# av-savchenko/HSE_FaceRec_tf

Measured on AMD Instinct MI355X. Metric: faces/sec embedding-extract (MobileNet-192, bs=256), higher is better.
Workload: dtype f32

## Files before the change

### hse_facerec_tf_amd/csrc/common.h

```cpp
#pragma once
#include <hip/hip_runtime.h>
#include <stdarg.h>
#include <stdio.h>

#include "../../include/hsefr.h"
#ifdef HSEFR_DEV
#include "hsefr_dev.h"
#endif

namespace hsefr {

void set_error(const char* fmt, ...);

#define HSEFR_HIP_CHECK(expr)                                                          \
    do {                                                                               \
        hipError_t _e = (expr);                                                        \
        if (_e != hipSuccess) {                                                        \
            ::hsefr::set_error("%s failed: %s (%s:%d)", #expr, hipGetErrorString(_e),  \
                               __FILE__, __LINE__);                                    \
            return HSEFR_ERR_HIP;                                                      \
        }                                                                              \
    } while (0)

#define HSEFR_REQUIRE(cond, code, ...)     \
// ... 88 lines not shown
__device__ __forceinline__ unsigned hsefr_udiv_do(unsigned x, hsefr_udiv k) {
    const unsigned q0 = __umulhi(x, k.m);
    return (((x - q0) >> 1) + q0) >> k.sh;
}

__device__ __forceinline__ unsigned xcd_remap_dir(unsigned bid, unsigned nwg, int reverse) {
    const unsigned lt = xcd_remap(bid, nwg);
    return reverse ? nwg - 1u - lt : lt;
}
int sweep_reverse();
void set_sweep_reverse(int v);

#ifdef HSEFR_DEV
#define HSEFR_KNOB(name, value) int name = value
#else
#define HSEFR_KNOB(name, value) constexpr int name = value
#endif

int launch_conv_c3(const float* x, const float* wgt, const float* shift, float* y, int n, int h, int w,
                   int kh, int kw, int stride, int pad_t, int pad_l, int oh, int ow, int cout, int act,
                   hipStream_t s);
int launch_dwconv3x3(const float* x, const float* wgt, const float* scale, const float* shift, float* y,
                     int n, int h, int w, int c, int stride, int pad_t, int pad_l, int oh, int ow, int act,
                     hipStream_t s);
int launch_dwconv3x3_split(const float* x, const float* wgt, const float* scale, const float* shift, void* y_split,
                           int n, int h, int w, int c, int stride, int pad_t, int pad_l, int oh, int ow, int act,
                           int a_log2, hipStream_t s);
int launch_pwconv_f32(const float* x, const float* wgt_t, const float* shift, float* y, long long m, int k,
                      int cout, int act, hipStream_t s);
int launch_pwconv_f16s(const float* x, const void* wsplit, const float* descale, const float* shift, float* y,
                       long long m, int k, int cout, int a_log2, int act, hipStream_t s);
bool pwconv_ps_supported(long long m, int k, int cout);
bool pwconv_ps_gap_supported(long long m, int k, int cout, int map_hw);
int launch_pwconv_ps_gap(const void* xs, const void* wsplit, const float* descale, const float* shift, float* y, long long m, int k, int cout,
                         int act, int map_hw, hipStream_t s);
bool pwconv_ps_dw_supported(long long m, int k, int cout, int map_w, int map_hw, int dw_stride);
int launch_pwconv_ps_dw(const void* xs, const void* wsplit, const float* descale, const float* shift, const float* dwc, void* ys, long long m,
                        int k, int cout, int act, int map_w, int map_hw, int dw_stride, int out_log2, hipStream_t s);
int launch_pwconv_ps(const void* xs, const void* wsplit, const float* descale, const float* shift, float* y, long long m, int k,
                     int cout, int act, hipStream_t s);
int launch_gap(const float* x, float* y, int n, int hw, int c, hipStream_t s);
int launch_dense(const float* x, const float* wgt, const float* bias, float* y, int n, int k, int cout,
                 int act, hipStream_t s);
int launch_softmax(const float* x, float* y, int n, int c, hipStream_t s);
int launch_heads_fused(const float* x, const float* w1, const float* b1, const float* wa, const float* ba, const float* wg, const float* bg,
                       float* hidden, float* logits, float* age_probs, float* gender, int n, int k, int a, hipStream_t s);
int launch_l2_normalize(const float* x, float* y, int n, int d, hipStream_t s);
int launch_nn1(const float* q, const float* g, int nq, int ng, int d, int* nn_index, float* nn_dist2,
               hipStream_t s);
int launch_knn(const float* q, const float* g, int nq, int ng, int d, int k, int* nn_index, float* nn_dist2, const int* g_label, int* pred,
               hipStream_t s);
long long nn1_fallbacks();

int launch_conv_bf16(const void* x, const void* wt, const float* scale, const float* shift, const void* res, void* y,
                     int n, int h, int w, int c, int oh, int ow, int cout, int kh, int kw, int stride, int pad_t,
                     int pad_l, int act, hipStream_t s);
int launch_conv1x1_bf16(const void* x, const void* wt, const float* scale, const float* shift, const void* res, void* y,
                        long long P, int K, int cout, int act, hipStream_t s);
int launch_conv1x1_sres_bf16(const void* x, const void* wt, const float* scale, const float* shift, const void* res, void* y, int n, int oh,
                             int ow, int K, int cout, int stride, int h2, int w2, int act, hipStream_t s);
bool conv1x1_bf16_enabled(bool has_res, int k, int cout);
int launch_conv1x1_proj_bf16(const void* x, const void* wt, const float* scale, const float* shift, const void* x2, const void* wt2,
                             const float* scale2, const float* shift2, void* y, int n, int oh, int ow, int K, int cout, int k2, int stride,
                             int h2, int w2, int act, hipStream_t s);
int launch_stem7x7_bf16(const float* x, const void* wt, const float* scale, const float* shift, void* y, int n, int h,
                        int w, int oh, int ow, int act, hipStream_t s);
int mtcnn_post_capacity();
int launch_mtcnn_stage1_level(const float* prob, const float* reg, int w, int h, double scale, float thr, double* found, int* counters,
                              hipStream_t s);
int launch_mtcnn_stage1_finish(const double* found, int* counters, double* boxes, int* tab, int img_w, int img_h, hipStream_t s);
int launch_mtcnn_stage23_finish(int stage, const double* boxes_in, int n, const float* prob, const float* reg, const float* pts, float thr,
                                double* boxes_out, int* tab_out, float* points_out, int* counters, int img_w, int img_h, hipStream_t s);
int launch_mtcnn_nms(const double* boxes, int n, double thr, int use_min, int* keep, int* n_keep, hipStream_t s);
bool conv3x3_win_forced();
bool conv3x3_win_bf16_supported(long long n, int h, int w, int c, int cout);
int launch_conv3x3_win_bf16(const void* x, const void* wt, const float* scale, const float* shift, const void* res, void* y, int n, int h,
                            int w, int c, int cout, int act, hipStream_t s);
bool conv3x3_w2_forced();
bool conv3x3_w2_bf16_supported(long long n, int h, int w, int c, int cout);
bool conv3x3_w2_bf16_preferred(int h, int w, int cout);
int launch_conv3x3_w2_bf16(const void* x, const void* wt, const float* scale, const float* shift, const void* res, void* y, int n, int h,
                           int w, int c, int cout, int act, hipStream_t s);
bool conv1x1_w4_forced();
bool conv1x1_w4_bf16_supported(long long n, int h, int w, int c, int oh, int ow, int cout, int stride);
bool conv1x1_w4_bf16_preferred(long long pixels, int c, int cout, bool has_res);
bool conv1x1_w4_proj_preferred(long long pixels, int c, int c2, int cout);
int launch_conv1x1_w4_proj_bf16(const void* x, const void* wt, const float* scale, const float* shift, const void* x2, const void* wt2,
                                const float* scale2, const float* shift2, void* y, int n, int oh, int ow, int c, int cout, int c2, int stride2,
                                int h2, int w2, int act, hipStream_t s);
int launch_conv1x1_w4_bf16(const void* x, const void* wt, const float* scale, const float* shift, const void* res, void* y, int n, int h,
                           int w, int c, int oh, int ow, int cout, int stride, int act, hipStream_t s);
bool conv1x1_pair_bf16_shape_supported(int c, int cout1, int cout2, int c2);
bool conv1x1_pair_bf16_supported(long long pixels, int c, int cout1, int cout2, int c2);
int launch_conv1x1_pair_bf16(const void* x, const void* w1, const float* scale1, const float* shift1, const void* res, const void* x2,
                             const void* wp, const float* scale_p, const float* shift_p, void* y1, const void* w2, const float* scale2,
                             const float* shift2, void* y2, long long pixels, int c, int cout1, int cout2, int c2, int act1, int act2,
                             hipStream_t s, int y1_stride = 1, int h = 0, int w = 0);
bool conv_dma_forced();
bool conv_dma_bf16_supported(long long n, int h, int w, int c, int oh, int ow, int cout, int kh, int kw);
int launch_conv_dma_bf16(const void* x, const void* wt, const float* scale, const float* shift, const void* res, void* y, int n, int h,
                         int w, int c, int oh, int ow, int cout, int kh, int kw, int stride, int pad_t, int pad_l, int act, hipStream_t s);
int launch_stem7x7_pool_bf16(const float* x, const void* wt, const float* scale, const float* shift, void* y, int n, int h, int w,
                             int ph, int pw, int pool_pad_t, int pool_pad_l, hipStream_t s, const void* wfrag = nullptr);
bool stem7s_stream_supported(long long n, int h, int w, int ph, int pw);
int launch_stem7s_stream(const float* x, const void* wt, const float* scale, const float* shift, void* y, int n, int h, int w, int ph, int pw,
                         int pool_pad_t, int pool_pad_l, hipStream_t s, const void* wfrag = nullptr);
constexpr size_t STEM7S_WFRAG_BYTES = 4 * 7 * 64 * 16;
int stem7s_reorder_weights(const void* wt, void* wfrag, hipStream_t s);
int launch_maxpool3x3s2_bf16(const void* x, void* y, int n, int h, int w, int c, int oh, int ow, int pad_t, int pad_l,
                             hipStream_t s);
int launch_gap_bf16(const void* x, float* y, int n, int hw, int c, hipStream_t s);

int launch_pil_resize(const unsigned char* in, unsigned char* tmp, float* out, int n, int H, int W, int oh, int ow, const int* xmin,
                      const int* xcnt, const int* xcoef, int xk, const int* ymin, const int* ycnt, const int* ycoef, int yk,
                      int mode, const double* mean, hipStream_t s);
int launch_cv_resize(const unsigned char* in, float* out, int n, int H, int W, int oh, int ow, const int* x0, const int* x1,
                     const int* wx1, const int* y0, const int* y1, const int* wy1, int mode, const double* mean, hipStream_t s);

int launch_area_level(const unsigned char* src, float* dst, int sh, int sw, int dh, int dw, hipStream_t s);
int launch_area_crops(const unsigned char* src, const int* boxes, float* dst, int sh, int sw, int n, int size, hipStream_t s);
int launch_pairwise_dist(const float* x, const float* y, int n, int m, int d, float* out, hipStream_t s);
struct DistSource {
    const float* x;
    int n, d;
    const float* born;
    const float* year;
    const double* dense;
};
int launch_single_linkage(const DistSource& src, int* edge_a, int* edge_b, double* edge_h, hipStream_t s);
int launch_dbscan(const DistSource& src, double eps, int min_samples, int* labels, unsigned char* core, hipStream_t s);
int launch_rank_order(const DistSource& src, const double* thresholds, int pairs, int* labels, int* iterations, hipStream_t s);
int launch_hier_linkage(const DistSource& src, int method, int* merge_a, int* merge_b, double* merge_h, int* merge_round, hipStream_t s);

bool dwpw_fused_supported(int c, int cout, int stride, int act_dw, int act_pw);
int launch_dwpw_fused(const float* x, const float* wd, const float* dscale, const float* dshift, const float* wp_t,
                      const float* pshift, float* y, int n, int h, int w, int c, int stride, int pad_t, int pad_l, int oh,
                      int ow, int cout, int act_dw, int act_pw, hipStream_t s);

int launch_conv2d_direct(const float* x, const float* w, const float* bias, const float* alpha, float* y, int n, int h, int wd, int c,
                         int oh, int ow, int cout, int kh, int kw, int stride, int pad_t, int pad_l, hipStream_t s);
int launch_conv_f32_mfma(const float* x, const float* w, const float* scale, const float* shift, const float* res, float* y, int n, int h,
                         int wd, int c, int oh, int ow, int cout, int kh, int kw, int stride, int pad_t, int pad_l, int act, hipStream_t s,
                         int res_stride = 0, int res_h = 0, int res_w = 0);
bool conv_f32_mfma_supported(int c, int cout);
int launch_conv2d_f32(const float* x, const float* w, const float* scale, const float* shift, const float* res, float* y, int n, int h,
                      int wd, int c, int oh, int ow, int cout, int kh, int kw, int stride, int pad_t, int pad_l, int act, hipStream_t s);
int launch_maxpool_f32(const float* x, float* y, int n, int h, int w, int c, int oh, int ow, int k, int stride, int pad_t, int pad_l,
                       hipStream_t s);

int launch_dwpw_f16s(const float* x, const float* wd, const float* dscale, const float* dshift, const void* wsplit,
                     const float* descale, const float* pshift, float* y, int n, int h, int w, int c, int stride, int pad_t,
                     int pad_l, int oh, int ow, int cout, int a_log2, int act, hipStream_t s);
bool dwpw_f16s_supported(int c, int cout, int stride);
int launch_stem_fused(const float* x, const float* cw, const float* cshift, const float* wd, const float* dscale,
                      const float* dshift, const void* wsplit, const float* descale, const float* pshift, float* y, int n,
                      int h, int w, int cpad_t, int cpad_l, int oh, int ow, int a_log2, int act, hipStream_t s);
int launch_stem2_fused(const float* x, const float* cw, const float* cshift, const float* wd1, const float* d1scale,
                       const float* d1shift, const void* wsplit, const float* descale, const float* pshift, const float* wd2,
                       const float* d2scale, const float* d2shift, float* y, int n, int h, int w, int cpad_t, int cpad_l,
                       int h1, int w1, int pad_t2, int pad_l2, int oh2, int ow2, int a_log2, int act, hipStream_t s);
int launch_stem3_fused(const float* x, const void* cw_split, const float* cdescale, const float* cshift, const float* wd1,
                       const float* d1scale, const float* d1shift, const void* wsplit, const float* descale, const float* pshift,
                       const float* wd2, const float* d2scale, const float* d2shift, float* y, int* overflow, int n, int h, int w,
                       int cpad_t, int cpad_l, int h1, int w1, int pad_t2, int pad_l2, int oh2, int ow2, int in_log2, int a_log2,
                       int act, hipStream_t s);
bool stem3_fused_supported(int cin, int c1, int c2, int conv_stride, int dw1_stride, int dw2_stride, int kh, int kw);
int launch_stem4_fused(const void* x, int x_is_u8, const void* cw4, const float* cdescale, const float* cshift, const float* wd1,
                       const float* d1scale, const float* d1shift, const void* wsplit, const float* descale, const float* pshift,
                       const float* wd2, const float* d2scale, const float* d2shift, float* y, int* overflow, int n, int h, int w,
                       int in_log2, int a_log2, int act, hipStream_t s);
bool stem4_fused_supported(int cin, int c1, int c2, int conv_stride, int dw1_stride, int dw2_stride, int kh, int kw, int h, int w);
int launch_stem5_stream(const void* x, int x_is_u8, const void* cw4, const float* cdescale, const float* cshift, const float* wd1,
                        const float* d1scale, const float* d1shift, const void* wsplit, const float* descale, const float* pshift,
                        const float* wd2, const float* d2scale, const float* d2shift, float* y, int* overflow, int n, int h, int w,
                        int in_log2, int a_log2, int act, hipStream_t s);
bool stem5_stream_supported(int cin, int c1, int c2, int conv_stride, int dw1_stride, int dw2_stride, int kh, int kw, int h, int w);
bool stem2_fused_supported(int cin, int c1, int c2, int conv_stride, int dw1_stride, int dw2_stride, int kh, int kw);
bool stem_fused_supported(int cin, int cmid, int cout, int conv_stride, int dw_stride, int kh, int kw);
int read_pws_stamps(void* host_out, size_t bytes);
int read_stem_stamps(void* host_out, size_t bytes);
#ifdef HSEFR_STEM_STAMPS
unsigned long long* stamp_buffer(hipStream_t s);
#define STEM_STAMP(i) do { const unsigned long long _t = __builtin_amdgcn_s_memtime(); st[i] += _t - tprev; tprev = _t; } while (0)
#define STEM_STAMP_DECL unsigned long long st[8] = {0, 0, 0, 0, 0, 0, 0, 0}; unsigned long long tprev = __builtin_amdgcn_s_memtime(); \
    const unsigned long long tstart = tprev; unsigned npatch = 0
#define STEM_STAMP_COUNT ++npatch
#define STEM_STAMP_FLUSH(buf, lane, wave) do { if ((lane) == 0 && (buf) && blockIdx.x < 512) { unsigned long long* o = (buf) + (blockIdx.x * 4 + (wave)) * 10; \
    for (int i_ = 0; i_ < 8; ++i_) o[i_] = st[i_]; o[8] = __builtin_amdgcn_s_memtime() - tstart; o[9] = npatch; } } while (0)
#else
#define STEM_STAMP(i) do { } while (0)
#define STEM_STAMP_DECL do { } while (0)
#define STEM_STAMP_COUNT do { } while (0)
#define STEM_STAMP_FLUSH(buf, lane, wave) do { } while (0)
#endif
#ifdef HSEFR_DEV
void set_stem4_grid(int v);
void set_stem5_grid(int v);
void set_stem5_segs(int v);
void set_c11(int v);
void set_c11_tile(int v);
void set_c11_bres(int v);
void set_c11_adv(int v);
int read_c11_stamps(void* host_out, size_t bytes);
void set_dwpws_tw(int v);
void set_dwpws_bn(int v);
void set_pw_tile(int v);
void set_pws_tile(int v);
void set_ps_mb(int v);
void set_ps_grid(int v);
void set_psdw_mode(int v);
void set_cd_rb(int v);
void set_w3_off(int v);
void set_w2_off(int v);
void set_w4_off(int v);
void set_w4_bres(int v);
void set_pair_off(int v);
void set_stem7s(int v);
void set_pair_ablate(int v);
void set_pair_nt(int v);
void set_nn1_y_mb(int v);
int read_w4_stamps(void* host_out, size_t bytes);
int read_s7_stamps(void* host_out, size_t bytes);
int read_w2_stamps(void* host_out, size_t bytes);
int read_w3_stamps(void* host_out, size_t bytes);
int read_cd_stamps(void* host_out, size_t bytes);
void set_cd_off(int v);
int read_ps_stamps(void* host_out, size_t bytes);
void set_pw_ablate(int v);
void set_pw_dma(int v);
void set_dw_th(int v);
void set_dw_variant(int v);
void set_dw_look(int v);
void set_dw_look2(int v);
void set_copy_variant(int v);
void set_clock_mode(int v);
void set_c3_impl(int v);
int launch_clock_probe(unsigned long long* out, int blocks, int iters, hipStream_t s);
int launch_copy(const void* src, void* dst, size_t bytes, hipStream_t s);
#endif

}
```

### hse_facerec_tf_amd/csrc/dwpw_f16s.hip

```cpp
#include "common.h"

namespace hsefr {

namespace {

typedef float f32x4 __attribute__((ext_vector_type(4)));
typedef float f32x16 __attribute__((ext_vector_type(16)));
typedef _Float16 f16x4 __attribute__((ext_vector_type(4)));
typedef _Float16 f16x8 __attribute__((ext_vector_type(8)));

struct DwPwSParams {
    const float4* x;
    const float4* wd;
    const float4* dscale;
    const float4* dshift;
    const float* wsplit;
    const float* descale;
    const float* pshift;
    float* y;
    int H, W, C4, KT, OH, OW, Cout, pad_t, pad_l, tiles_w, tiles_h, tiles_n;
    unsigned total;
    float a_scale;
    int reverse;
    int nimg;
    unsigned m_n, m_w, m_h;
    unsigned long long* stamps;
};

constexpr int ROWB = 128;
__device__ __forceinline__ int swzb(int row, int chunk) { return row * ROWB + 16 * (chunk ^ ((row >> 1) & 7) ^ ((row & 1) << 2)); }
__device__ __forceinline__ float4 fma4(float4 a, float4 b, float4 c) {
    return make_float4(fmaf(a.x, b.x, c.x), fmaf(a.y, b.y, c.y), fmaf(a.z, b.z, c.z), fmaf(a.w, b.w, c.w));
}
__device__ __forceinline__ float relu6(float v) { return fminf(fmaxf(v, 0.f), 6.f); }
__device__ __forceinline__ unsigned fastdiv(unsigned x, unsigned m) { return m ? __umulhi(x, m) : x; }

template <int STRIDE, int TW, int BN, int OCC, int ACT>
__global__ __launch_bounds__(256, OCC) void dwpw_f16s_kernel(DwPwSParams p) {
    constexpr int TH = 128 / TW;
    constexpr int U = TW * 8;
    constexpr int RG = 256 / U;
    constexpr int RPT = TH / RG;
    static_assert(RPT == 4, "patch shapes 8x16 and 16x8");
    constexpr int WN = BN / 2, NI = WN / 32, BP = BN / 32;
    __shared__ __attribute__((aligned(16))) unsigned char As[128 * ROWB];
    __shared__ __attribute__((aligned(16))) unsigned char Bs[BN * ROWB];

    const int tid = threadIdx.x;
    const int lane = tid & 63, wave = tid >> 6;
    const int wm = wave >> 1, wn = wave & 1;
    const int li = lane & 31, lh = lane >> 5;
    const int srow = tid >> 3, skq = tid & 7;
    const int u = tid % U, tw = u >> 3, c4l = u & 7;
    const int row0 = (tid / U) * RPT;
    const int arow = wm * 64 + li, brow = wn * WN + li;

    for (unsigned t = blockIdx.x; t < p.total; t += gridDim.x) {
        const unsigned lt = xcd_remap_dir(t, p.total, p.reverse);
        const int n0 = (lt % p.tiles_n) * BN;
        const unsigned pt = lt / p.tiles_n;
        const int ow0 = (pt % p.tiles_w) * TW;
        const int oh0 = ((pt / p.tiles_w) % p.tiles_h) * TH;
        const int n = pt / (p.tiles_w * p.tiles_h);

        const int ow = min(ow0 + tw, p.OW - 1);
        const int iw0 = ow * STRIDE - p.pad_l;
        const float ml = iw0 >= 0 ? 1.f : 0.f, mm = (iw0 + 1 >= 0 && iw0 + 1 < p.W) ? 1.f : 0.f, mr = iw0 + 2 < p.W ? 1.f : 0.f;
        const int cl = max(iw0, 0) * p.C4, cm = min(max(iw0 + 1, 0), p.W - 1) * p.C4, cr = min(iw0 + 2, p.W - 1) * p.C4;
        const float4* ximg = p.x + (size_t)n * p.H * p.W * p.C4;
        const int ih0 = (oh0 + row0) * STRIDE - p.pad_t;
        const float* bsrc = p.wsplit + (size_t)(n0 + srow) * p.KT * 32 + 4 * skq;

        f32x16 acc[2][NI];
#pragma unroll
        for (int mi = 0; mi < 2; ++mi)
#pragma unroll
            for (int ni = 0; ni < NI; ++ni)
#pragma unroll
                for (int r = 0; r < 16; ++r) acc[mi][ni][r] = 0.f;

        for (int kc = 0; kc < p.KT; ++kc) {
            f32x4 rb[BP];
#pragma unroll
            for (int q = 0; q < BP; ++q) rb[q] = *(const f32x4*)(bsrc + (size_t)32 * q * p.KT * 32 + kc * 32);
            const int c4 = kc * 8 + c4l;
            const float4* xin = ximg + c4;
            float4 wk[9];
#pragma unroll
            for (int i = 0; i < 9; ++i) {
                const float m = (i % 3 == 0) ? ml : (i % 3 == 1 ? mm : mr);
                const float4 wr = p.wd[i * p.C4 + c4];
                wk[i] = make_float4(wr.x * m, wr.y * m, wr.z * m, wr.w * m);
            }
            const float4 dsc = p.dscale[c4], dsh = p.dshift[c4];
            struct Row { float4 l, m, r; float k; };
            auto load_row = [&](int ih) {
                Row q;
                const int ihc = min(max(ih, 0), p.H - 1);
                const float4* row = xin + (size_t)ihc * p.W * p.C4;
                q.l = row[cl]; q.m = row[cm]; q.r = row[cr];
                q.k = (ih >= 0 && ih < p.H) ? 1.f : 0.f;
                return q;
            };
            auto row_sum = [&](const Row& q, int b) {
                float4 a = make_float4(q.l.x * wk[b].x, q.l.y * wk[b].y, q.l.z * wk[b].z, q.l.w * wk[b].w);
                a = fma4(q.m, wk[b + 1], a);
                return fma4(q.r, wk[b + 2], a);
            };
            f16x4 ohi[RPT], olo[RPT];
            auto emit = [&](int j, const Row& a, const Row& b, const Row& c) {
                const float4 sa = row_sum(a, 0), sb = row_sum(b, 3), sc = row_sum(c, 6);
                float4 s = make_float4(sa.x * a.k, sa.y * a.k, sa.z * a.k, sa.w * a.k);
                s = make_float4(fmaf(sb.x, b.k, s.x), fmaf(sb.y, b.k, s.y), fmaf(sb.z, b.k, s.z), fmaf(sb.w, b.k, s.w));
                s = make_float4(fmaf(sc.x, c.k, s.x), fmaf(sc.y, c.k, s.y), fmaf(sc.z, c.k, s.z), fmaf(sc.w, c.k, s.w));
                const float4 o = fma4(s, dsc, dsh);
                f32x4 v;
                v[0] = relu6(o.x); v[1] = relu6(o.y); v[2] = relu6(o.z); v[3] = relu6(o.w);
                v = v * p.a_scale;
                ohi[j] = __builtin_convertvector(v, f16x4);
                olo[j] = __builtin_convertvector(v - __builtin_convertvector(ohi[j], f32x4), f16x4);
            };
            if (STRIDE == 1) {
                Row r0 = load_row(ih0), r1 = load_row(ih0 + 1), r2 = load_row(ih0 + 2), r3 = load_row(ih0 + 3);
#pragma unroll
                for (int j = 0; j < RPT; ++j) {
                    const Row r4 = load_row(ih0 + j + 4);
                    emit(j, r0, r1, r2);
                    r0 = r1; r1 = r2; r2 = r3; r3 = r4;
                }
            } else {
                Row r0 = load_row(ih0), r1 = load_row(ih0 + 1), r2 = load_row(ih0 + 2);
#pragma unroll
                for (int j = 0; j < RPT; ++j) {
                    const Row n1 = load_row(ih0 + 2 * j + 3), n2 = load_row(ih0 + 2 * j + 4);
                    emit(j, r0, r1, r2);
                    r0 = r2; r1 = n1; r2 = n2;
                }
            }
            __syncthreads();
#pragma unroll
            for (int j = 0; j < RPT; ++j) {
                const int R = (row0 + j) * TW + tw;
                *(f16x4*)(&As[swzb(R, c4l >> 1) + 8 * (c4l & 1)]) = ohi[j];
                *(f16x4*)(&As[swzb(R, 4 + (c4l >> 1)) + 8 * (c4l & 1)]) = olo[j];
            }
#pragma unroll
            for (int q = 0; q < BP; ++q) *(f32x4*)(&Bs[swzb(srow + 32 * q, skq)]) = rb[q];
            __syncthreads();
#pragma unroll
            for (int s = 0; s < 2; ++s) {
                f16x8 ah[2], al[2], bh[NI], bl[NI];
#pragma unroll
// ... 191 lines not shown
        const int cw = wave - 4, wm = cw / CWN, wn = cw % CWN;
        const int li = lane & 31, lh = lane >> 5;
        const int arow = wm * 64 + li, brow = wn * WN + li;
        const int erow = lane >> 3, ech = lane & 7;
        unsigned bv[BPW];
        unsigned pb_i = 0;
        int pb_kc = 0, pb_step = 0;
        auto setup_b = [&](unsigned i) {
            const Item it = decode(i);
#pragma unroll
            for (int j = 0; j < BPW; ++j) {
                const int r = (cw * BPW + j) * 8 + (lane >> 3);
                bv[j] = ((unsigned)(it.n0 + r) * (unsigned)C + 4u * ((lane & 7) ^ ((r >> 1) & 7) ^ ((r & 1) << 2))) * 4u;
            }
        };
        auto b_dma = [&]() {
            const unsigned base = lds0 + B_OFF + (pb_step & 1) * B_ST;
            const unsigned so = (unsigned)pb_kc * 128u;
#pragma unroll
            for (int j = 0; j < BPW; ++j) piece(rw, base + (cw * BPW + j) * 1024, bv[j], so);
            ++pb_step;
            if (++pb_kc == KT) {
                pb_kc = 0;
                setup_b(++pb_i);
            }
        };
        f32x16 acc[2][NI];
        auto zero_acc = [&]() {
#pragma unroll
            for (int mi = 0; mi < 2; ++mi)
#pragma unroll
                for (int ni = 0; ni < NI; ++ni)
#pragma unroll
                    for (int r = 0; r < 16; ++r) acc[mi][ni][r] = 0.f;
        };
        auto epilogue = [&](const Item& cur, int stage) {
            unsigned char* scr = smem + B_OFF + stage * B_ST + cw * (BPW * 1024);
            const float* el = (const float*)(smem + E_OFF);
            unsigned sv[2][4];
#pragma unroll
            for (int mi = 0; mi < 2; ++mi)
#pragma unroll
                for (int i = 0; i < 4; ++i) {
                    const int R = wm * 64 + mi * 32 + erow + 8 * i;
                    const int oh = cur.oh0 + R / TW, ow = cur.ow0 + R % TW;
                    sv[mi][i] = (oh < p.OH && ow < p.OW)
                                    ? ((unsigned)((cur.n * p.OH + oh) * p.OW + ow) * (unsigned)p.Cout + (unsigned)(cur.n0 + wn * WN + 4 * ech)) * 4u
                                    : OOB;
                }
#pragma unroll
            for (int ni = 0; ni < NI; ++ni) {
                const int nl = cur.n0 + wn * WN + ni * 32 + 4 * ech;
                const f32x4 ds = *(const f32x4*)(el + nl), sh = *(const f32x4*)(el + CMAX2 + nl);
#pragma unroll
                for (int mi = 0; mi < 2; ++mi) {
#pragma unroll
                    for (int j = 0; j < 4; ++j) {
                        f32x4 v;
#pragma unroll
                        for (int e = 0; e < 4; ++e) v[e] = acc[mi][ni][4 * j + e];
                        *(f32x4*)(scr + li * 128 + 16 * ((2 * j + lh) ^ (li & 7))) = v;
                    }
                    f32x4 rv[4];
#pragma unroll
                    for (int i = 0; i < 4; ++i) {
                        const int r = erow + 8 * i;
                        rv[i] = *(const f32x4*)(scr + r * 128 + 16 * (ech ^ (r & 7)));
                    }
#pragma unroll
                    for (int i = 0; i < 4; ++i) {
                        const f32x4 v = rv[i];
                        const f32x4 z = __builtin_elementwise_fma(v, ds, sh);
                        f32x4 o;
#pragma unroll
                        for (int e = 0; e < 4; ++e) o[e] = apply_act<ACT>(z[e]);
                        bstore16_welded(o, ry, sv[mi][i], __builtin_amdgcn_readfirstlane((unsigned)(ni * 32) * 4u));
                    }
                }
            }
        };
        zero_acc();
        setup_b(0);
        Item cur = decode(0);
        unsigned ci = 0;
        int ckc = 0;
        bool pending = false;
        if (HALO_BY_CONSUMER) {
            setup_halo(0);
#pragma unroll
            for (int i = 0; i < HS - 1; ++i)
                if (i < nsteps) halo_dma();
            asm volatile("s_waitcnt vmcnt(0)" ::: "memory");
        }
        __syncthreads();
        for (int g = -1; g < nsteps; ++g) {
            if (pending) {
                epilogue(cur, (g + 1) & 1);
                zero_acc();
                cur = decode(++ci);
                pending = false;
                STEM_STAMP_COUNT;
            }
            STEM_STAMP(5);
            if (pb_step < nsteps) b_dma();
            const bool halo_issued = HALO_BY_CONSUMER && pf_step < nsteps;
            if (halo_issued) halo_dma();
            STEM_STAMP(1);
            if (g >= 0) {
                const unsigned char* As = smem + A_OFF + (g & 1) * (128 * ROWB);
                const unsigned char* Bs = smem + B_OFF + (g & 1) * B_ST;
#pragma unroll
                for (int s = 0; s < 2; ++s) {
                    f16x8 ah[2], al[2], bh[NI], bl[NI];
#pragma unroll
                    for (int mi = 0; mi < 2; ++mi) {
                        ah[mi] = *(const f16x8*)(As + swzb(arow + mi * 32, 2 * s + lh));
                        al[mi] = *(const f16x8*)(As + swzb(arow + mi * 32, 4 + 2 * s + lh));
                    }
#pragma unroll
                    for (int ni = 0; ni < NI; ++ni) {
                        bh[ni] = *(const f16x8*)(Bs + swzb(brow + ni * 32, 2 * s + lh));
                        bl[ni] = *(const f16x8*)(Bs + swzb(brow + ni * 32, 4 + 2 * s + lh));
                    }
#pragma unroll
                    for (int mi = 0; mi < 2; ++mi)
#pragma unroll
                        for (int ni = 0; ni < NI; ++ni) {
                            acc[mi][ni] = __builtin_amdgcn_mfma_f32_32x32x16_f16(bh[ni], al[mi], acc[mi][ni], 0, 0, 0);
                            acc[mi][ni] = __builtin_amdgcn_mfma_f32_32x32x16_f16(bl[ni], ah[mi], acc[mi][ni], 0, 0, 0);
                            acc[mi][ni] = __builtin_amdgcn_mfma_f32_32x32x16_f16(bh[ni], ah[mi], acc[mi][ni], 0, 0, 0);
                        }
                }
                if (++ckc == KT) { ckc = 0; pending = true; }
            }
            STEM_STAMP(4);
            if (HS >= 3 && halo_issued) asm volatile("s_waitcnt vmcnt(%0)" ::"n"(HPW) : "memory");
            else asm volatile("s_waitcnt vmcnt(0)" ::: "memory");
            STEM_STAMP(0);
            __syncthreads();
            STEM_STAMP(3);
        }
        if (pending) { epilogue(cur, (nsteps - 1) & 1); STEM_STAMP_COUNT; }
#ifdef HSEFR_STEM_STAMPS
        if (lane == 0 && p.stamps && blockIdx.x < 256 && cw < 4) {
            unsigned long long* o = p.stamps + ((blockIdx.x + 256) * 4 + cw) * 10;
            for (int i_ = 0; i_ < 8; ++i_) o[i_] = st[i_];
            o[8] = __builtin_amdgcn_s_memtime() - tstart;
            o[9] = npatch;
        }
#endif
    }
}

HSEFR_KNOB(g_tw, 0);
HSEFR_KNOB(g_bn, 0);

template <int STRIDE, int TW, int BN, int OCC>
int launch_t(DwPwSParams& p, int n, int act, hipStream_t s) {
    constexpr int TH = 128 / TW;
    p.tiles_w = (p.OW + TW - 1) / TW;
    p.tiles_h = (p.OH + TH - 1) / TH;
    p.tiles_n = p.Cout / BN;
    const long long total = (long long)n * p.tiles_w * p.tiles_h * p.tiles_n;
    HSEFR_REQUIRE(total < (1ll << 31), HSEFR_ERR_UNSUPPORTED, "dwpw_f16split: grid too large");
    p.total = (unsigned)total;
    const unsigned cap = 256u * OCC;
    const unsigned g = p.total < cap ? p.total : cap;
#define HSEFR_DWPWS(A) HSEFR_LAUNCH((dwpw_f16s_kernel<STRIDE, TW, BN, OCC, A>), dim3(g), dim3(256), 0, s, p)
    if (act == HSEFR_ACT_RELU6) HSEFR_DWPWS(HSEFR_ACT_RELU6);
    else if (act == HSEFR_ACT_RELU) HSEFR_DWPWS(HSEFR_ACT_RELU);
    else if (act == HSEFR_ACT_NONE) HSEFR_DWPWS(HSEFR_ACT_NONE);
    else { set_error("dwpw_f16split: act %d", act); return HSEFR_ERR_UNSUPPORTED; }
#undef HSEFR_DWPWS
    return launch_status("dwpw_f16split");
}

template <int STRIDE, int TW>
int launch_bn(DwPwSParams& p, int n, int bn, int act, hipStream_t s) {
    if (bn == 64) return launch_t<STRIDE, TW, 64, 2>(p, n, act, s);
#ifdef HSEFR_DEV
    if (bn == 256) return launch_t<STRIDE, TW, 256, 2>(p, n, act, s);
#endif
    return launch_t<STRIDE, TW, 128, 2>(p, n, act, s);
}

template <int TW, int BN, int HS>
int launch_v3(DwPwSParams& p, int n, int act, hipStream_t s) {
    constexpr int TH = 128 / TW;
    p.tiles_w = (p.OW + TW - 1) / TW;
    p.tiles_h = (p.OH + TH - 1) / TH;
    p.tiles_n = p.Cout / BN;
    const long long total = (long long)n * p.tiles_w * p.tiles_h * p.tiles_n;
    HSEFR_REQUIRE(total < (1ll << 31) / 16, HSEFR_ERR_UNSUPPORTED, "dwpw_f16split: grid too large");
    p.total = (unsigned)total;
    auto magic = [](unsigned d) { return d == 1 ? 0u : (unsigned)((0x100000000ull + d - 1) / d); };
    p.m_n = magic(p.tiles_n); p.m_w = magic(p.tiles_w); p.m_h = magic(p.tiles_h);
    HSEFR_REQUIRE(total * (long long)(p.tiles_n > p.tiles_w ? (p.tiles_n > p.tiles_h ? p.tiles_n : p.tiles_h) : (p.tiles_w > p.tiles_h ? p.tiles_w : p.tiles_h)) < (1ll << 32),
                  HSEFR_ERR_UNSUPPORTED, "dwpw_f16split: grid too large for the quotient multipliers");
    const unsigned g = p.total < 256u ? p.total : 256u;
#define HSEFR_DWPW3(A) HSEFR_LAUNCH((dwpw3_f16s_kernel<TW, BN, HS, A>), dim3(g), dim3(256 + 64 * (BN == 256 ? 8 : 4)), 0, s, p)
    if (act == HSEFR_ACT_RELU6) HSEFR_DWPW3(HSEFR_ACT_RELU6);
    else if (act == HSEFR_ACT_RELU) HSEFR_DWPW3(HSEFR_ACT_RELU);
    else if (act == HSEFR_ACT_NONE) HSEFR_DWPW3(HSEFR_ACT_NONE);
    else { set_error("dwpw_f16split: act %d", act); return HSEFR_ERR_UNSUPPORTED; }
#undef HSEFR_DWPW3
    return launch_status("dwpw_f16split");
}

}

#ifdef HSEFR_DEV
void set_dwpws_tw(int v) { g_tw = v; }
void set_dwpws_bn(int v) { g_bn = v; }
#endif

bool dwpw_f16s_supported(int c, int cout, int stride) {
    return c > 0 && c % 32 == 0 && cout > 0 && cout % 64 == 0 && (stride == 1 || stride == 2);
}

int launch_dwpw_f16s(const float* x, const float* wd, const float* dscale, const float* dshift, const void* wsplit,
                     const float* descale, const float* pshift, float* y, int n, int h, int w, int c, int stride, int pad_t,
                     int pad_l, int oh, int ow, int cout, int a_log2, int act, hipStream_t s) {
    HSEFR_REQUIRE(dwpw_f16s_supported(c, cout, stride), HSEFR_ERR_UNSUPPORTED,
                  "dwpw_f16split: c=%d cout=%d stride=%d not covered (c %% 32, cout %% 64, stride 1|2)", c, cout, stride);
    HSEFR_REQUIRE(n >= 0 && h > 0 && w > 0 && oh > 0 && ow > 0, HSEFR_ERR_INVALID, "dwpw_f16split: bad shape");
    HSEFR_REQUIRE(a_log2 > 0 && a_log2 <= 12, HSEFR_ERR_INVALID, "dwpw_f16split: a_log2=%d (the depthwise result is in [0,6]: 1..12)", a_log2);
    if (n == 0) return HSEFR_OK;
    DwPwSParams p;
    p.x = (const float4*)x; p.wd = (const float4*)wd; p.dscale = (const float4*)dscale; p.dshift = (const float4*)dshift;
    p.wsplit = (const float*)wsplit; p.descale = descale; p.pshift = pshift; p.y = y;
    p.H = h; p.W = w; p.C4 = c / 4; p.KT = c / 32; p.OH = oh; p.OW = ow; p.Cout = cout; p.pad_t = pad_t; p.pad_l = pad_l;
    p.a_scale = ldexpf(1.f, a_log2);
    p.reverse = sweep_reverse();
    p.nimg = n;
    p.stamps = nullptr;
#ifdef HSEFR_STEM_STAMPS
    p.stamps = stamp_buffer(s);
#endif
    const long long in_bytes = (long long)n * h * w * c * 4, out_bytes = (long long)n * oh * ow * cout * 4;
    if (stride == 1 && c <= 256 && cout <= CMAX2 && cout % 128 == 0 && in_bytes < (1ll << 32) - 16 && out_bytes < (1ll << 32) - 16) {
        auto padded = [&](int tw) { const int th = 128 / tw; return (long long)((ow + tw - 1) / tw * tw) * ((oh + th - 1) / th * th); };
        int tw = padded(16) <= padded(8) ? 16 : 8;
        if (g_tw == 8 || g_tw == 16) tw = g_tw;
        int bn = cout % 256 == 0 ? 256 : 128;
        if ((g_bn == 128 || g_bn == 256) && cout % g_bn == 0) bn = g_bn;
        if (bn == 256) return tw == 16 ? launch_v3<16, 256, 2>(p, n, act, s) : launch_v3<8, 256, 2>(p, n, act, s);
        return tw == 16 ? launch_v3<16, 128, 3>(p, n, act, s) : launch_v3<8, 128, 3>(p, n, act, s);
    }
    int bn = cout % 128 == 0 ? 128 : 64;
    if (g_bn && cout % g_bn == 0) bn = g_bn;
    int tw = (ow % 16 == 0 || ow % 8 != 0) ? 16 : 8;
    if (ow <= 8) tw = 8;
    if (g_tw == 8 || g_tw == 16) tw = g_tw;
    if (stride == 1) return tw == 16 ? launch_bn<1, 16>(p, n, bn, act, s) : launch_bn<1, 8>(p, n, bn, act, s);
    return tw == 16 ? launch_bn<2, 16>(p, n, bn, act, s) : launch_bn<2, 8>(p, n, bn, act, s);
}

}
```

### hse_facerec_tf_amd/csrc/engine.hip

```cpp
#include <math.h>
#include <string.h>

#include <cxxabi.h>
#include <dlfcn.h>
#include <elf.h>

#include <map>
#include <new>
#include <string>
#include <vector>

#include "common.h"

namespace hsefr {

static thread_local char g_err[512] = "";

void set_error(const char* fmt, ...) {
    va_list ap;
    va_start(ap, fmt);
    vsnprintf(g_err, sizeof(g_err), fmt, ap);
    va_end(ap);
}

// ... 114 lines not shown
                          "plan op %u: input exceeds buffer %d", i, o.in_buf);
        }
        HSEFR_REQUIRE(o.res_buf != o.out_buf, HSEFR_ERR_INVALID, "plan op %u: residual aliases the output", i);
        auto need = [&](uint64_t off, uint64_t bytes, const char* what) {
            if (off != HSEFR_NO_OFFSET && off + bytes <= h.blob_bytes) return true;
            set_error("plan op %u (kind %u): operand %s missing or %llu bytes beyond the %llu-byte blob", i, o.kind, what,
                      (unsigned long long)bytes, (unsigned long long)h.blob_bytes);
            return false;
        };
        const uint64_t co = o.cout, ci = o.cin, kk = (uint64_t)o.kh * o.kw;
        const Geometry g = geometry(o.aux);
        switch (o.kind) {
            case HSEFR_OP_GAP: case HSEFR_OP_SOFTMAX: case HSEFR_OP_MAXPOOL_BF16: case HSEFR_OP_GAP_BF16: case HSEFR_OP_MAXPOOL_F32:
                break;
            case HSEFR_OP_CONV_F32:
                if (!need(o.w_off, kk * ci * co * 4, "kernel")) return HSEFR_ERR_INVALID;
                if (o.scale_off != HSEFR_NO_OFFSET && !need(o.scale_off, co * 4, "scale")) return HSEFR_ERR_INVALID;
                if (o.shift_off != HSEFR_NO_OFFSET && !need(o.shift_off, co * 4, "shift")) return HSEFR_ERR_INVALID;
                HSEFR_REQUIRE(o.cout % 4 == 0, HSEFR_ERR_UNSUPPORTED, "plan op %u: fp32 convolution with cout=%d (must be a multiple of 4)", i, o.cout);
                if (o.aux != 0) {
                    HSEFR_REQUIRE(g.c2 == 0 && o.kh == 1 && o.kw == 1 && o.stride == 1 && o.pad_t == 0 && o.pad_l == 0 && o.res_buf >= 0 && g.stride2 >= 1 &&
                                      o.oh == o.h && o.ow == o.w && o.oh * o.ow > 1 && o.ow > 1 && (o.oh - 1) * g.stride2 < g.h2 &&
                                      (o.ow - 1) * g.stride2 < g.w2 && conv_f32_mfma_supported(o.cin, o.cout),
                                  HSEFR_ERR_INVALID, "plan op %u: bad strided residual (stride %d, %dx%d)", i, g.stride2, g.h2, g.w2);
                    HSEFR_REQUIRE((uint64_t)g.h2 * g.w2 * co * 4 <= bufs[o.res_buf].elems_per_image * bufs[o.res_buf].elem_bytes, HSEFR_ERR_INVALID,
                                  "plan op %u: strided residual exceeds buffer %d", i, o.res_buf);
                }
                break;
            case HSEFR_OP_CONV_C3:
                if (!need(o.w_off, kk * ci * co * 4, "kernel") || !need(o.shift_off, co * 4, "shift")) return HSEFR_ERR_INVALID;
                break;
            case HSEFR_OP_DWCONV3X3:
                if (!need(o.w_off, 9 * ci * 4, "kernel") || !need(o.scale_off, ci * 4, "scale") || !need(o.shift_off, ci * 4, "shift"))
                    return HSEFR_ERR_INVALID;
                HSEFR_REQUIRE(o.aux == 0 || (o.aux > 0 && o.aux <= 12 && o.act == HSEFR_ACT_RELU6 && o.cin % 32 == 0),
                              HSEFR_ERR_INVALID, "plan op %u: split-row depthwise output needs ReLU6, c %% 32 == 0 and a_log2 in [1, 12]", i);
                break;
            case HSEFR_OP_PWCONV_F32:
                if (!need(o.w_off, ci * co * 4, "kernel") || !need(o.shift_off, co * 4, "shift")) return HSEFR_ERR_INVALID;
                break;
            case HSEFR_OP_DENSE:
                if (!need(o.w_off, ci * co * 4, "kernel")) return HSEFR_ERR_INVALID;
                if (o.shift_off != HSEFR_NO_OFFSET && !need(o.shift_off, co * 4, "bias")) return HSEFR_ERR_INVALID;
                break;
            case HSEFR_OP_CONV_BF16:
                if (!need(o.w_off, kk * ci * co * 2, "kernel") || !need(o.scale_off, co * 4, "scale") || !need(o.shift_off, co * 4, "shift"))
                    return HSEFR_ERR_INVALID;
                if (o.w2_off != HSEFR_NO_OFFSET) {
                    HSEFR_REQUIRE(o.kh == 1 && o.kw == 1 && o.stride == 1 && o.res_buf >= 0 && g.c2 > 0 && g.c2 % 64 == 0 && g.stride2 >= 1 &&
                                      (o.oh - 1) * g.stride2 < g.h2 && (o.ow - 1) * g.stride2 < g.w2,
                                  HSEFR_ERR_INVALID, "plan op %u: bad projected shortcut (k2 %d, stride %d, %dx%d)", i, g.c2, g.stride2, g.h2, g.w2);
                    if (!need(o.w2_off, (uint64_t)g.c2 * co * 2, "projection kernel") || !need(o.shift2_off, 2 * co * 4, "projection scale / shift"))
                        return HSEFR_ERR_INVALID;
                    HSEFR_REQUIRE((uint64_t)g.h2 * g.w2 * g.c2 * 2 <= bufs[o.res_buf].elems_per_image * bufs[o.res_buf].elem_bytes, HSEFR_ERR_INVALID,
                                  "plan op %u: projected shortcut input exceeds buffer %d", i, o.res_buf);
                } else if (o.aux != 0) {
                    HSEFR_REQUIRE(g.c2 == 0 && o.kh == 1 && o.kw == 1 && o.stride == 1 && o.pad_t == 0 && o.pad_l == 0 && o.res_buf >= 0 && g.stride2 >= 1 &&
                                      o.oh == o.h && o.ow == o.w && o.oh * o.ow > 1 && o.ow > 1 && (o.oh - 1) * g.stride2 < g.h2 && (o.ow - 1) * g.stride2 < g.w2,
                                  HSEFR_ERR_INVALID, "plan op %u: bad strided residual (stride %d, %dx%d)", i, g.stride2, g.h2, g.w2);
                    HSEFR_REQUIRE((uint64_t)g.h2 * g.w2 * co * 2 <= bufs[o.res_buf].elems_per_image * bufs[o.res_buf].elem_bytes, HSEFR_ERR_INVALID,
                                  "plan op %u: strided residual exceeds buffer %d", i, o.res_buf);
                }
                break;
            case HSEFR_OP_STEM7X7_POOL_BF16:
                HSEFR_REQUIRE(o.act == HSEFR_ACT_RELU && (o.aux & ~(1 | 1 << HSEFR_AUX_POOL_PAD_L_SHIFT)) == 0 && o.cin == 3 && o.cout == 64, HSEFR_ERR_INVALID,
                              "plan op %u: fused stem + pool needs ReLU, 3 -> 64 channels and pool pads in {0, 1}", i);
                [[fallthrough]];
            case HSEFR_OP_STEM7X7_BF16:
                if (!need(o.w_off, 64 * 256 * 2, "kernel") || !need(o.scale_off, co * 4, "scale") || !need(o.shift_off, co * 4, "shift"))
                    return HSEFR_ERR_INVALID;
                break;
            case HSEFR_OP_PWCONV_PS_GAP:
                HSEFR_REQUIRE(pwconv_ps_gap_supported(0, o.cin, o.cout, o.h * o.w) && o.oh == 1 && o.ow == 1, HSEFR_ERR_UNSUPPORTED,
                              "plan op %u: fused pointwise + global pool on a %dx%d map not covered (33 .. 288 pixels)", i, o.h, o.w);
                if (!need(o.w_off, ci * co * 4, "split rows") || !need(o.scale_off, co * 4, "descale") || !need(o.shift_off, co * 4, "shift"))
                    return HSEFR_ERR_INVALID;
                HSEFR_REQUIRE(o.aux > 0 && o.aux <= 24, HSEFR_ERR_INVALID, "plan op %u: a_log2 out of range (reserved %d)", i, o.aux);
                break;
            case HSEFR_OP_PWCONV_PS_DW:
                HSEFR_REQUIRE(pwconv_ps_dw_supported(0, o.cin, o.cout, o.w, o.h * o.w, o.stride) && o.oh * o.stride == o.h && o.ow * o.stride == o.w &&
                                  (o.stride == 1 ? (o.pad_t == 1 && o.pad_l == 1) : (o.pad_t == 0 && o.pad_l == 0)),
                              HSEFR_ERR_UNSUPPORTED, "plan op %u: fused pointwise + depthwise (stride %d) on a %dx%d map not covered", i, o.stride, o.h, o.w);
                if (!need(o.w_off, ci * co * 4, "split rows") || !need(o.scale_off, co * 4, "descale") || !need(o.shift_off, co * 4, "shift") ||
                    !need(o.w2_off, 11 * co * 4, "depthwise constants"))
                    return HSEFR_ERR_INVALID;
                {
                    const PsDwAux a = ps_dw_aux(o.aux);
                    HSEFR_REQUIRE(a.a_log2 > 0 && a.a_log2 <= 24 && a.out_log2 >= 1 && a.out_log2 <= 12,
                                  HSEFR_ERR_INVALID, "plan op %u: a_log2 / out_log2 out of range (reserved %d)", i, o.aux);
                }
                break;
            case HSEFR_OP_PWCONV_PS:
                HSEFR_REQUIRE(pwconv_ps_supported(0, o.cin, o.cout), HSEFR_ERR_UNSUPPORTED,
                              "plan op %u: pre-split pointwise cin=%d cout=%d not covered", i, o.cin, o.cout);
                [[fallthrough]];
            case HSEFR_OP_PWCONV_F16S:
                if (!need(o.w_off, ci * co * 4, "split rows") || !need(o.scale_off, co * 4, "descale") || !need(o.shift_off, co * 4, "shift"))
                    return HSEFR_ERR_INVALID;
                HSEFR_REQUIRE(o.w_off != HSEFR_NO_OFFSET && o.scale_off != HSEFR_NO_OFFSET && o.shift_off != HSEFR_NO_OFFSET &&
                                  o.aux > 0 && o.aux <= 24,
                              HSEFR_ERR_INVALID, "plan op %u: split-f16 pointwise needs split rows, descale, shift and a_log2 in (0, 24]", i);
                break;
            case HSEFR_OP_STEM3_F16S: {
                const StemAux a = stem_aux(o.aux);
                HSEFR_REQUIRE(stem3_fused_supported(o.cin, 32, o.cout, o.stride, 1, 2, o.kh, stem_kw(o.kw).k) && a.a_log2 > 0 && a.a_log2 <= 12 &&
                                  a.in_log2 >= -8 && a.in_log2 <= 14 &&
                                  o.w_off != HSEFR_NO_OFFSET && o.w2_off != HSEFR_NO_OFFSET && o.shift2_off != HSEFR_NO_OFFSET &&
                                  o.w_off + HSEFR_STEM_PACK_STEM3_END * 4 <= h.blob_bytes && o.w2_off + 64 * 128 <= h.blob_bytes &&
                                  o.shift2_off + 128 * 4 <= h.blob_bytes && o.in_buf == HSEFR_BUF_INPUT,
                              HSEFR_ERR_UNSUPPORTED, "plan op %u: bounded fused stem cin=%d cout=%d stride=%d not covered", i, o.cin, o.cout, o.stride);
                break;
            }
            case HSEFR_OP_STEM2_F16S:
                HSEFR_REQUIRE(stem2_fused_supported(o.cin, 32, o.cout, o.stride, 1, 2, o.kh, stem_kw(o.kw).k) && o.aux > 0 && o.aux <= 12 &&
                                  o.w_off != HSEFR_NO_OFFSET && o.w2_off != HSEFR_NO_OFFSET && o.shift2_off != HSEFR_NO_OFFSET &&
                                  o.w_off + HSEFR_STEM_PACK_STEM2_END * 4 <= h.blob_bytes && o.in_buf == HSEFR_BUF_INPUT,
                              HSEFR_ERR_UNSUPPORTED, "plan op %u: fused stem+dw2 cin=%d cout=%d stride=%d not covered", i, o.cin, o.cout, o.stride);
                break;
            case HSEFR_OP_STEM_F16S:
#ifndef HSEFR_DEV
                set_error("plan op %u: HSEFR_OP_STEM_F16S (round 1's fused stem) runs on development builds of the library only", i);
                return HSEFR_ERR_UNSUPPORTED;
#else
                HSEFR_REQUIRE(stem_fused_supported(o.cin, 32, o.cout, o.stride, 1, o.kh, o.kw) && o.aux > 0 && o.aux <= 12 &&
                                  o.w_off != HSEFR_NO_OFFSET && o.w2_off != HSEFR_NO_OFFSET && o.shift2_off != HSEFR_NO_OFFSET &&
                                  o.w_off + HSEFR_STEM_PACK_DW2 * 4 <= h.blob_bytes && o.in_buf == HSEFR_BUF_INPUT,
                              HSEFR_ERR_UNSUPPORTED, "plan op %u: fused stem cin=%d cout=%d stride=%d not covered", i, o.cin, o.cout, o.stride);
                break;
#endif
            case HSEFR_OP_DWPW_F16S:
                if (!need(o.w_off, 9 * ci * 4, "depthwise kernel") || !need(o.scale_off, ci * 4, "scale") || !need(o.shift_off, ci * 4, "shift") ||
                    !need(o.w2_off, ci * co * 4, "split rows") || !need(o.shift2_off, 2 * co * 4, "descale | shift"))
                    return HSEFR_ERR_INVALID;
                HSEFR_REQUIRE(dwpw_f16s_supported(o.cin, o.cout, o.stride) && o.aux > 0 && o.aux <= 12 &&
                                  o.w_off != HSEFR_NO_OFFSET && o.scale_off != HSEFR_NO_OFFSET && o.shift_off != HSEFR_NO_OFFSET &&
                                  o.w2_off != HSEFR_NO_OFFSET && o.shift2_off != HSEFR_NO_OFFSET,
                              HSEFR_ERR_UNSUPPORTED, "plan op %u: split-f16 fused block cin=%d cout=%d stride=%d a_log2=%d not covered",
                              i, o.cin, o.cout, o.stride, o.aux);
                break;
            case HSEFR_OP_DWPW_F32:
                if (!need(o.w_off, 9 * ci * 4, "depthwise kernel") || !need(o.scale_off, ci * 4, "scale") || !need(o.shift_off, ci * 4, "shift") ||
                    !need(o.w2_off, ci * co * 4, "pointwise kernel") || !need(o.shift2_off, co * 4, "pointwise shift"))
                    return HSEFR_ERR_INVALID;
                HSEFR_REQUIRE(dwpw_fused_supported(o.cin, o.cout, o.stride, HSEFR_ACT_RELU6, (int)o.act), HSEFR_ERR_UNSUPPORTED,
                              "plan op %u: fused depthwise-pointwise block cin=%d cout=%d not covered", i, o.cin, o.cout);
                break;
            default:
                set_error("plan op %u: unknown kind %u", i, o.kind);
                return HSEFR_ERR_UNSUPPORTED;
        }
    }
    for (uint32_t i = 0; i < h.n_ops; ++i) {
        const hsefr_plan_op& o = ops[i];
        HSEFR_REQUIRE((o.flags & ~(HSEFR_OPF_PAIR_NEXT | HSEFR_OPF_HEADS | HSEFR_OPF_OUT_SUB2)) == 0, HSEFR_ERR_INVALID, "plan op %u: unknown flags 0x%x", i, o.flags);
        HSEFR_REQUIRE(!(o.flags & HSEFR_OPF_OUT_SUB2) || (o.flags & HSEFR_OPF_PAIR_NEXT), HSEFR_ERR_INVALID, "plan op %u: OUT_SUB2 without PAIR_NEXT", i);
        if (o.flags & HSEFR_OPF_PAIR_NEXT) {
            HSEFR_REQUIRE(i + 1 < h.n_ops, HSEFR_ERR_INVALID, "plan op %u: PAIR_NEXT on the last op", i);
            const hsefr_plan_op& b = ops[i + 1];
            const bool proj = o.w2_off != HSEFR_NO_OFFSET;
            const Geometry g = geometry(o.aux);
            const int c2 = proj ? g.c2 : 0;
            const bool sub2 = (o.flags & HSEFR_OPF_OUT_SUB2) != 0;
            HSEFR_REQUIRE(o.kind == HSEFR_OP_CONV_BF16 && b.kind == HSEFR_OP_CONV_BF16 && o.kh == 1 && o.kw == 1 && o.stride == 1 && o.pad_t == 0 &&
                              o.pad_l == 0 && (sub2 ? (o.oh == (o.h + 1) / 2 && o.ow == (o.w + 1) / 2 && o.h > 1 && o.w > 1) : (o.oh == o.h && o.ow == o.w)) &&
                              b.kh == 1 && b.kw == 1 && b.stride == 1 && b.pad_t == 0 && b.pad_l == 0 &&
                              b.h == o.h && b.w == o.w && b.oh == b.h && b.ow == b.w && b.cin == o.cout && b.in_buf == o.out_buf &&
                              b.res_buf == HSEFR_BUF_NONE && b.w2_off == HSEFR_NO_OFFSET && b.flags == 0 && o.res_buf >= 0 &&
                              (!proj || (g.stride2 == 1 && g.h2 == o.h && g.w2 == o.w)),
                          HSEFR_ERR_INVALID, "plan op %u: PAIR_NEXT needs two 1x1 stride-1 bf16 convolutions at the same pixels, the first with a residual "
                          "or a same-pixel projected shortcut, the second reading the first", i);
            HSEFR_REQUIRE(b.out_buf != o.in_buf && b.out_buf != o.res_buf && b.out_buf != o.out_buf, HSEFR_ERR_INVALID,
                          "plan op %u: PAIR_NEXT: the second output (buffer %d) aliases an operand of the first", i, b.out_buf);
            HSEFR_REQUIRE(conv1x1_pair_bf16_shape_supported(o.cin, o.cout, b.cout, c2), HSEFR_ERR_UNSUPPORTED,
                          "plan op %u: PAIR_NEXT %d -> %d -> %d (projection from %d) not covered", i, o.cin, o.cout, b.cout, c2);
        }
        if (o.flags & HSEFR_OPF_HEADS) {
            HSEFR_REQUIRE(i + 3 < h.n_ops, HSEFR_ERR_INVALID, "plan op %u: HEADS needs three ops behind it", i);
            const hsefr_plan_op &a = ops[i + 1], &sm = ops[i + 2], &g = ops[i + 3];
            HSEFR_REQUIRE(o.kind == HSEFR_OP_DENSE && o.act == HSEFR_ACT_RELU && o.cout == 256 && o.cin > 0 && o.cin % 256 == 0 && o.cin <= 2048 &&
                              o.shift_off != HSEFR_NO_OFFSET && a.kind == HSEFR_OP_DENSE && a.act == HSEFR_ACT_NONE && a.cin == 256 && a.cout >= 1 &&
                              a.cout <= 128 && a.in_buf == o.out_buf && a.shift_off != HSEFR_NO_OFFSET && sm.kind == HSEFR_OP_SOFTMAX &&
                              sm.in_buf == a.out_buf && sm.cout == a.cout && g.kind == HSEFR_OP_DENSE && g.act == HSEFR_ACT_SIGMOID && g.cin == 256 &&
                              g.cout == 1 && g.in_buf == o.out_buf && g.shift_off != HSEFR_NO_OFFSET && a.flags == 0 && sm.flags == 0 && g.flags == 0,
                          HSEFR_ERR_INVALID, "plan op %u: HEADS needs DENSE k -> 256 + ReLU, DENSE 256 -> a (<= 128) + bias, SOFTMAX, DENSE 256 -> 1 + sigmoid", i);
            const int outs[4] = {o.out_buf, a.out_buf, sm.out_buf, g.out_buf};
            for (int x = 0; x < 4; ++x) {
                HSEFR_REQUIRE(outs[x] != o.in_buf, HSEFR_ERR_INVALID, "plan op %u: HEADS: an output aliases the pooled features", i);
                for (int y = x + 1; y < 4; ++y)
                    HSEFR_REQUIRE(outs[x] != outs[y], HSEFR_ERR_INVALID, "plan op %u: HEADS: two of the four tensors share buffer %d", i, outs[x]);
            }
        }
    }
    for (int s = 0; s < HSEFR_N_OUTPUT_SLOTS; ++s) {
        HSEFR_REQUIRE(h.out_buffer[s] == HSEFR_BUF_NONE || (h.out_buffer[s] >= 0 && h.out_buffer[s] < (int)h.n_buffers),
                      HSEFR_ERR_INVALID, "plan: output slot %d names buffer %d", s, h.out_buffer[s]);
        if (h.out_buffer[s] == HSEFR_BUF_NONE) continue;
        const int b = h.out_buffer[s];
        uint32_t producers = 0;
        for (uint32_t i = 0; i < h.n_ops; ++i) producers += (ops[i].out_buf == b);
        HSEFR_REQUIRE(producers == 1, HSEFR_ERR_INVALID, "plan: output slot %d: buffer %d has %u producing ops (must be exactly 1)", s, b,
                      producers);
        HSEFR_REQUIRE((uint64_t)bufs[b].elems_per_image * bufs[b].elem_bytes == (uint64_t)h.out_elems[s] * 4, HSEFR_ERR_INVALID,
                      "plan: output slot %d: buffer %d holds %llu x %u bytes per image, the slot declares %u fp32 elements", s, b,
                      (unsigned long long)bufs[b].elems_per_image, (unsigned)bufs[b].elem_bytes, h.out_elems[s]);
    }
    return HSEFR_OK;
}

namespace hsefr {
#ifdef HSEFR_STEM_STAMPS
static unsigned long long* g_stamp_buf = nullptr;
unsigned long long* stamp_buffer(hipStream_t s) {
    if (!g_stamp_buf && hipMalloc((void**)&g_stamp_buf, 512 * 4 * 10 * 8) != hipSuccess) return nullptr;
    (void)hipMemsetAsync(g_stamp_buf, 0, 512 * 4 * 10 * 8, s);
    return g_stamp_buf;
}
int read_stem_stamps(void* host_out, size_t bytes) {
    HSEFR_REQUIRE(g_stamp_buf && bytes <= 512 * 4 * 10 * 8, HSEFR_ERR_INVALID, "read_stem_stamps: nothing recorded / too many bytes");
    HSEFR_HIP_CHECK(hipMemcpy(host_out, g_stamp_buf, bytes, hipMemcpyDeviceToHost));
    return HSEFR_OK;
}
#else
int read_stem_stamps(void* host_out, size_t bytes) {
    (void)host_out; (void)bytes;
    set_error("read_stem_stamps: library built without -DHSEFR_STEM_STAMPS");
    return HSEFR_ERR_UNSUPPORTED;
}
#endif
static thread_local std::string* g_route_sink = nullptr;
bool route_probe() { return g_route_sink != nullptr; }
static const std::map<uintptr_t, std::string>& stub_names() {
    static const std::map<uintptr_t, std::string> table = [] {
        std::map<uintptr_t, std::string> m;
        Dl_info info;
        if (!dladdr(reinterpret_cast<const void*>(&stub_names), &info) || !info.dli_fname) return m;
        FILE* f = fopen(info.dli_fname, "rb");
        if (!f) return m;
        std::vector<unsigned char> img;
        fseek(f, 0, SEEK_END);
        const long sz = ftell(f);
        fseek(f, 0, SEEK_SET);
        if (sz > 0) { img.resize((size_t)sz); if (fread(img.data(), 1, img.size(), f) != img.size()) img.clear(); }
        fclose(f);
        if (img.size() < sizeof(Elf64_Ehdr)) return m;
        const Elf64_Ehdr* eh = reinterpret_cast<const Elf64_Ehdr*>(img.data());
        if (memcmp(eh->e_ident, ELFMAG, SELFMAG) != 0 || eh->e_shentsize != sizeof(Elf64_Shdr) ||
            eh->e_shoff + (uint64_t)eh->e_shnum * sizeof(Elf64_Shdr) > img.size()) return m;
        const Elf64_Shdr* sh = reinterpret_cast<const Elf64_Shdr*>(img.data() + eh->e_shoff);
        for (int i = 0; i < eh->e_shnum; ++i) {
            if (sh[i].sh_type != SHT_SYMTAB || sh[i].sh_link >= eh->e_shnum) continue;
            const Elf64_Shdr& st = sh[sh[i].sh_link];
            if (sh[i].sh_offset + sh[i].sh_size > img.size() || st.sh_offset + st.sh_size > img.size()) continue;
            const Elf64_Sym* sym = reinterpret_cast<const Elf64_Sym*>(img.data() + sh[i].sh_offset);
            const char* str = reinterpret_cast<const char*>(img.data() + st.sh_offset);
            for (size_t k = 0; k < sh[i].sh_size / sizeof(Elf64_Sym); ++k) {
                if (ELF64_ST_TYPE(sym[k].st_info) != STT_OBJECT || sym[k].st_name >= st.sh_size) continue;
                const char* nm = str + sym[k].st_name;
                if (strncmp(nm, "_ZN5hsefr", 9) != 0 || !strstr(nm, "_kernel")) continue;
                int status = 0;
                char* dm = abi::__cxa_demangle(nm, nullptr, nullptr, &status);
                std::string t = (status == 0 && dm) ? dm : nm;
                free(dm);
                size_t cut = std::string::npos, depth = 0;
                for (size_t q = 0; q < t.size(); ++q) {
                    if (t[q] == '<') ++depth;
                    else if (t[q] == '>') --depth;
                    else if (t[q] == '(' && depth == 0 && q > 0 && t.compare(q, 21, "(anonymous namespace)") != 0) { cut = q; break; }
                }
                if (cut != std::string::npos) t.erase(cut);
                for (const char* ns : {"void ", "hsefr::", "(anonymous namespace)::", "__device_stub__"})
                    for (size_t q; (q = t.find(ns)) != std::string::npos;) t.erase(q, strlen(ns));
                m[(uintptr_t)info.dli_fbase + sym[k].st_value] = t;
            }
        }
        return m;
    }();
    return table;
}
void route_record(const void* host_stub, const char* expr) {
    if (!g_route_sink) return;
    const auto& tab = stub_names();
    const auto it = tab.find((uintptr_t)host_stub);
    std::string t = it != tab.end() ? it->second : std::string(expr ? expr : "?");
    if (!g_route_sink->empty() && g_route_sink->back() != '\t') *g_route_sink += " + ";
    *g_route_sink += t;
}
static thread_local int g_sweep_reverse = 0;
int sweep_reverse() { return g_sweep_reverse; }
void set_sweep_reverse(int v) { g_sweep_reverse = v; }
}
HSEFR_KNOB(g_sweep_alternate, 1);
HSEFR_KNOB(g_stem5, 1);
HSEFR_KNOB(g_heads_off, 0);
HSEFR_KNOB(g_stem4, 1);

#pragma GCC visibility push(default)
extern "C" {

int hsefr_version(void) { return HSEFR_VERSION; }

const char* hsefr_last_error_string(void) { return g_err; }

#ifdef HSEFR_DEV
int hsefr_debug_set(const char* key, int value) {
    HSEFR_REQUIRE(key, HSEFR_ERR_INVALID, "debug_set: null key");
    if (!strcmp(key, "pw_tile")) { set_pw_tile(value); return HSEFR_OK; }
    if (!strcmp(key, "pws_tile")) { set_pws_tile(value); return HSEFR_OK; }
    if (!strcmp(key, "ps_mb")) { set_ps_mb(value); return HSEFR_OK; }
    if (!strcmp(key, "ps_grid")) { set_ps_grid(value); return HSEFR_OK; }
    if (!strcmp(key, "psdw_mode")) { set_psdw_mode(value); return HSEFR_OK; }
    if (!strcmp(key, "cd_rb")) { set_cd_rb(value); return HSEFR_OK; }
    if (!strcmp(key, "cd_off")) { set_cd_off(value); return HSEFR_OK; }
    if (!strcmp(key, "w3_off")) { set_w3_off(value); return HSEFR_OK; }
    if (!strcmp(key, "w2_off")) { set_w2_off(value); return HSEFR_OK; }
    if (!strcmp(key, "w4_off")) { set_w4_off(value); return HSEFR_OK; }
    if (!strcmp(key, "w4_bres")) { set_w4_bres(value); return HSEFR_OK; }
    if (!strcmp(key, "nn1_y_mb")) { set_nn1_y_mb(value); return HSEFR_OK; }
    if (!strcmp(key, "c11")) { set_c11(value); return HSEFR_OK; }
    if (!strcmp(key, "c11_tile")) { set_c11_tile(value); return HSEFR_OK; }
    if (!strcmp(key, "c11_bres")) { set_c11_bres(value); return HSEFR_OK; }
    if (!strcmp(key, "c11_adv")) { set_c11_adv(value); return HSEFR_OK; }
    if (!strcmp(key, "stem4_grid")) { set_stem4_grid(value); return HSEFR_OK; }
    if (!strcmp(key, "stem4")) { g_stem4 = value; return HSEFR_OK; }
    if (!strcmp(key, "stem5")) { g_stem5 = value; return HSEFR_OK; }
    if (!strcmp(key, "stem5_grid")) { set_stem5_grid(value); return HSEFR_OK; }
    if (!strcmp(key, "stem5_segs")) { set_stem5_segs(value); return HSEFR_OK; }
    if (!strcmp(key, "pair_off")) { set_pair_off(value); return HSEFR_OK; }
    if (!strcmp(key, "stem7s")) { set_stem7s(value); return HSEFR_OK; }
    if (!strcmp(key, "pair_ablate")) { set_pair_ablate(value); return HSEFR_OK; }
    if (!strcmp(key, "pair_nt")) { set_pair_nt(value); return HSEFR_OK; }
    if (!strcmp(key, "heads_off")) { g_heads_off = value; return HSEFR_OK; }
    if (!strcmp(key, "dw_look")) { set_dw_look(value); return HSEFR_OK; }
    if (!strcmp(key, "dw_look2")) { set_dw_look2(value); return HSEFR_OK; }
    if (!strcmp(key, "sweep_alternate")) { g_sweep_alternate = value; return HSEFR_OK; }
    if (!strcmp(key, "clock_mode")) { set_clock_mode(value); return HSEFR_OK; }
    if (!strcmp(key, "dwpws_tw")) { set_dwpws_tw(value); return HSEFR_OK; }
    if (!strcmp(key, "dwpws_bn")) { set_dwpws_bn(value); return HSEFR_OK; }
    if (!strcmp(key, "pw_ablate")) { set_pw_ablate(value); return HSEFR_OK; }
    if (!strcmp(key, "pw_dma")) { set_pw_dma(value); return HSEFR_OK; }
    if (!strcmp(key, "dw_th")) { set_dw_th(value); return HSEFR_OK; }
    if (!strcmp(key, "dw_variant")) { set_dw_variant(value); return HSEFR_OK; }
    if (!strcmp(key, "copy_variant")) { set_copy_variant(value); return HSEFR_OK; }
    if (!strcmp(key, "c3_impl")) { set_c3_impl(value); return HSEFR_OK; }
    set_error("debug_set: unknown key %s", key);
    return HSEFR_ERR_INVALID;
}

int hsefr_debug_copy(const void* d_src, void* d_dst, size_t bytes, hsefr_stream_t stream) {
    HSEFR_REQUIRE(bytes == 0 || (d_src && d_dst), HSEFR_ERR_INVALID, "debug_copy: null pointer");
    return launch_copy(d_src, d_dst, bytes, (hipStream_t)stream);
}

int hsefr_debug_read_stamps(int kernel, void* host_out, size_t bytes) {
    switch (kernel) {
        case HSEFR_STAMPS_PWS: return read_pws_stamps(host_out, bytes);
        case HSEFR_STAMPS_STEM: return read_stem_stamps(host_out, bytes);
        case HSEFR_STAMPS_PS: return read_ps_stamps(host_out, bytes);
        case HSEFR_STAMPS_CD: return read_cd_stamps(host_out, bytes);
        case HSEFR_STAMPS_C11: return read_c11_stamps(host_out, bytes);
        case HSEFR_STAMPS_W4: return read_w4_stamps(host_out, bytes);
        case HSEFR_STAMPS_W2: return read_w2_stamps(host_out, bytes);
        case HSEFR_STAMPS_W3: return read_w3_stamps(host_out, bytes);
        case HSEFR_STAMPS_S7: return read_s7_stamps(host_out, bytes);
        default: set_error("debug_read_stamps: unknown kernel id %d", kernel); return HSEFR_ERR_INVALID;
    }
}

int hsefr_debug_clock_probe(unsigned long long* d_out, int blocks, int iters, hsefr_stream_t stream) {
    return launch_clock_probe(d_out, blocks, iters, (hipStream_t)stream);
}
#endif

static int check_plan_blob(const void* plan, size_t plan_bytes, hsefr_plan_header& h, std::vector<hsefr_plan_buffer>& bufs,
                           std::vector<hsefr_plan_op>& ops, const char*& blob) {
    HSEFR_REQUIRE(plan, HSEFR_ERR_INVALID, "plan: null pointer");
    HSEFR_REQUIRE(plan_bytes >= sizeof(hsefr_plan_header), HSEFR_ERR_INVALID, "engine_create: plan too short");
    memcpy(&h, plan, sizeof(h));
    HSEFR_REQUIRE(h.magic == HSEFR_PLAN_MAGIC && h.version == 2, HSEFR_ERR_INVALID, "engine_create: bad plan magic/version");
    const unsigned long long tables = sizeof(h) + (unsigned long long)h.n_buffers * sizeof(hsefr_plan_buffer) +
                                      (unsigned long long)h.n_ops * sizeof(hsefr_plan_op);
    HSEFR_REQUIRE(tables <= plan_bytes && h.blob_bytes == plan_bytes - tables, HSEFR_ERR_INVALID,
                  "engine_create: plan is %zu bytes, header implies %llu + %llu", plan_bytes, tables, (unsigned long long)h.blob_bytes);
    HSEFR_REQUIRE(h.n_buffers > 0 && h.n_ops > 0, HSEFR_ERR_INVALID, "engine_create: plan without %s", h.n_ops ? "buffers" : "ops");
    const char* p = (const char*)plan + sizeof(h);
    try {
        bufs.resize(h.n_buffers);
        ops.resize(h.n_ops);
    } catch (const std::bad_alloc&) {
        set_error("engine_create: out of host memory for %u buffers / %u ops", h.n_buffers, h.n_ops);
        return HSEFR_ERR_NOMEM;
    }
    memcpy(bufs.data(), p, h.n_buffers * sizeof(hsefr_plan_buffer));
    p += h.n_buffers * sizeof(hsefr_plan_buffer);
    memcpy(ops.data(), p, h.n_ops * sizeof(hsefr_plan_op));
    blob = p + h.n_ops * sizeof(hsefr_plan_op);
    return validate_plan(h, bufs.data(), ops.data());
}

int hsefr_plan_validate(const void* plan, size_t plan_bytes) {
    hsefr_plan_header h;
    std::vector<hsefr_plan_buffer> bufs;
    std::vector<hsefr_plan_op> ops;
    const char* blob = nullptr;
    return check_plan_blob(plan, plan_bytes, h, bufs, ops, blob);
}

int hsefr_engine_create(const void* plan, size_t plan_bytes, int max_batch, hsefr_engine** out) {
    HSEFR_REQUIRE(plan && out, HSEFR_ERR_INVALID, "engine_create: null argument");
    *out = nullptr;
    HSEFR_REQUIRE(max_batch > 0, HSEFR_ERR_INVALID, "engine_create: max_batch=%d", max_batch);
    hsefr_engine* e = new (std::nothrow) hsefr_engine();
    HSEFR_REQUIRE(e, HSEFR_ERR_NOMEM, "engine_create: out of host memory");
    const char* p = nullptr;
    int rc = check_plan_blob(plan, plan_bytes, e->hdr, e->bufs, e->ops, p);
    if (rc != HSEFR_OK) { delete e; return rc; }
    const hsefr_plan_header& h = e->hdr;
    e->max_batch = max_batch;

    auto fail = [&](int code) { hsefr_engine_destroy(e); return code; };
    if (hipGetDevice(&e->device) != hipSuccess) { set_error("engine_create: hipGetDevice failed"); return fail(HSEFR_ERR_HIP); }
    if (h.blob_bytes) {
        if (hipMalloc((void**)&e->d_blob, h.blob_bytes) != hipSuccess) {
            set_error("engine_create: hipMalloc(%llu) for weights failed", (unsigned long long)h.blob_bytes);
            return fail(HSEFR_ERR_NOMEM);
        }
        if (hipMemcpy(e->d_blob, p, h.blob_bytes, hipMemcpyHostToDevice) != hipSuccess) {
            set_error("engine_create: weight upload failed");
            return fail(HSEFR_ERR_HIP);
        }
        e->device_bytes += h.blob_bytes;
    }
    if (hipMalloc((void**)&e->d_overflow, 16) != hipSuccess || hipMemset(e->d_overflow, 0, 16) != hipSuccess) {
        set_error("engine_create: hipMalloc for the overflow flag failed");
        return fail(HSEFR_ERR_NOMEM);
    }
    e->d_derived.assign(e->ops.size(), nullptr);
    for (size_t i = 0; i < e->ops.size(); ++i) {
        const hsefr_plan_op& o = e->ops[i];
        if (o.kind != HSEFR_OP_STEM7X7_POOL_BF16) continue;
        if (hipMalloc(&e->d_derived[i], STEM7S_WFRAG_BYTES) != hipSuccess) {
            set_error("engine_create: hipMalloc for the stem's fragment-ordered weights failed");
            return fail(HSEFR_ERR_NOMEM);
        }
        e->device_bytes += STEM7S_WFRAG_BYTES;
        if (int rc = stem7s_reorder_weights(blob_ptr(e, o.w_off), e->d_derived[i], nullptr)) return fail(rc);
        if (hipStreamSynchronize(nullptr) != hipSuccess) { set_error("engine_create: re-ordering the stem's weights failed"); return fail(HSEFR_ERR_HIP); }
    }
    e->d_bufs.assign(h.n_buffers, nullptr);
    for (uint32_t i = 0; i < h.n_buffers; ++i) {
        const size_t bytes = (size_t)e->bufs[i].elems_per_image * e->bufs[i].elem_bytes * max_batch;
        if (hipMalloc(&e->d_bufs[i], bytes ? bytes : 16) != hipSuccess) {
            set_error("engine_create: hipMalloc(%zu) for activation buffer %u failed", bytes, i);
            return fail(HSEFR_ERR_NOMEM);
        }
        e->device_bytes += bytes;
    }
    *out = e;
    return HSEFR_OK;
}

size_t hsefr_engine_workspace_bytes(const hsefr_engine* e) { return e ? e->device_bytes : 0; }
int hsefr_engine_max_batch(const hsefr_engine* e) { return e ? e->max_batch : 0; }

void* hsefr_engine_buffer(hsefr_engine* e, int buffer) {
    if (!e || buffer < 0 || buffer >= (int)e->d_bufs.size()) return nullptr;
    return e->d_bufs[buffer];
}

int hsefr_engine_copy_buffer(hsefr_engine* e, int buffer, void* d_dst, size_t bytes, hsefr_stream_t stream) {
    HSEFR_REQUIRE(e && d_dst, HSEFR_ERR_INVALID, "copy_buffer: null argument");
    HSEFR_REQUIRE(buffer >= 0 && buffer < (int)e->d_bufs.size(), HSEFR_ERR_INVALID, "copy_buffer: buffer %d", buffer);
    const size_t cap = (size_t)e->bufs[buffer].elems_per_image * e->bufs[buffer].elem_bytes * e->max_batch;
    HSEFR_REQUIRE(bytes <= cap, HSEFR_ERR_SHAPE, "copy_buffer: %zu bytes exceed buffer %d (%zu)", bytes, buffer, cap);
    HSEFR_HIP_CHECK(hipMemcpyAsync(d_dst, e->d_bufs[buffer], bytes, hipMemcpyDeviceToDevice, (hipStream_t)stream));
    return HSEFR_OK;
}

int hsefr_engine_set_profiling(hsefr_engine* e, int depth) {
    HSEFR_REQUIRE(e && depth >= 0, HSEFR_ERR_INVALID, "set_profiling: bad argument");
    for (auto ev : e->events) (void)hipEventDestroy(ev);
    e->events.clear();
    e->prof_depth = 0;
    e->prof_calls = 0;
    if (depth > 0) {
        e->events.resize((size_t)depth * (e->ops.size() + 1));
        for (auto& ev : e->events) HSEFR_HIP_CHECK(hipEventCreate(&ev));
        e->prof_depth = depth;
    }
    return HSEFR_OK;
}

long long hsefr_engine_profiled_calls(const hsefr_engine* e) { return e ? e->prof_calls : 0; }

int hsefr_engine_op_times_ms(hsefr_engine* e, int slot, float* ms, int n_ops) {
    HSEFR_REQUIRE(e && ms, HSEFR_ERR_INVALID, "op_times: null argument");
    HSEFR_REQUIRE(e->prof_depth > 0 && slot >= 0 && slot < e->prof_depth && slot < e->prof_calls, HSEFR_ERR_INVALID,
                  "op_times: slot %d has no profiled forward (depth %d, calls %lld)", slot, e->prof_depth, e->prof_calls);
    HSEFR_REQUIRE(n_ops == (int)e->ops.size(), HSEFR_ERR_INVALID, "op_times: expected %zu ops", e->ops.size());
    hipEvent_t* ev = e->events.data() + (size_t)slot * (e->ops.size() + 1);
    HSEFR_HIP_CHECK(hipEventSynchronize(ev[n_ops]));
    for (int i = 0; i < n_ops; ++i) HSEFR_HIP_CHECK(hipEventElapsedTime(&ms[i], ev[i], ev[i + 1]));
    return HSEFR_OK;
}

static int run_ops(hsefr_engine* e, const std::vector<void*>& tab, const void* d_input, int n, const std::vector<char>& needed,
                   hipStream_t s, hipEvent_t* pev, bool input_u8 = false) {
    const bool prof = pev != nullptr;
    unsigned launches = 0;
    if (prof) HSEFR_HIP_CHECK(hipEventRecord(pev[0], s));
    for (size_t i = 0; i < e->ops.size(); ++i) {
        const hsefr_plan_op& o = e->ops[i];
        if (!needed[i]) {
            if (prof) HSEFR_HIP_CHECK(hipEventRecord(pev[i + 1], s));
            continue;
        }
        const void* in = buf_ptr(tab, o.in_buf, d_input);
        void* out = buf_ptr(tab, o.out_buf, d_input);
        int rc = HSEFR_OK;
        size_t covered = 0;
        set_sweep_reverse(g_sweep_alternate ? (int)(launches++ & 1) : 0);
        const bool sub2 = (o.flags & HSEFR_OPF_OUT_SUB2) != 0;
        const Geometry g = geometry(o.aux);
        const int c2 = o.w2_off != HSEFR_NO_OFFSET ? g.c2 : 0;
        const bool pair_ok = (o.flags & HSEFR_OPF_PAIR_NEXT) && needed[i + 1] &&
                             conv1x1_pair_bf16_supported((long long)n * o.h * o.w, o.cin, o.cout, e->ops[i + 1].cout, c2);
        HSEFR_REQUIRE(!sub2 || pair_ok, HSEFR_ERR_UNSUPPORTED, "forward: op %zu stores its output at every second pixel (OUT_SUB2) and cannot run without the pair launch", i);
        if (pair_ok) {
            const hsefr_plan_op& b = e->ops[i + 1];
            const bool proj = o.w2_off != HSEFR_NO_OFFSET;
            const float* ssp = (const float*)blob_ptr(e, o.shift2_off);
            rc = launch_conv1x1_pair_bf16(in, blob_ptr(e, o.w_off), (const float*)blob_ptr(e, o.scale_off), (const float*)blob_ptr(e, o.shift_off),
                                          proj ? nullptr : tab[o.res_buf], proj ? tab[o.res_buf] : nullptr, proj ? blob_ptr(e, o.w2_off) : nullptr,
                                          proj ? ssp : nullptr, proj ? ssp + o.cout : nullptr, out, blob_ptr(e, b.w_off),
                                          (const float*)blob_ptr(e, b.scale_off), (const float*)blob_ptr(e, b.shift_off), tab[b.out_buf],
                                          (long long)n * o.h * o.w, o.cin, o.cout, b.cout, c2, o.act, b.act, s, sub2 ? 2 : 1, o.h, o.w);
            covered = 1;
        } else if ((o.flags & HSEFR_OPF_HEADS) && !g_heads_off && needed[i + 1] && needed[i + 2] && needed[i + 3]) {
            const hsefr_plan_op &a = e->ops[i + 1], &sm = e->ops[i + 2], &g = e->ops[i + 3];
            rc = launch_heads_fused((const float*)in, (const float*)blob_ptr(e, o.w_off), (const float*)blob_ptr(e, o.shift_off),
                                    (const float*)blob_ptr(e, a.w_off), (const float*)blob_ptr(e, a.shift_off), (const float*)blob_ptr(e, g.w_off),
                                    (const float*)blob_ptr(e, g.shift_off), (float*)out, (float*)tab[a.out_buf], (float*)tab[sm.out_buf],
                                    (float*)tab[g.out_buf], n, o.cin, a.cout, s);
            covered = 3;
        } else
        switch (o.kind) {
            case HSEFR_OP_CONV_C3:
                rc = launch_conv_c3((const float*)in, (const float*)blob_ptr(e, o.w_off),
                                    (const float*)blob_ptr(e, o.shift_off), (float*)out, n, o.h, o.w, o.kh, o.kw,
                                    o.stride, o.pad_t, o.pad_l, o.oh, o.ow, o.cout, o.act, s);
                break;
            case HSEFR_OP_DWCONV3X3:
                if (o.aux > 0)
                    rc = launch_dwconv3x3_split((const float*)in, (const float*)blob_ptr(e, o.w_off),
                                                (const float*)blob_ptr(e, o.scale_off), (const float*)blob_ptr(e, o.shift_off),
                                                out, n, o.h, o.w, o.cin, o.stride, o.pad_t, o.pad_l, o.oh, o.ow, o.act, o.aux, s);
                else
                    rc = launch_dwconv3x3((const float*)in, (const float*)blob_ptr(e, o.w_off),
                                          (const float*)blob_ptr(e, o.scale_off), (const float*)blob_ptr(e, o.shift_off),
                                          (float*)out, n, o.h, o.w, o.cin, o.stride, o.pad_t, o.pad_l, o.oh, o.ow, o.act, s);
                break;
            case HSEFR_OP_PWCONV_PS_GAP:
                rc = launch_pwconv_ps_gap(in, blob_ptr(e, o.w_off), (const float*)blob_ptr(e, o.scale_off), (const float*)blob_ptr(e, o.shift_off),
                                          (float*)out, (long long)n * o.h * o.w, o.cin, o.cout, o.act, o.h * o.w, s);
                break;
            case HSEFR_OP_PWCONV_PS_DW:
                rc = launch_pwconv_ps_dw(in, blob_ptr(e, o.w_off), (const float*)blob_ptr(e, o.scale_off), (const float*)blob_ptr(e, o.shift_off),
                                         (const float*)blob_ptr(e, o.w2_off), out, (long long)n * o.h * o.w, o.cin, o.cout, o.act, o.w,
                                         o.h * o.w, o.stride, ps_dw_aux(o.aux).out_log2, s);
                break;
            case HSEFR_OP_PWCONV_PS:
                rc = launch_pwconv_ps(in, blob_ptr(e, o.w_off), (const float*)blob_ptr(e, o.scale_off),
                                      (const float*)blob_ptr(e, o.shift_off), (float*)out, (long long)n * o.h * o.w, o.cin, o.cout,
                                      o.act, s);
                break;
            case HSEFR_OP_PWCONV_F32:
                rc = launch_pwconv_f32((const float*)in, (const float*)blob_ptr(e, o.w_off),
                                       (const float*)blob_ptr(e, o.shift_off), (float*)out,
                                       (long long)n * o.h * o.w, o.cin, o.cout, o.act, s);
                break;
            case HSEFR_OP_PWCONV_F16S:
                rc = launch_pwconv_f16s((const float*)in, blob_ptr(e, o.w_off), (const float*)blob_ptr(e, o.scale_off),
                                        (const float*)blob_ptr(e, o.shift_off), (float*)out, (long long)n * o.h * o.w,
                                        o.cin, o.cout, o.aux, o.act, s);
                break;
            case HSEFR_OP_GAP:
                rc = launch_gap((const float*)in, (float*)out, n, o.h * o.w, o.cin, s);
                break;
            case HSEFR_OP_DENSE:
                rc = launch_dense((const float*)in, (const float*)blob_ptr(e, o.w_off),
                                  (const float*)blob_ptr(e, o.shift_off), (float*)out, n, o.cin, o.cout, o.act, s);
                break;
            case HSEFR_OP_SOFTMAX:
                rc = launch_softmax((const float*)in, (float*)out, n, o.cout, s);
                break;
            case HSEFR_OP_CONV_BF16:
                if (o.w2_off != HSEFR_NO_OFFSET) {
                    const float* ss2 = (const float*)blob_ptr(e, o.shift2_off);
                    rc = launch_conv1x1_proj_bf16(in, blob_ptr(e, o.w_off), (const float*)blob_ptr(e, o.scale_off),
                                                  (const float*)blob_ptr(e, o.shift_off), tab[o.res_buf], blob_ptr(e, o.w2_off), ss2, ss2 + o.cout,
                                                  out, n, o.oh, o.ow, o.cin, o.cout, g.c2, g.stride2, g.h2, g.w2, o.act, s);
                    break;
                }
                if (o.res_buf >= 0 && o.aux != 0) {
                    rc = launch_conv1x1_sres_bf16(in, blob_ptr(e, o.w_off), (const float*)blob_ptr(e, o.scale_off), (const float*)blob_ptr(e, o.shift_off),
                                                  tab[o.res_buf], out, n, o.oh, o.ow, o.cin, o.cout, g.stride2, g.h2, g.w2, o.act, s);
                    break;
                }
                rc = launch_conv_bf16(in, blob_ptr(e, o.w_off), (const float*)blob_ptr(e, o.scale_off),
                                      (const float*)blob_ptr(e, o.shift_off),
                                      o.res_buf >= 0 ? tab[o.res_buf] : nullptr, out, n, o.h, o.w, o.cin, o.oh,
                                      o.ow, o.cout, o.kh, o.kw, o.stride, o.pad_t, o.pad_l, o.act, s);
                break;
            case HSEFR_OP_CONV_F32:
                if (conv_f32_mfma_supported(o.cin, o.cout)) {
                    rc = launch_conv_f32_mfma((const float*)in, (const float*)blob_ptr(e, o.w_off), (const float*)blob_ptr(e, o.scale_off),
                                              (const float*)blob_ptr(e, o.shift_off), o.res_buf >= 0 ? (const float*)tab[o.res_buf] : nullptr,
                                              (float*)out, n, o.h, o.w, o.cin, o.oh, o.ow, o.cout, o.kh, o.kw, o.stride, o.pad_t, o.pad_l, o.act, s,
                                              o.res_buf >= 0 ? g.stride2 : 0, g.h2, g.w2);
                    break;
                }
                rc = launch_conv2d_f32((const float*)in, (const float*)blob_ptr(e, o.w_off), (const float*)blob_ptr(e, o.scale_off),
                                       (const float*)blob_ptr(e, o.shift_off), o.res_buf >= 0 ? (const float*)tab[o.res_buf] : nullptr,
                                       (float*)out, n, o.h, o.w, o.cin, o.oh, o.ow, o.cout, o.kh, o.kw, o.stride, o.pad_t, o.pad_l, o.act, s);
                break;
            case HSEFR_OP_MAXPOOL_F32:
                rc = launch_maxpool_f32((const float*)in, (float*)out, n, o.h, o.w, o.cin, o.oh, o.ow, o.kh, o.stride, o.pad_t, o.pad_l, s);
                break;
            case HSEFR_OP_STEM7X7_BF16:
                rc = launch_stem7x7_bf16((const float*)in, blob_ptr(e, o.w_off), (const float*)blob_ptr(e, o.scale_off),
                                         (const float*)blob_ptr(e, o.shift_off), out, n, o.h, o.w, o.oh, o.ow, o.act, s);
                break;
            case HSEFR_OP_STEM7X7_POOL_BF16:
                rc = launch_stem7x7_pool_bf16((const float*)in, blob_ptr(e, o.w_off), (const float*)blob_ptr(e, o.scale_off),
                                              (const float*)blob_ptr(e, o.shift_off), out, n, o.h, o.w, o.oh, o.ow, pool_pads(o.aux).t,
                                              pool_pads(o.aux).l, s, i < e->d_derived.size() ? e->d_derived[i] : nullptr);
                break;
            case HSEFR_OP_MAXPOOL_BF16:
                rc = launch_maxpool3x3s2_bf16(in, out, n, o.h, o.w, o.cin, o.oh, o.ow, o.pad_t, o.pad_l, s);
                break;
            case HSEFR_OP_GAP_BF16:
                rc = launch_gap_bf16(in, (float*)out, n, o.h * o.w, o.cin, s);
                break;
            case HSEFR_OP_DWPW_F32:
                rc = launch_dwpw_fused((const float*)in, (const float*)blob_ptr(e, o.w_off), (const float*)blob_ptr(e, o.scale_off),
                                       (const float*)blob_ptr(e, o.shift_off), (const float*)blob_ptr(e, o.w2_off),
                                       (const float*)blob_ptr(e, o.shift2_off), (float*)out, n, o.h, o.w, o.cin, o.stride,
                                       o.pad_t, o.pad_l, o.oh, o.ow, o.cout, HSEFR_ACT_RELU6, o.act, s);
                break;
            case HSEFR_OP_STEM3_F16S: {
                const StemPack p = stem_pack(e, o);
                const StemAux a = stem_aux(o.aux);
                const StemKw kw = stem_kw(o.kw);
                const int h1 = (o.h + 1) / 2, w1 = (o.w + 1) / 2;
                if (input_u8) {
                    rc = (g_stem5 ? launch_stem5_stream : launch_stem4_fused)(in, 1, p.conv4_u8, p.u8_descale, p.u8_shift, p.dw1, p.dw1_scale, p.dw1_shift,
                                                                            blob_ptr(e, o.w2_off), p.descale, p.pshift, p.dw2, p.dw2_scale, p.dw2_shift,
                                                                            (float*)out, nullptr, n, o.h, o.w, 0, a.a_log2, o.act, s);
                    break;
                }
                if (g_stem4 && stem4_route(o)) {
                    rc = (g_stem5 ? launch_stem5_stream : launch_stem4_fused)(in, 0, p.conv4, p.conv_descale, p.conv_shift, p.dw1, p.dw1_scale, p.dw1_shift,
                                                                            blob_ptr(e, o.w2_off), p.descale, p.pshift, p.dw2, p.dw2_scale, p.dw2_shift,
                                                                            (float*)out, e->d_overflow, n, o.h, o.w, a.in_log2, a.a_log2, o.act, s);
                    break;
                }
                rc = launch_stem3_fused((const float*)in, p.conv_split, p.conv_descale, p.conv_shift, p.dw1, p.dw1_scale, p.dw1_shift,
                                        blob_ptr(e, o.w2_off), p.descale, p.pshift, p.dw2, p.dw2_scale, p.dw2_shift, (float*)out, e->d_overflow, n,
                                        o.h, o.w, o.pad_t, o.pad_l, h1, w1, kw.pad_t2, kw.pad_l2, o.oh, o.ow, a.in_log2, a.a_log2, o.act, s);
                break;
            }
            case HSEFR_OP_STEM2_F16S: {
                const StemPack p = stem_pack(e, o);
                const StemKw kw = stem_kw(o.kw);
                const int h1 = (o.h + 1) / 2, w1 = (o.w + 1) / 2;
                rc = launch_stem2_fused((const float*)in, p.conv, p.conv_shift, p.dw1, p.dw1_scale, p.dw1_shift, blob_ptr(e, o.w2_off), p.descale,
                                        p.pshift, p.dw2, p.dw2_scale, p.dw2_shift, (float*)out, n, o.h, o.w, o.pad_t, o.pad_l, h1, w1,
                                        kw.pad_t2, kw.pad_l2, o.oh, o.ow, o.aux, o.act, s);
                break;
            }
#ifdef HSEFR_DEV
            case HSEFR_OP_STEM_F16S: {
                const StemPack p = stem_pack(e, o);
                rc = launch_stem_fused((const float*)in, p.conv, p.conv_shift, p.dw1, p.dw1_scale, p.dw1_shift, blob_ptr(e, o.w2_off), p.descale,
                                       p.pshift, (float*)out, n, o.h, o.w, o.pad_t, o.pad_l, o.oh, o.ow, o.aux, o.act, s);
                break;
            }
#endif
            case HSEFR_OP_DWPW_F16S: {
                const float* ds2 = (const float*)blob_ptr(e, o.shift2_off);
                rc = launch_dwpw_f16s((const float*)in, (const float*)blob_ptr(e, o.w_off), (const float*)blob_ptr(e, o.scale_off),
                                      (const float*)blob_ptr(e, o.shift_off), blob_ptr(e, o.w2_off), ds2, ds2 + o.cout,
                                      (float*)out, n, o.h, o.w, o.cin, o.stride, o.pad_t, o.pad_l, o.oh, o.ow, o.cout,
                                      o.aux, o.act, s);
                break;
            }
            default:
                set_error("forward: op %zu has unknown kind %u", i, o.kind);
                rc = HSEFR_ERR_UNSUPPORTED;
        }
        if (rc != HSEFR_OK) return rc;
        for (size_t k = 0; k <= covered; ++k)
            if (prof) HSEFR_HIP_CHECK(hipEventRecord(pev[i + 1 + k], s));
        i += covered;
    }
    set_sweep_reverse(0);
    return HSEFR_OK;
}

static int engine_forward(hsefr_engine* e, const void* d_input, bool input_u8, int n, void* d_features, void* d_age_probs,
                          void* d_gender, hsefr_stream_t stream);

int hsefr_engine_forward(hsefr_engine* e, const void* d_input, int n, void* d_features, void* d_age_probs,
                         void* d_gender, hsefr_stream_t stream) {
    return engine_forward(e, d_input, false, n, d_features, d_age_probs, d_gender, stream);
}

int hsefr_engine_accepts_u8(const hsefr_engine* e) {
    if (!e || e->ops.empty()) return 0;
    const hsefr_plan_op& o = e->ops[0];
    return o.kind == HSEFR_OP_STEM3_F16S && o.in_buf == HSEFR_BUF_INPUT && stem_aux(o.aux).u8 && stem4_route(o);
}

int hsefr_engine_forward_u8(hsefr_engine* e, const void* d_input_u8, int n, void* d_features, void* d_age_probs,
                            void* d_gender, hsefr_stream_t stream) {
    HSEFR_REQUIRE(e, HSEFR_ERR_INVALID, "forward_u8: null engine");
    HSEFR_REQUIRE(hsefr_engine_accepts_u8(e), HSEFR_ERR_UNSUPPORTED,
                  "forward_u8: this plan takes no uint8 input (it needs the fused stem lowered with a BGR mean and an input whose "
                  "edges are multiples of 4)");
    return engine_forward(e, d_input_u8, true, n, d_features, d_age_probs, d_gender, stream);
}

static int engine_forward(hsefr_engine* e, const void* d_input, bool input_u8, int n, void* d_features, void* d_age_probs,
                          void* d_gender, hsefr_stream_t stream) {
    HSEFR_REQUIRE(e, HSEFR_ERR_INVALID, "forward: null engine");
    HSEFR_REQUIRE(d_input || n == 0, HSEFR_ERR_INVALID, "forward: null input");
    HSEFR_REQUIRE(n >= 0 && n <= e->max_batch, HSEFR_ERR_SHAPE, "forward: batch %d outside [0, %d]", n, e->max_batch);
    void* outs[HSEFR_N_OUTPUT_SLOTS] = {d_features, d_age_probs, d_gender};
    for (int s = 0; s < HSEFR_N_OUTPUT_SLOTS; ++s)
        HSEFR_REQUIRE(!outs[s] || e->hdr.out_buffer[s] != HSEFR_BUF_NONE, HSEFR_ERR_INVALID,
                      "forward: the plan does not produce output slot %d", s);
    if (n == 0) return HSEFR_OK;
    hipStream_t s = (hipStream_t)stream;
    const bool prof = e->prof_depth > 0;
    hipEvent_t* pev = prof ? e->events.data() + (size_t)(e->prof_calls % e->prof_depth) * (e->ops.size() + 1) : nullptr;
    std::vector<char> needed(e->ops.size(), 1);
    if (d_features || d_age_probs || d_gender) {
        std::vector<char> live(e->d_bufs.size(), 0);
        for (int sl = 0; sl < HSEFR_N_OUTPUT_SLOTS; ++sl)
            if (outs[sl]) live[e->hdr.out_buffer[sl]] = 1;
        for (size_t i = e->ops.size(); i-- > 0;) {
            const hsefr_plan_op& o = e->ops[i];
            needed[i] = live[o.out_buf];
            if (!needed[i]) continue;
            live[o.out_buf] = 0;
            if (o.in_buf >= 0) live[o.in_buf] = 1;
            if (o.res_buf >= 0) live[o.res_buf] = 1;
        }
    }
    const int mask = (d_features ? 1 : 0) | (d_age_probs ? 2 : 0) | (d_gender ? 4 : 0);
    if (!prof && !input_u8 && mask != 0 && n <= e->graph_max_n && e->ops.size() > 0 && e->ops[0].in_buf == HSEFR_BUF_INPUT) {
        const size_t in_bytes = (size_t)e->hdr.in_h * e->hdr.in_w * e->hdr.in_c * sizeof(float);
        if (!e->d_in_stage) {
            HSEFR_HIP_CHECK(hipMalloc(&e->d_in_stage, in_bytes * e->graph_max_n));
            e->device_bytes += in_bytes * e->graph_max_n;
            HSEFR_HIP_CHECK(hipStreamCreateWithFlags(&e->cap_stream, hipStreamNonBlocking));
        }
        hipGraphExec_t exec = nullptr;
        for (const auto& g : e->graphs)
            if (g.n == n && g.mask == mask) exec = g.exec;
        if (!exec) {
            hipGraph_t graph = nullptr;
            HSEFR_HIP_CHECK(hipStreamBeginCapture(e->cap_stream, hipStreamCaptureModeThreadLocal));
            const int rc = run_ops(e, e->d_bufs, e->d_in_stage, n, needed, e->cap_stream, nullptr);
            const hipError_t ce = hipStreamEndCapture(e->cap_stream, &graph);
            if (rc != HSEFR_OK) { if (graph) (void)hipGraphDestroy(graph); return rc; }
            HSEFR_HIP_CHECK(ce);
            HSEFR_HIP_CHECK(hipGraphInstantiate(&exec, graph, nullptr, nullptr, 0));
            (void)hipGraphDestroy(graph);
            e->graphs.push_back({n, mask, exec});
        }
        HSEFR_HIP_CHECK(hipMemcpyAsync(e->d_in_stage, d_input, in_bytes * n, hipMemcpyDeviceToDevice, s));
        HSEFR_HIP_CHECK(hipGraphLaunch(exec, s));
        e->graph_launches++;
        for (int sl = 0; sl < HSEFR_N_OUTPUT_SLOTS; ++sl) {
            if (!outs[sl]) continue;
            const size_t bytes = (size_t)e->hdr.out_elems[sl] * sizeof(float) * n;
            HSEFR_HIP_CHECK(hipMemcpyAsync(outs[sl], e->d_bufs[e->hdr.out_buffer[sl]], bytes, hipMemcpyDeviceToDevice, s));
        }
    } else {
        std::vector<void*> tab(e->d_bufs);
        const void* src_of[HSEFR_N_OUTPUT_SLOTS] = {nullptr, nullptr, nullptr};
        for (int sl = 0; sl < HSEFR_N_OUTPUT_SLOTS; ++sl) {
            if (!outs[sl]) continue;
            const int b = e->hdr.out_buffer[sl];
            if (tab[b] != e->d_bufs[b]) { src_of[sl] = tab[b]; continue; }
            if (((uintptr_t)outs[sl] & 15) == 0) tab[b] = outs[sl];
            else src_of[sl] = e->d_bufs[b];
        }
        for (int sl = 0; sl < HSEFR_N_OUTPUT_SLOTS; ++sl)
            if (outs[sl] && src_of[sl] == e->d_bufs[e->hdr.out_buffer[sl]]) src_of[sl] = tab[e->hdr.out_buffer[sl]];
        const int rc = run_ops(e, tab, d_input, n, needed, s, prof ? pev : nullptr, input_u8);
        if (rc != HSEFR_OK) return rc;
        for (int sl = 0; sl < HSEFR_N_OUTPUT_SLOTS; ++sl)
            if (outs[sl] && src_of[sl])
                HSEFR_HIP_CHECK(hipMemcpyAsync(outs[sl], src_of[sl], (size_t)e->hdr.out_elems[sl] * sizeof(float) * n,
                                               hipMemcpyDeviceToDevice, s));
    }
    if (prof) e->prof_calls++;
    return HSEFR_OK;
}

int hsefr_plan_describe(const void* plan, size_t plan_bytes, int n, char* out, size_t out_bytes) {
    HSEFR_REQUIRE(out && out_bytes > 0 && n > 0, HSEFR_ERR_INVALID, "plan_describe: bad argument");
    out[0] = 0;
    hsefr_engine e;
    const char* blob = nullptr;
    int rc = check_plan_blob(plan, plan_bytes, e.hdr, e.bufs, e.ops, blob);
    if (rc != HSEFR_OK) return rc;
    e.max_batch = n;
    e.d_blob = reinterpret_cast<char*>(uintptr_t(1) << 40);
    e.d_overflow = reinterpret_cast<int*>(uintptr_t(1) << 39);
    e.d_bufs.resize(e.hdr.n_buffers);
    for (uint32_t i = 0; i < e.hdr.n_buffers; ++i) e.d_bufs[i] = reinterpret_cast<void*>((uintptr_t(2) << 40) + (uintptr_t(i) << 32));
    std::string text;
    std::vector<char> only(e.ops.size(), 0);
    for (size_t i = 0; i < e.ops.size(); ++i) {
        std::fill(only.begin(), only.end(), 0);
        only[i] = 1;
        const size_t span = (e.ops[i].flags & HSEFR_OPF_PAIR_NEXT) ? 1 : (e.ops[i].flags & HSEFR_OPF_HEADS) ? 3 : 0;
        for (size_t k = 1; k <= span && i + k < e.ops.size(); ++k) only[i + k] = 1;
        std::string line = std::to_string(i) + "\t" + std::to_string(e.ops[i].kind) + "\t";
        g_route_sink = &line;
        rc = run_ops(&e, e.d_bufs, reinterpret_cast<const void*>(uintptr_t(3) << 40), n, only, nullptr, nullptr,
                     false);
        g_route_sink = nullptr;
        if (rc != HSEFR_OK) { e.d_blob = nullptr; e.d_overflow = nullptr; e.d_bufs.clear(); return rc; }
        text += line + "\n";
        for (size_t k = 1; k <= span && i + k < e.ops.size(); ++k)
            text += std::to_string(i + k) + "\t" + std::to_string(e.ops[i + k].kind) + "\t(inside op " + std::to_string(i) + ")\n";
        i += span;
    }
    e.d_blob = nullptr; e.d_overflow = nullptr; e.d_bufs.clear();
    HSEFR_REQUIRE(text.size() + 1 <= out_bytes, HSEFR_ERR_INVALID, "plan_describe: the table needs %zu bytes, the buffer holds %zu", text.size() + 1, out_bytes);
    memcpy(out, text.c_str(), text.size() + 1);
    return HSEFR_OK;
}

int hsefr_engine_input_overflow(hsefr_engine* e, int* host_flag, hsefr_stream_t stream) {
    HSEFR_REQUIRE(e && host_flag, HSEFR_ERR_INVALID, "input_overflow: null argument");
    HSEFR_HIP_CHECK(hipMemcpyAsync(host_flag, e->d_overflow, sizeof(int), hipMemcpyDeviceToHost, (hipStream_t)stream));
    HSEFR_HIP_CHECK(hipMemsetAsync(e->d_overflow, 0, sizeof(int), (hipStream_t)stream));
    HSEFR_HIP_CHECK(hipStreamSynchronize((hipStream_t)stream));
    return HSEFR_OK;
}

int hsefr_engine_input_overflow_async(hsefr_engine* e, int* pinned_host_flag, hsefr_stream_t stream) {
    HSEFR_REQUIRE(e && pinned_host_flag, HSEFR_ERR_INVALID, "input_overflow_async: null argument");
    HSEFR_HIP_CHECK(hipMemcpyAsync(pinned_host_flag, e->d_overflow, sizeof(int), hipMemcpyDeviceToHost, (hipStream_t)stream));
    HSEFR_HIP_CHECK(hipMemsetAsync(e->d_overflow, 0, sizeof(int), (hipStream_t)stream));
    return HSEFR_OK;
}

int hsefr_engine_set_graph_batch(hsefr_engine* e, int max_n) {
    HSEFR_REQUIRE(e && max_n >= 0 && max_n <= e->max_batch, HSEFR_ERR_INVALID, "set_graph_batch: bad argument");
    for (auto& g : e->graphs) (void)hipGraphExecDestroy(g.exec);
    e->graphs.clear();
    if (e->d_in_stage) {
        (void)hipFree(e->d_in_stage);
        e->d_in_stage = nullptr;
        e->device_bytes -= (size_t)e->hdr.in_h * e->hdr.in_w * e->hdr.in_c * sizeof(float) * e->graph_max_n;
        (void)hipStreamDestroy(e->cap_stream);
        e->cap_stream = nullptr;
    }
    e->graph_max_n = max_n;
    return HSEFR_OK;
}

long long hsefr_engine_graph_launches(const hsefr_engine* e) { return e ? e->graph_launches : 0; }

int hsefr_engine_destroy(hsefr_engine* e) {
    if (!e) return HSEFR_OK;
    for (void* b : e->d_bufs)
        if (b) (void)hipFree(b);
    if (e->d_blob) (void)hipFree(e->d_blob);
    if (e->d_overflow) (void)hipFree(e->d_overflow);
    for (void* b : e->d_derived)
        if (b) (void)hipFree(b);
    for (auto ev : e->events) (void)hipEventDestroy(ev);
    for (auto& g : e->graphs) (void)hipGraphExecDestroy(g.exec);
    if (e->cap_stream) (void)hipStreamDestroy(e->cap_stream);
    if (e->d_in_stage) (void)hipFree(e->d_in_stage);
    delete e;
    return HSEFR_OK;
}

int hsefr_conv_c3_bias_act(const float* x, const float* wgt, const float* shift, float* y, int n, int h, int w,
                           int kh, int kw, int stride, int pad_t, int pad_l, int oh, int ow, int cout, int act,
                           hsefr_stream_t stream) {
    HSEFR_REQUIRE(n == 0 || (x && wgt && shift && y), HSEFR_ERR_INVALID, "conv_c3: null pointer");
    return launch_conv_c3(x, wgt, shift, y, n, h, w, kh, kw, stride, pad_t, pad_l, oh, ow, cout, act, (hipStream_t)stream);
}

int hsefr_dwconv3x3_bn_relu6(const float* x, const float* wgt, const float* scale, const float* shift, float* y,
                             int n, int h, int w, int c, int stride, int pad_t, int pad_l, int oh, int ow, int act,
                             hsefr_stream_t stream) {
    HSEFR_REQUIRE(n == 0 || (x && wgt && scale && shift && y), HSEFR_ERR_INVALID, "dwconv3x3: null pointer");
    return launch_dwconv3x3(x, wgt, scale, shift, y, n, h, w, c, stride, pad_t, pad_l, oh, ow, act, (hipStream_t)stream);
}

int hsefr_dwconv3x3_bn_relu6_split(const float* x, const float* wgt, const float* scale, const float* shift, void* y_split,
                                   int n, int h, int w, int c, int stride, int pad_t, int pad_l, int oh, int ow, int act,
                                   int a_log2, hsefr_stream_t stream) {
    HSEFR_REQUIRE(n == 0 || (x && wgt && scale && shift && y_split), HSEFR_ERR_INVALID, "dwconv3x3_split: null pointer");
    return launch_dwconv3x3_split(x, wgt, scale, shift, y_split, n, h, w, c, stride, pad_t, pad_l, oh, ow, act, a_log2, (hipStream_t)stream);
}

int hsefr_pwconv1x1_presplit_gap(const void* x_split, const void* w_split, const float* descale, const float* shift, float* y,
                                 long long m, int k, int cout, int act, int map_hw, hsefr_stream_t stream) {
    HSEFR_REQUIRE(m == 0 || (x_split && w_split && descale && shift && y), HSEFR_ERR_INVALID, "pwconv1x1_presplit_gap: null pointer");
    return launch_pwconv_ps_gap(x_split, w_split, descale, shift, y, m, k, cout, act, map_hw, (hipStream_t)stream);
}

int hsefr_pwconv1x1_presplit_dw(const void* x_split, const void* w_split, const float* descale, const float* shift, const float* dw_consts,
                                void* y_split, long long m, int k, int cout, int act, int map_w, int map_hw, int dw_stride, int out_log2,
                                hsefr_stream_t stream) {
    HSEFR_REQUIRE(m == 0 || (x_split && w_split && descale && shift && dw_consts && y_split), HSEFR_ERR_INVALID, "pwconv1x1_presplit_dw: null pointer");
    return launch_pwconv_ps_dw(x_split, w_split, descale, shift, dw_consts, y_split, m, k, cout, act, map_w, map_hw, dw_stride, out_log2,
                               (hipStream_t)stream);
}

int hsefr_pwconv1x1_presplit(const void* x_split, const void* w_split, const float* descale, const float* shift, float* y,
                             long long m, int k, int cout, int act, hsefr_stream_t stream) {
    HSEFR_REQUIRE(m == 0 || (x_split && w_split && descale && shift && y), HSEFR_ERR_INVALID, "pwconv_presplit: null pointer");
    return launch_pwconv_ps(x_split, w_split, descale, shift, y, m, k, cout, act, (hipStream_t)stream);
}

int hsefr_pwconv1x1_bias_relu6(const float* x, const float* wgt_t, const float* shift, float* y, long long m, int k,
                               int cout, int act, hsefr_stream_t stream) {
    HSEFR_REQUIRE(m == 0 || (x && wgt_t && shift && y), HSEFR_ERR_INVALID, "pwconv: null pointer");
    return launch_pwconv_f32(x, wgt_t, shift, y, m, k, cout, act, (hipStream_t)stream);
}

int hsefr_pwconv1x1_f16split(const float* x, const void* w_split, const float* descale, const float* shift, float* y,
                             long long m, int k, int cout, int a_log2, int act, hsefr_stream_t stream) {
    HSEFR_REQUIRE(m == 0 || (x && w_split && descale && shift && y), HSEFR_ERR_INVALID, "pwconv_f16split: null pointer");
    return launch_pwconv_f16s(x, w_split, descale, shift, y, m, k, cout, a_log2, act, (hipStream_t)stream);
}

int hsefr_stem2_fused(const float* x, const float* conv_w, const float* conv_shift, const float* wd1, const float* d1scale,
                      const float* d1shift, const void* w_split, const float* descale, const float* pshift, const float* wd2,
                      const float* d2scale, const float* d2shift, float* y, int n, int h, int w, int cpad_t, int cpad_l,
                      int h1, int w1, int pad_t2, int pad_l2, int oh2, int ow2, int a_log2, int act, hsefr_stream_t stream) {
    HSEFR_REQUIRE(n == 0 || (x && conv_w && conv_shift && wd1 && d1scale && d1shift && w_split && descale && pshift && wd2 &&
                             d2scale && d2shift && y), HSEFR_ERR_INVALID, "stem2_fused: null pointer");
    return launch_stem2_fused(x, conv_w, conv_shift, wd1, d1scale, d1shift, w_split, descale, pshift, wd2, d2scale, d2shift, y, n,
                              h, w, cpad_t, cpad_l, h1, w1, pad_t2, pad_l2, oh2, ow2, a_log2, act, (hipStream_t)stream);
}

int hsefr_stem3_fused(const float* x, const void* cw_split, const float* cdescale, const float* conv_shift, const float* wd1,
                      const float* d1scale, const float* d1shift, const void* w_split, const float* descale, const float* pshift,
                      const float* wd2, const float* d2scale, const float* d2shift, float* y, int* d_overflow, int n, int h, int w,
                      int cpad_t, int cpad_l, int h1, int w1, int pad_t2, int pad_l2, int oh2, int ow2, int in_log2, int a_log2,
                      int act, hsefr_stream_t stream) {
    HSEFR_REQUIRE(n == 0 || (x && cw_split && cdescale && conv_shift && wd1 && d1scale && d1shift && w_split && descale && pshift && wd2 &&
                             d2scale && d2shift && y), HSEFR_ERR_INVALID, "stem3_fused: null pointer");
    return launch_stem3_fused(x, cw_split, cdescale, conv_shift, wd1, d1scale, d1shift, w_split, descale, pshift, wd2, d2scale, d2shift, y,
                              d_overflow, n, h, w, cpad_t, cpad_l, h1, w1, pad_t2, pad_l2, oh2, ow2, in_log2, a_log2, act, (hipStream_t)stream);
}

int hsefr_stem4_fused(const void* x, int x_is_u8, const void* cw4, const float* cdescale, const float* conv_shift, const float* wd1,
                      const float* d1scale, const float* d1shift, const void* w_split, const float* descale, const float* pshift,
                      const float* wd2, const float* d2scale, const float* d2shift, float* y, int* d_overflow, int n, int h, int w,
                      int in_log2, int a_log2, int act, hsefr_stream_t stream) {
    HSEFR_REQUIRE(n == 0 || (x && cw4 && cdescale && conv_shift && wd1 && d1scale && d1shift && w_split && descale && pshift && wd2 &&
                             d2scale && d2shift && y), HSEFR_ERR_INVALID, "stem4_fused: null pointer");
    return launch_stem4_fused(x, x_is_u8, cw4, cdescale, conv_shift, wd1, d1scale, d1shift, w_split, descale, pshift, wd2, d2scale, d2shift, y,
                              d_overflow, n, h, w, in_log2, a_log2, act, (hipStream_t)stream);
}

int hsefr_stem5_stream(const void* x, int x_is_u8, const void* cw4, const float* cdescale, const float* conv_shift, const float* wd1,
                       const float* d1scale, const float* d1shift, const void* w_split, const float* descale, const float* pshift,
                       const float* wd2, const float* d2scale, const float* d2shift, float* y, int* d_overflow, int n, int h, int w,
// ... 296 lines not shown
```

### hse_facerec_tf_amd/csrc/fuzz_plan.cc

```cpp
#include <stdint.h>
#include <stdio.h>
#include <stdlib.h>
#include <string.h>

#include <string>
#include <vector>

#include "../../include/hsefr.h"

static uint64_t rng_state = 0x9E3779B97F4A7C15ull;
static uint64_t rnd() {
    rng_state ^= rng_state << 13;
    rng_state ^= rng_state >> 7;
    rng_state ^= rng_state << 17;
    return rng_state;
}

static long long n_ok = 0, n_err = 0, n_silent = 0;

static void run_one(const void* blob, size_t bytes, const char* what) {
    int rc = hsefr_plan_validate(blob, bytes);
    if (rc == HSEFR_OK) {
        ++n_ok;
        static char table[1 << 18];
        const int rd = hsefr_plan_describe(blob, bytes, 4, table, sizeof(table));
        if (rd != HSEFR_OK && !hsefr_last_error_string()[0]) { ++n_silent; fprintf(stderr, "no message for status %d (%s, plan_describe)\n", rd, what); }
        hsefr_engine* e = nullptr;
        rc = hsefr_engine_create(blob, bytes, 4, &e);
        if (rc == HSEFR_OK) hsefr_engine_destroy(e);
        else if (!hsefr_last_error_string()[0]) { ++n_silent; fprintf(stderr, "no message for status %d (%s, engine_create)\n", rc, what); }
        return;
    }
    ++n_err;
    if (rc > 0 || rc < HSEFR_ERR_SHAPE || !hsefr_last_error_string()[0]) {
        ++n_silent;
        fprintf(stderr, "status %d without a message / outside hsefr_status (%s)\n", rc, what);
    }
    hsefr_engine* e = nullptr;
    const int rc2 = hsefr_engine_create(blob, bytes, 4, &e);
    if (rc2 == HSEFR_OK) { fprintf(stderr, "engine_create accepted what plan_validate refused (%s)\n", what); abort(); }
}

int main(int argc, char** argv) {
    if (argc < 3) { fprintf(stderr, "usage: fuzz_plan <mutants per seed> <plan file>...\n"); return 2; }
    const long long per_seed = atoll(argv[1]);
    static const int32_t edge32[] = {0, 1, -1, -2, -3, 2, 3, 7, 63, 64, 65, 127, 128, 255, 256, 511, 512, 4095, 4096, 65535, 65536, 0x7fffffff,
                                     (int32_t)0x80000000, (int32_t)0xffff0000, 1 << 20, 1 << 24, 1 << 30};
    static const uint64_t edge64[] = {0ull, 1ull, 15ull, 16ull, 17ull, 0xffffffffull, 0x100000000ull, 0x7fffffffffffffffull, 0x8000000000000000ull,
                                      0xffffffffffffffffull, 0xfffffffffffffff0ull};
    for (int f = 2; f < argc; ++f) {
        FILE* fp = fopen(argv[f], "rb");
        if (!fp) { perror(argv[f]); return 2; }
        fseek(fp, 0, SEEK_END);
        const size_t bytes = (size_t)ftell(fp);
        fseek(fp, 0, SEEK_SET);
        std::vector<unsigned char> seed(bytes);
        if (fread(seed.data(), 1, bytes, fp) != bytes) { fprintf(stderr, "short read\n"); return 2; }
        fclose(fp);
        if (bytes < sizeof(hsefr_plan_header)) { fprintf(stderr, "%s: not a plan\n", argv[f]); return 2; }
        hsefr_plan_header h;
        memcpy(&h, seed.data(), sizeof(h));
        const size_t tables = sizeof(h) + (size_t)h.n_buffers * sizeof(hsefr_plan_buffer) + (size_t)h.n_ops * sizeof(hsefr_plan_op);
        if (hsefr_plan_validate(seed.data(), bytes) != HSEFR_OK) {
            fprintf(stderr, "%s: the seed itself is refused: %s\n", argv[f], hsefr_last_error_string());
            return 1;
        }
        unsigned char* w = (unsigned char*)malloc(bytes);
        memcpy(w, seed.data(), bytes);
        char what[160];
        for (long long it = 0; it < per_seed; ++it) {
            const unsigned mode = (unsigned)(rnd() % 10);
            if (mode == 0) {
                size_t cut = (rnd() & 1) ? (size_t)(rnd() % (tables + 64 < bytes ? tables + 64 : bytes)) : (size_t)(rnd() % bytes);
                unsigned char* t = (unsigned char*)malloc(cut ? cut : 1);
                memcpy(t, seed.data(), cut);
                snprintf(what, sizeof(what), "%s truncated to %zu", argv[f], cut);
                run_one(t, cut, what);
                free(t);
                continue;
            }
            const int nmut = 1 + (int)(rnd() % 3);
            size_t where[3];
            unsigned char saved[3][8];
            size_t len[3];
            for (int m = 0; m < nmut; ++m) {
                size_t off;
                if (mode == 1) {
                    off = (size_t)(rnd() % tables);
                    len[m] = 1;
                    memcpy(saved[m], w + off, 1);
                    w[off] ^= (unsigned char)(1u << (rnd() % 8));
                } else if (mode == 2 && bytes > tables) {
                    off = tables + (size_t)(rnd() % (bytes - tables));
                    len[m] = 1;
                    memcpy(saved[m], w + off, 1);
                    w[off] = (unsigned char)rnd();
                } else if (mode <= 6) {
                    off = (size_t)(rnd() % (tables / 4)) * 4;
                    len[m] = 4;
                    memcpy(saved[m], w + off, 4);
                    const int32_t v = edge32[rnd() % (sizeof(edge32) / sizeof(edge32[0]))];
                    memcpy(w + off, &v, 4);
                } else if (mode <= 8) {
                    off = (size_t)(rnd() % (tables / 8)) * 8;
                    len[m] = 8;
                    memcpy(saved[m], w + off, 8);
                    uint64_t v = edge64[rnd() % (sizeof(edge64) / sizeof(edge64[0]))];
                    if (rnd() & 1) v = h.blob_bytes - 64 + (rnd() % 128);
                    if (rnd() % 4 == 0) v &= ~15ull;
                    memcpy(w + off, &v, 8);
                } else {
                    off = (size_t)(rnd() % (tables / 4)) * 4;
                    len[m] = 4;
                    memcpy(saved[m], w + off, 4);
                    const uint32_t v = (uint32_t)rnd();
                    memcpy(w + off, &v, 4);
                }
                where[m] = off;
            }
            snprintf(what, sizeof(what), "%s mode %u at %zu", argv[f], mode, where[0]);
            run_one(w, bytes, what);
            for (int m = nmut - 1; m >= 0; --m) memcpy(w + where[m], saved[m], len[m]);
        }
        if (memcmp(w, seed.data(), bytes) != 0) { fprintf(stderr, "internal: working copy not restored\n"); return 1; }
        free(w);
    }
    printf("fuzz_plan: %lld mutants still valid, %lld refused, %lld without a message\n", n_ok, n_err, n_silent);
    return n_silent ? 1 : 0;
}
```

### hse_facerec_tf_amd/lowering.py

```python
from __future__ import annotations

import struct
from dataclasses import dataclass, field
from typing import Dict, List, Optional, Sequence, Tuple

import numpy as np

from .graphdef import Graph, GraphNode

ACT_NONE, ACT_RELU, ACT_RELU6, ACT_SIGMOID = 0, 1, 2, 3
OP_CONV_C3, OP_DWCONV3X3, OP_PWCONV_F32, OP_GAP, OP_DENSE, OP_SOFTMAX = 1, 2, 3, 4, 5, 6
OP_CONV_BF16, OP_MAXPOOL_BF16, OP_GAP_BF16, OP_STEM7X7_BF16, OP_DWPW_F32 = 7, 8, 9, 10, 11
OP_PWCONV_F16S = 12
OP_DWPW_F16S = 13
OP_STEM_F16S = 14
OP_STEM2_F16S = 15
OP_STEM3_F16S = 17
OP_CONV_F32, OP_MAXPOOL_F32 = 18, 19
OP_STEM7X7_POOL_BF16 = 20
OP_PWDW_PS = 21
OP_PWGAP_PS = 22
OP_PWCONV_PS = 16
_BF16_OUT = (OP_CONV_BF16, OP_MAXPOOL_BF16, OP_STEM7X7_BF16, OP_STEM7X7_POOL_BF16)
OUT_FEATURES, OUT_AGE, OUT_GENDER = 0, 1, 2
BUF_INPUT, BUF_NONE = -1, -2
PLAN_MAGIC = 0x314C505246455348
NO_OFFSET = 0xFFFFFFFFFFFFFFFF

_HEADER = struct.Struct("<QIIIIII3i3IQ")
_BUFFER = struct.Struct("<QII")
_OP = struct.Struct("<II3i3i3i3i2iii5Q")
OPF_PAIR_NEXT, OPF_HEADS, OPF_OUT_SUB2 = 1, 2, 4
AUX_C2_SHIFT, AUX_C2_BITS, AUX_STRIDE2_SHIFT, AUX_STRIDE2_BITS = 0, 12, 12, 2
AUX_H2_SHIFT, AUX_H2_BITS, AUX_W2_SHIFT, AUX_W2_BITS = 14, 9, 23, 9
AUX_LOG2_BITS, AUX_OUT_LOG2_SHIFT, AUX_IN_LOG2_SHIFT, AUX_IN_LOG2_BIAS, AUX_U8_BIT = 8, 8, 8, 64, 16
AUX_POOL_PAD_L_SHIFT = 4
STEM_KW_PAD_T2_BIT, STEM_KW_PAD_L2_BIT = 4, 5
STEM_PACK_CONV, STEM_PACK_CONV_SHIFT, STEM_PACK_DW1, STEM_PACK_DW1_SCALE, STEM_PACK_DW1_SHIFT = 0, 864, 896, 1184, 1216
STEM_PACK_DW2, STEM_PACK_DW2_SCALE, STEM_PACK_DW2_SHIFT, STEM_PACK_STEM2_END = 1248, 1824, 1888, 1952
STEM_PACK_CONV_SPLIT, STEM_PACK_CONV_DESCALE, STEM_PACK_CONV4, STEM_PACK_CONV4_U8 = 1952, 2976, 3008, 5056
STEM_PACK_U8_SHIFT, STEM_PACK_U8_DESCALE, STEM_PACK_STEM3_END = 7104, 7232, 7264
STEM_SHIFT2_DESCALE, STEM_SHIFT2_SHIFT = 0, 64


PRODUCT_KERNEL_FAMILIES = frozenset({
    "stem5_stream_kernel", "stem4_fused_kernel", "stem3_fused_kernel", "stem2_fused_kernel", "conv3x3_c3_kernel", "conv3x3_c3_mfma_kernel",
    "dwconv3x3_kernel", "pwconv_f32_dma_kernel", "pwconv_f32_kernel", "pwconv_f16s_kernel", "pwconv_ps_kernel", "dwpw_fused_kernel",
    "dwpw_f16s_kernel", "dwpw2_f16s_kernel", "dwpw3_f16s_kernel", "gap_kernel", "dense_kernel", "softmax_kernel", "heads_kernel",
    "stem7s_stream_kernel", "stem7x7_pool_bf16_kernel", "stem7x7_bf16_kernel", "maxpool3x3s2_bf16_kernel", "conv_bf16_kernel", "conv1x1_bf16_kernel",
    "conv1x1_w4_bf16_kernel", "conv1x1_pair_bf16_kernel", "conv3x3_w2_bf16_kernel", "conv_dma_bf16_kernel", "gap_bf16_kernel",
    "conv_f32_mfma_kernel", "conv2d_f32_kernel", "maxpool_f32_kernel"})


class LoweringError(NotImplementedError):
    """The graph uses a construct the engine has no kernel for (analogue of TF's
    'No OpKernel was registered' error)."""


def dequantize_min_first_u8(q: np.ndarray, range_min, range_max) -> np.ndarray:
    lo = np.float32(range_min)
    hi = np.float32(range_max)
    if lo == hi:
        return np.full(q.shape, lo, dtype=np.float32)
    step = np.float32(np.float64(hi - lo) / 255.0)
    lo_snapped = np.float32(np.round(lo / step) * step)
    return q.astype(np.float32) * step + lo_snapped


def tf_same_padding(size: int, k: int, stride: int) -> Tuple[int, int]:
    out = (size + stride - 1) // stride
    total = max((out - 1) * stride + k - size, 0)
    return out, total // 2


F16S_ACT_LOG2_RELU6 = 12


def split_pointwise_weights(w_t: np.ndarray, a_log2: int = F16S_ACT_LOG2_RELU6) -> Tuple[np.ndarray, np.ndarray]:
    w = np.ascontiguousarray(w_t, dtype=np.float32)
    cout, k = w.shape
    if k % 32:
        raise LoweringError("split_pointwise_weights: k=%d must be a multiple of 32" % k)
    amax = np.abs(w).max(axis=1).astype(np.float64)
    e = np.zeros(cout, np.int64)
    nz = amax > 0
    e[nz] = 14 - np.frexp(amax[nz])[1]
    e = np.clip(e, -100, 100)
    ws = np.ldexp(w.astype(np.float64), e[:, None]).astype(np.float32)
    hi = ws.astype(np.float16)
    lo = (ws - hi.astype(np.float32)).astype(np.float16)
    assert np.isfinite(hi.astype(np.float32)).all()
    img = np.empty((cout, k // 32, 64), np.uint16)
    img[:, :, :32] = hi.view(np.uint16).reshape(cout, k // 32, 32)
    img[:, :, 32:] = lo.view(np.uint16).reshape(cout, k // 32, 32)
    descale = np.ldexp(np.ones(cout, np.float64), -(e + a_log2)).astype(np.float32)
    return img, descale


def stem4_conv_image(w_hwio: np.ndarray, in_log2: int, reverse_channels: bool = False) -> Tuple[np.ndarray, np.ndarray]:
    w = np.asarray(w_hwio, dtype=np.float32).reshape(3, 3, 3, 32)
    if reverse_channels:
        w = w[:, :, ::-1, :]
    w = w.reshape(3, 9, 32)
    full = np.zeros((32, 64), np.float32)
    for dy in range(3):
        full[:, 8 * dy:8 * dy + 8] = w[dy, :8, :].T
        full[:, 32 + 8 * dy] = w[dy, 8, :]
    img, ds = split_pointwise_weights(full, in_log2)
    return np.ascontiguousarray(img.transpose(1, 0, 2)), ds


def stem4_u8_shifts(w_hwio: np.ndarray, shift: np.ndarray, mean_bgr) -> np.ndarray:
    w = np.asarray(w_hwio, dtype=np.float64).reshape(3, 3, 3, 32)
    m = np.asarray(mean_bgr, dtype=np.float64).reshape(1, 1, 3, 1)
    out = np.zeros((4, 32), np.float64)
    for case in range(4):
        rows = 2 if case & 2 else 3
        cols = 2 if case & 1 else 3
        out[case] = np.asarray(shift, np.float64) - (w[:rows, :cols] * m).sum(axis=(0, 1, 2))
    return out.astype(np.float32)


def unsplit_pointwise_weights(img: np.ndarray, descale: np.ndarray, a_log2: int) -> np.ndarray:
    cout, kt, _ = img.shape
    hi = img[:, :, :32].copy().view(np.float16).astype(np.float64).reshape(cout, kt * 32)
    lo = img[:, :, 32:].copy().view(np.float16).astype(np.float64).reshape(cout, kt * 32)
    return (hi + lo) * (descale.astype(np.float64) * 2.0 ** a_log2)[:, None]


@dataclass
class Layer:
    kind: int
    name: str
    src: int
    in_shape: Tuple[int, int, int]
    out_shape: Tuple[int, int, int]
    w: Optional[np.ndarray] = None
    scale: Optional[np.ndarray] = None
    shift: Optional[np.ndarray] = None
    act: int = ACT_NONE
    kh: int = 1
    kw: int = 1
    stride: int = 1
    pad_t: int = 0
    pad_l: int = 0
    tensors: List[str] = field(default_factory=list)
    sealed: bool = False
    version: int = 0
    res: int = -1
    w2: Optional[np.ndarray] = None
    shift2: Optional[np.ndarray] = None
    a_log2: int = 0
    w0: Optional[np.ndarray] = None
    shift0: Optional[np.ndarray] = None
    w3: Optional[np.ndarray] = None
    scale3: Optional[np.ndarray] = None
    shift3: Optional[np.ndarray] = None
    pad3: Tuple[int, int] = (0, 0)
    in_log2: int = 0
    u8_mean_bgr: Optional[Tuple[float, float, float]] = None
    proj: Optional[Tuple[int, int, int, int]] = None
    res_geom: Optional[Tuple[int, int, int]] = None
    graph_hw: Optional[Tuple[int, int]] = None
    out_split: int = 0
    in_split: bool = False
    flags: int = 0
    out_buf: int = BUF_NONE

    @property
    def out_bytes(self) -> int:
        return int(np.prod(self.out_shape)) * (2 if self.kind in _BF16_OUT else 4)


def geometry_word(c2: int, stride2: int, h2: int, w2: int) -> int:
    assert 0 <= c2 < 1 << AUX_C2_BITS and 1 <= stride2 < 1 << AUX_STRIDE2_BITS and 0 < h2 < 1 << AUX_H2_BITS and 0 < w2 < 1 << AUX_W2_BITS
    aux = c2 << AUX_C2_SHIFT | stride2 << AUX_STRIDE2_SHIFT | h2 << AUX_H2_SHIFT | w2 << AUX_W2_SHIFT
    return aux - (1 << 32) if aux >= 1 << 31 else aux


def stem_pack(L: Layer) -> np.ndarray:
    segs = [(STEM_PACK_CONV, L.w0), (STEM_PACK_CONV_SHIFT, L.shift0), (STEM_PACK_DW1, L.w), (STEM_PACK_DW1_SCALE, L.scale),
            (STEM_PACK_DW1_SHIFT, L.shift)]
    end = STEM_PACK_DW2
    if L.kind != OP_STEM_F16S:
        segs += [(STEM_PACK_DW2, L.w3), (STEM_PACK_DW2_SCALE, L.scale3), (STEM_PACK_DW2_SHIFT, L.shift3)]
        end = STEM_PACK_STEM2_END
    if L.kind == OP_STEM3_F16S:
        cw_t = np.zeros((32, 32), np.float32)
        cw_t[:, :27] = L.w0.reshape(27, 32).T
        cimg, cds = split_pointwise_weights(cw_t, L.in_log2)
        img4, ds4 = stem4_conv_image(L.w0, L.in_log2)
        assert np.array_equal(ds4, cds)
        if L.u8_mean_bgr is not None:
            img8, ds8 = stem4_conv_image(L.w0, 0, reverse_channels=True)
            sh8 = stem4_u8_shifts(L.w0, L.shift0, L.u8_mean_bgr)
        else:
            img8, ds8, sh8 = np.zeros_like(img4), np.zeros(32, np.float32), np.zeros((4, 32), np.float32)

        def rows(img):
            return np.ascontiguousarray(img).reshape(-1).view(np.float32)

# ... 423 lines not shown
            h, wd, c = self.shape_of(src)
            s = node.attr_ints("strides")
            if s[1] != s[2] or s[0] != 1 or s[3] != 1:
                raise LoweringError("%s: strides %r" % (node.name, s))
            if any(d != 1 for d in node.attr_ints("dilations") or [1]):
                raise LoweringError("%s: dilated convolution" % node.name)
            kh, kw = int(w.shape[0]), int(w.shape[1])
            pad = node.attr_s("padding")
            if pad == "SAME":
                oh, pt = tf_same_padding(h, kh, s[1])
                ow, pl = tf_same_padding(wd, kw, s[1])
            elif pad == "VALID":
                oh, ow, pt, pl = (h - kh) // s[1] + 1, (wd - kw) // s[1] + 1, 0, 0
            else:
                raise LoweringError("%s: padding %r" % (node.name, pad))
            if op == "DepthwiseConv2dNative":
                if w.shape[3] != 1 or (kh, kw) != (3, 3) or w.shape[2] != c or c % 4:
                    raise LoweringError("%s: depthwise kernel %r over %d channels" % (node.name, w.shape, c))
                L = Layer(OP_DWCONV3X3, node.name, src, (h, wd, c), (oh, ow, c), w=w, kh=3, kw=3, stride=s[1],
                          pad_t=pt, pad_l=pl)
            else:
                cout = int(w.shape[3])
                if w.shape[2] != c:
                    raise LoweringError("%s: kernel %r does not match %d input channels" % (node.name, w.shape, c))
                if (kh, kw) == (1, 1) and s[1] == 1 and c % 32 == 0 and cout % 64 == 0:
                    kind = OP_PWCONV_F32
                elif c == 3 and (kh, kw) == (3, 3) and cout % 4 == 0:
                    kind = OP_CONV_C3
                else:
                    raise LoweringError("%s: no fp32 kernel for Conv2D k=%r stride %d" % (node.name, w.shape, s[1]))
                L = Layer(kind, node.name, src, (h, wd, c), (oh, ow, cout), w=w, kh=kh, kw=kw, stride=s[1],
                          pad_t=pt, pad_l=pl)
            return self.new_layer(L, node)
        if op == "MatMul":
            if node.attr_b("transpose_a") or node.attr_b("transpose_b"):
                raise LoweringError("%s: transposed MatMul" % node.name)
            src = self.finished(self.lower_node(acts[0][0]))
            w = consts[0].astype(np.float32)
            h, wd, c = self.shape_of(src)
            if h * wd * c != w.shape[0]:
                raise LoweringError("%s: MatMul %r on a tensor of %d features" % (node.name, w.shape, h * wd * c))
            L = Layer(OP_DENSE, node.name, src, (1, 1, int(w.shape[0])), (1, 1, int(w.shape[1])), w=w)
            return self.new_layer(L, node)
        if op == "Mean":
            axes = sorted(int(a) for a in consts[0].reshape(-1))
            if axes != [1, 2]:
                raise LoweringError("%s: Mean over axes %r" % (node.name, axes))
            src = self.finished(self.lower_node(acts[0][0]))
            h, wd, c = self.shape_of(src)
            L = Layer(OP_GAP_BF16 if self.bf16 else OP_GAP, node.name, src, (h, wd, c), (1, 1, c), sealed=True)
            return self.new_layer(L, node)
        if op == "Softmax":
            src = self.finished(self.lower_node(acts[0][0]))
            shp = self.shape_of(src)
            L = Layer(OP_SOFTMAX, node.name, src, shp, shp, sealed=True)
            return self.new_layer(L, node)
        if op in ("Reshape", "Squeeze"):
            r = self.lower_node(acts[0][0])
            if self.shape_of(r)[0] * self.shape_of(r)[1] != 1:
                raise LoweringError("%s: reshape of a spatial tensor" % node.name)
            self.where[node.name] = r
            return r

        if len(acts) != 1:
            raise LoweringError("%s: op %s with %d non-constant inputs" % (node.name, op, len(acts)))
        idx = self.lower_node(acts[0][0])
        if idx < 0:
            raise LoweringError("%s: elementwise op directly on the graph input" % node.name)
        L = self.layers[idx]
        nconsumers = self.live_consumers(acts[0][0].name)
        if nconsumers != 1:
            raise LoweringError("%s: cannot fuse, input %s has %d consumers" % (node.name, acts[0][0].name, nconsumers))
        cout = L.out_shape[2]

        def vec(v):
            v = np.asarray(v, dtype=np.float32).reshape(-1)
            if v.size == 1:
                v = np.full(cout, v[0], np.float32)
            if v.size != cout:
                raise LoweringError("%s: operand of %d elements against %d channels" % (node.name, v.size, cout))
            return v

        if L.res >= 0 and op not in ("Relu", "Relu6", "Minimum", "Maximum"):
            raise LoweringError("%s: affine op after a fused residual sum" % node.name)
        if op in ("Mul",) and not L.sealed and L.act == ACT_NONE and L.kind in (OP_CONV_C3, OP_DWCONV3X3, OP_PWCONV_F32, OP_DENSE, OP_CONV_BF16, OP_STEM7X7_BF16, OP_CONV_F32):
            v = vec(consts[0])
            L.scale = v if L.scale is None else L.scale * v
            if L.shift is not None:
                L.shift = L.shift * v
        elif op in ("Add", "AddV2", "BiasAdd") and not L.sealed and L.act == ACT_NONE and L.kind in (OP_CONV_C3, OP_DWCONV3X3, OP_PWCONV_F32, OP_DENSE, OP_CONV_BF16, OP_STEM7X7_BF16, OP_CONV_F32):
            v = vec(consts[0])
            L.shift = v if L.shift is None else L.shift + v
        elif op == "Sub" and not L.sealed and L.act == ACT_NONE and ins[0][0] is acts[0][0]:
            v = vec(consts[0])
            L.shift = -v if L.shift is None else L.shift - v
        elif op in ("FusedBatchNorm", "FusedBatchNormV3") and not L.sealed and L.act == ACT_NONE:
            if node.attr_b("is_training", True):
                raise LoweringError("%s: training-mode FusedBatchNorm in a frozen graph" % node.name)
            gamma, beta, mean, var = [vec(c) for c in consts[:4]]
            k = gamma / np.sqrt(var + np.float32(node.attr_f("epsilon", 1e-3)))
            L.scale = k if L.scale is None else L.scale * k
            L.shift = (beta - mean * k) if L.shift is None else (L.shift * k + beta - mean * k)
        elif op == "Relu" and not L.sealed and L.act == ACT_NONE:
            L.act = ACT_RELU
        elif op == "Relu6" and not L.sealed and L.act == ACT_NONE:
            L.act = ACT_RELU6
        elif op == "Minimum" and not L.sealed and L.act == ACT_RELU and float(np.asarray(consts[0]).reshape(-1)[0]) == 6.0:
            L.act = ACT_RELU6
        elif op == "Maximum" and L.act in (ACT_RELU, ACT_RELU6) and float(np.asarray(consts[0]).reshape(-1)[0]) == 0.0:
            pass
        elif op == "Sigmoid" and not L.sealed and L.act == ACT_NONE and L.kind == OP_DENSE:
            L.act = ACT_SIGMOID
        else:
            raise LoweringError("%s: cannot fuse op %s into layer %s (act=%d sealed=%s)" %
                                (node.name, op, L.name, L.act, L.sealed))
        L.version += 1
        self.where[node.name] = idx
        return idx

    def is_final(self, name: str) -> bool:
        li = self.where[name]
        return li >= 0 and self.ver.get(name, 0) == self.layers[li].version


def assign_buffers(layers: List[Layer], pinned) -> List[int]:
    last_use = list(range(len(layers)))
    for i, L in enumerate(layers):
        for s in (L.src, L.res):
            if s >= 0:
                last_use[s] = i
    for i, L in enumerate(layers):
        span = 1 if L.flags & OPF_PAIR_NEXT else 3 if L.flags & OPF_HEADS else 0
        for j in range(i, min(i + span, len(layers) - 1) + 1 if span else i):
            for s in (layers[j].src, layers[j].res, j):
                if s >= 0:
                    last_use[s] = max(last_use[s], i + span)
    buffers: List[int] = []
    free: List[int] = []
    for i, L in enumerate(layers):
        need = L.out_bytes
        pick = None
        if i not in pinned and free:
            fits = [b for b in free if buffers[b] >= need]
            pick = min(fits, key=lambda b: buffers[b]) if fits else max(free, key=lambda b: buffers[b])
            free.remove(pick)
            buffers[pick] = max(buffers[pick], need)
        if pick is None:
            buffers.append(need)
            pick = len(buffers) - 1
        L.out_buf = pick
        for j in range(i + 1):
            if last_use[j] == i and j not in pinned and layers[j].out_buf not in free:
                free.append(layers[j].out_buf)
    return buffers


def consumers_of(layers: List[Layer]) -> Dict[int, List[Tuple[int, str]]]:
    consumers: Dict[int, List[Tuple[int, str]]] = {}
    for i, L in enumerate(layers):
        for how in ("src", "res"):
            s = getattr(L, how)
            if s >= 0:
                consumers.setdefault(s, []).append((i, how))
    return consumers


def sole_reader(consumers: Dict[int, List[Tuple[int, str]]], i: int, keep: Sequence[int]) -> int:
    cons = consumers.get(i, [])
    return cons[0][0] if i not in keep and len(cons) == 1 and cons[0][1] == "src" else -1


def rebuild(layers: List[Layer], drop, put: Dict[int, Layer]) -> Tuple[List[Layer], Dict[int, int]]:
    new_layers: List[Layer] = []
    remap: Dict[int, int] = {}
    for i, L in enumerate(layers):
        if i in drop:
            remap[i] = -1
        else:
            remap[i] = len(new_layers)
            new_layers.append(put.get(i, L))
    for L in new_layers:
        for how in ("src", "res"):
            s = getattr(L, how)
            if s >= 0:
                if remap[s] < 0:
                    raise LoweringError("%s still reads %s (as %s), which a fusion pass removed" % (L.name, layers[s].name, how))
                setattr(L, how, remap[s])
    return new_layers, remap


def dwpw_fusable(dw: Layer, pw: Layer) -> bool:
    return (dw.kind == OP_DWCONV3X3 and pw.kind == OP_PWCONV_F32 and dw.act == ACT_RELU6 and pw.act == ACT_RELU6 and
            dw.in_shape[2] in (32, 64) and pw.out_shape[2] in (64, 128) and dw.stride in (1, 2))


def fuse_dwpw(layers: List[Layer], keep: Sequence[int]) -> Tuple[List[Layer], Dict[int, int]]:
    consumers = consumers_of(layers)
    put: Dict[int, Layer] = {}
    drop = set()
    for i, dw in enumerate(layers):
        j = sole_reader(consumers, i, keep)
        if dw.kind == OP_DWCONV3X3 and j >= 0 and dwpw_fusable(dw, layers[j]):
            pw = layers[j]
            put[j] = Layer(OP_DWPW_F32, pw.name, dw.src, dw.in_shape, pw.out_shape, w=dw.w, scale=dw.scale, shift=dw.shift,
                           act=pw.act, kh=3, kw=3, stride=dw.stride, pad_t=dw.pad_t, pad_l=dw.pad_l, sealed=True,
                           w2=pw.w, shift2=pw.shift)
            drop.add(i)
    return rebuild(layers, drop, put)


def fuse_stem_pool(layers: List[Layer], keep: Sequence[int]) -> Tuple[List[Layer], Dict[int, int]]:
    consumers = consumers_of(layers)
    for i, L in enumerate(layers):
        p = sole_reader(consumers, i, keep)
        if not (L.kind == OP_STEM7X7_BF16 and L.act == ACT_RELU and p >= 0):
            continue
        P = layers[p]
        oh, ow = L.out_shape[0], L.out_shape[1]
        if not (P.kind == OP_MAXPOOL_BF16 and P.pad_t in (0, 1) and P.pad_l in (0, 1) and
                2 * (P.out_shape[0] - 1) - P.pad_t < oh and 2 * (P.out_shape[1] - 1) - P.pad_l < ow):
            continue
        S = Layer(OP_STEM7X7_POOL_BF16, P.name, -1, L.in_shape, P.out_shape, w=L.w, scale=L.scale, shift=L.shift, act=ACT_RELU,
                  kh=7, kw=7, stride=2, pad_t=3, pad_l=3, sealed=True, pad3=(P.pad_t, P.pad_l), tensors=list(P.tensors))
        return rebuild(layers, {i}, {p: S})
    return rebuild(layers, set(), {})


def fuse_proj(layers: List[Layer], keep: Sequence[int]) -> Tuple[List[Layer], Dict[int, int]]:
    consumers = consumers_of(layers)
    drop = set()
    for i, P in enumerate(layers):
        cons = consumers.get(i, [])
        if not (P.kind == OP_CONV_BF16 and P.kh == 1 and P.kw == 1 and P.pad_t == 0 and P.pad_l == 0 and P.act == ACT_NONE and P.res < 0 and
                P.proj is None and P.src >= 0 and i not in keep and len(cons) == 1 and cons[0][1] == "res" and 1 <= P.stride <= 3):
            continue
        I = layers[cons[0][0]]
        h2, w2, c2 = P.in_shape
        oh, ow, cout = I.out_shape
        if not (I.kind == OP_CONV_BF16 and I.kh == 1 and I.kw == 1 and I.stride == 1 and I.pad_t == 0 and I.pad_l == 0 and I.proj is None and
                I.src != i and tuple(P.out_shape) == tuple(I.out_shape) and c2 % 64 == 0 and I.in_shape[2] % 64 == 0 and cout % 64 == 0 and
                c2 < 4096 and h2 < 512 and w2 < 512 and (oh - 1) * P.stride < h2 and (ow - 1) * P.stride < w2):
            continue
        I.res, I.proj, I.w2 = P.src, (c2, P.stride, h2, w2), P.w
        I.shift2 = np.concatenate([P.scale.astype(np.float32).reshape(-1), P.shift.astype(np.float32).reshape(-1)])
        I.tensors = list(I.tensors)
        drop.add(i)
    return rebuild(layers, drop, {})


def subsample_stage_tails(layers: List[Layer], keep: Sequence[int]) -> int:
    consumers = consumers_of(layers)
    done = 0
    for t, I in enumerate(layers):
        cons = consumers.get(t, [])
        conv = I.kind
        if conv == OP_CONV_F32 and I.out_shape[2] % 64 != 0:
            continue
        if not cons or t in keep or not (I.kind in (OP_CONV_BF16, OP_CONV_F32) and I.kh == 1 and I.kw == 1 and I.stride == 1 and I.pad_t == 0 and I.pad_l == 0 and
                                         I.res >= 0 and I.proj is None and I.res_geom is None and I.src >= 0 and I.flags == 0):
            continue
        h, w, c = I.out_shape
        strides = set()
        for j, how in cons:
            C = layers[j]
            if how == "src" and C.kind == conv and C.kh == 1 and C.kw == 1 and C.pad_t == 0 and C.pad_l == 0 and C.stride > 1 and C.proj is None:
                strides.add(C.stride)
            elif how == "res" and C.kind == conv and C.proj is not None and C.proj[1] > 1 and C.proj[2:] == (h, w):
                strides.add(C.proj[1])
            else:
                strides.add(0)
        if len(strides) != 1 or 0 in strides:
            continue
        s = strides.pop()
        X = layers[I.src]
        if not (X.kind == conv and X.kh == 3 and X.kw == 3 and X.stride == 1 and X.pad_t == 1 and X.pad_l == 1 and X.res < 0 and X.proj is None and
                I.src not in keep and [q for q, _ in consumers.get(I.src, [])] == [t] and X.flags == 0 and tuple(X.out_shape[:2]) == (h, w) and
                tuple(layers[I.res].out_shape) == (h, w, c) and h < 512 and w < 512):
            continue
        oh, ow = (h - 1) // s + 1, (w - 1) // s + 1
        if oh * ow <= 1 or ow <= 1:
            continue
        X.stride, X.out_shape, X.graph_hw = s, (oh, ow, X.out_shape[2]), (h, w)
        I.in_shape, I.out_shape, I.res_geom, I.graph_hw = X.out_shape, (oh, ow, c), (s, h, w), (h, w)
        for j, how in cons:
            C = layers[j]
            if how == "src":
                C.stride, C.in_shape = 1, I.out_shape
                assert tuple(C.out_shape[:2]) == (oh, ow), (C.name, C.out_shape, oh, ow)
            else:
                C.proj = (C.proj[0], 1, oh, ow)
        done += 1
    return done


def pair_fusable(A: Layer, B: Layer, a_index: int) -> bool:
    def plain_1x1(L):
        return (L.kind == OP_CONV_BF16 and L.kh == 1 and L.kw == 1 and L.stride == 1 and L.pad_t == 0 and L.pad_l == 0 and
                tuple(L.in_shape[:2]) == tuple(L.out_shape[:2]) and L.flags == 0)
    if not (plain_1x1(A) and plain_1x1(B) and B.src == a_index and B.res < 0 and B.proj is None and A.res >= 0 and A.res_geom is None):
        return False
    if A.proj is not None and not (A.proj[0] == 64 and A.proj[1] == 1 and tuple(A.proj[2:]) == tuple(A.out_shape[:2])):
        return False
    return A.in_shape[2] == 64 and A.out_shape[2] == 256 and B.out_shape[2] == 64 and A.act in (ACT_NONE, ACT_RELU, ACT_RELU6) and \
        B.act in (ACT_NONE, ACT_RELU, ACT_RELU6)


def mark_pairs(layers: List[Layer]) -> int:
    n = 0
    for i in range(len(layers) - 1):
        if layers[i].flags == 0 and pair_fusable(layers[i], layers[i + 1], i):
            layers[i].flags |= OPF_PAIR_NEXT
            n += 1
    return n


def compact_pair_outputs(layers: List[Layer], keep: Sequence[int]) -> int:
    consumers = consumers_of(layers)
    done = 0
    for a, A in enumerate(layers):
        if not (A.flags & OPF_PAIR_NEXT) or A.flags & OPF_OUT_SUB2 or a in keep or a + 1 >= len(layers) or layers[a + 1].src != a:
            continue
        h, w, c = A.out_shape
        others = [layers[j] for j, _ in consumers.get(a, []) if j != a + 1]
        if not others or h < 2 or w < 2 or tuple(A.in_shape[:2]) != (h, w):
            continue
        if not all(L.res == a and L.src != a and L.proj is None and L.res_geom == (2, h, w) for L in others):
            continue
        A.flags |= OPF_OUT_SUB2
        A.graph_hw, A.out_shape = (h, w), ((h + 1) // 2, (w + 1) // 2, c)
        for L in others:
            assert tuple(L.out_shape) == tuple(A.out_shape), (L.name, L.out_shape, A.out_shape)
            L.res_geom = None
        done += 1
    return done


def mark_heads(layers: List[Layer]) -> int:
    n = 0
    for i in range(len(layers) - 3):
        F, A, S, G = layers[i:i + 4]
        if (F.kind == OP_DENSE and F.act == ACT_RELU and F.out_shape[2] == 256 and F.in_shape[2] % 256 == 0 and F.in_shape[2] <= 2048 and F.flags == 0 and
                A.kind == OP_DENSE and A.act == ACT_NONE and A.src == i and 1 <= A.out_shape[2] <= 128 and
                S.kind == OP_SOFTMAX and S.src == i + 1 and
                G.kind == OP_DENSE and G.act == ACT_SIGMOID and G.src == i and G.out_shape[2] == 1 and
                all(L.shift is not None and L.scale is None for L in (F, A, G))):
            F.flags |= OPF_HEADS
            n += 1
    return n


def fuse_stem(layers: List[Layer], keep: Sequence[int]) -> Tuple[List[Layer], Dict[int, int]]:
    consumers = consumers_of(layers)
    for i, L in enumerate(layers):
        b = sole_reader(consumers, i, keep)
        if not (L.kind == OP_CONV_C3 and b >= 0 and L.src == -1 and L.in_shape[2] == 3 and
                L.out_shape[2] == 32 and L.stride == 2 and L.kh == 3 and L.kw == 3 and L.act == ACT_RELU6):
            continue
        B = layers[b]
        if not (B.kind == OP_DWPW_F32 and B.stride == 1 and B.in_shape[2] == 32 and B.out_shape[2] == 64):
            continue
        S = Layer(OP_STEM_F16S, B.name, -1, L.in_shape, B.out_shape, w=B.w, scale=B.scale, shift=B.shift, act=B.act, kh=3, kw=3,
                  stride=2, pad_t=L.pad_t, pad_l=L.pad_l, sealed=True, w2=B.w2, shift2=B.shift2, a_log2=F16S_ACT_LOG2_RELU6,
                  w0=L.w, shift0=L.shift)
        return rebuild(layers, {i}, {b: S})
    return rebuild(layers, set(), {})


def fuse_stem2(layers: List[Layer], keep: Sequence[int]) -> Tuple[List[Layer], Dict[int, int]]:
    consumers = consumers_of(layers)
    for i0, L0 in enumerate(layers):
        if not (L0.kind == OP_CONV_C3 and L0.src == -1 and L0.in_shape[2] == 3 and L0.out_shape[2] == 32 and L0.stride == 2 and
                L0.kh == 3 and L0.kw == 3 and L0.act == ACT_RELU6):
            continue
        i1 = sole_reader(consumers, i0, keep)
        if i1 < 0 or not (layers[i1].kind == OP_DWCONV3X3 and layers[i1].stride == 1 and layers[i1].act == ACT_RELU6):
            continue
        i2 = sole_reader(consumers, i1, keep)
        if i2 < 0 or not (layers[i2].kind == OP_PWCONV_F32 and layers[i2].out_shape[2] == 64 and layers[i2].act == ACT_RELU6):
            continue
        i3 = sole_reader(consumers, i2, keep)
        if i3 < 0 or not (layers[i3].kind == OP_DWCONV3X3 and layers[i3].stride == 2 and layers[i3].in_shape[2] == 64 and
                          layers[i3].act in (ACT_NONE, ACT_RELU, ACT_RELU6)):
            continue
        L1, L2, L3 = layers[i1], layers[i2], layers[i3]
        S = Layer(OP_STEM2_F16S, L3.name, -1, L0.in_shape, L3.out_shape, w=L1.w, scale=L1.scale, shift=L1.shift, act=L3.act, kh=3, kw=3,
                  stride=2, pad_t=L0.pad_t, pad_l=L0.pad_l, sealed=True, w2=L2.w, shift2=L2.shift, a_log2=F16S_ACT_LOG2_RELU6,
                  w0=L0.w, shift0=L0.shift, w3=L3.w, scale3=L3.scale, shift3=L3.shift, pad3=(L3.pad_t, L3.pad_l))
        return rebuild(layers, {i0, i1, i2}, {i3: S})
    return rebuild(layers, set(), {})


BLOCK_F16S_AUTO = ((128, 128), (256, 256))


def block_f16s_fusable(dw: Layer, pw: Layer, which: str) -> bool:
    c, cout = dw.in_shape[2], pw.out_shape[2]
    if not (dw.kind == OP_DWCONV3X3 and pw.kind == OP_PWCONV_F32 and pw.a_log2 > 0 and dw.act == ACT_RELU6 and
            pw.act in (ACT_NONE, ACT_RELU, ACT_RELU6) and dw.stride in (1, 2) and c % 32 == 0 and cout % 64 == 0):
        return False
    return which == "all" or (dw.stride == 1 and (c, cout) in BLOCK_F16S_AUTO)


def fuse_block_f16s(layers: List[Layer], keep: Sequence[int], which: str) -> Tuple[List[Layer], Dict[int, int]]:
    consumers = consumers_of(layers)
    put: Dict[int, Layer] = {}
    drop = set()
    for i, dw in enumerate(layers):
        j = sole_reader(consumers, i, keep)
        if dw.kind == OP_DWCONV3X3 and j >= 0 and block_f16s_fusable(dw, layers[j], which):
            pw = layers[j]
            put[j] = Layer(OP_DWPW_F16S, pw.name, dw.src, dw.in_shape, pw.out_shape, w=dw.w, scale=dw.scale, shift=dw.shift,
                           act=pw.act, kh=3, kw=3, stride=dw.stride, pad_t=dw.pad_t, pad_l=dw.pad_l, sealed=True,
                           w2=pw.w, shift2=pw.shift, a_log2=pw.a_log2)
            drop.add(i)
    return rebuild(layers, drop, put)


def choose_pointwise_math(layers: List[Layer], pw_math: str) -> None:
    if pw_math not in ("auto", "f32", "f16split"):
        raise ValueError("pw_math must be 'auto', 'f32' or 'f16split', not %r" % (pw_math,))
    if pw_math == "f32":
        return
    for L in layers:
        if L.kind != OP_PWCONV_F32:
            continue
        bounded = L.src >= 0 and layers[L.src].act == ACT_RELU6 and layers[L.src].kind not in _BF16_OUT
        if bounded and L.in_shape[2] % 32 == 0 and L.out_shape[2] % 64 == 0:
            L.a_log2 = F16S_ACT_LOG2_RELU6
        elif pw_math == "f16split":
            raise LoweringError("%s: split-f16 pointwise needs a ReLU6-bounded input, k %% 32 == 0 and cout %% 64 == 0" % L.name)


PRESPLIT_MIN_K = 256


def presplit_activations(layers: List[Layer], keep: Sequence[int]) -> int:
    consumers = consumers_of(layers)
    n = 0
    for i, L in enumerate(layers):
        if not (L.kind == OP_PWCONV_F32 and L.a_log2 > 0 and L.src >= 0):
            continue
        P = layers[L.src]
        k, cout = L.in_shape[2], L.out_shape[2]
        if (P.kind == OP_DWCONV3X3 and P.act == ACT_RELU6 and L.src not in keep and consumers.get(L.src) == [(i, "src")] and
                k % 32 == 0 and k >= PRESPLIT_MIN_K and cout % 128 == 0 and 0 < L.a_log2 <= 12):
            P.out_split = L.a_log2
            L.in_split = True
            n += 1
    return n


def pwdw_fusable(pw: Layer, dw: Layer) -> bool:
    h, w, _ = dw.in_shape
    if not (pw.kind == OP_PWCONV_F32 and pw.a_log2 > 0 and pw.in_split and pw.out_shape[2] % 128 == 0 and
            dw.kind == OP_DWCONV3X3 and dw.act == ACT_RELU6 and 0 < dw.out_split <= 12 and h * w <= 288):
        return False
    if dw.stride == 1:
        return dw.pad_t == 1 and dw.pad_l == 1 and dw.out_shape == dw.in_shape
    return (dw.stride == 2 and (h, w) in ((12, 12), (14, 14)) and (dw.pad_t, dw.pad_l) == (0, 0) and dw.out_shape[:2] == (h // 2, w // 2) and
            pw.act == ACT_RELU6)


def fuse_pwgap(layers: List[Layer], keep: Sequence[int]) -> Tuple[List[Layer], Dict[int, int]]:
    consumers = consumers_of(layers)
    for i, L in enumerate(layers):
        j = sole_reader(consumers, i, keep)
        h, w, c = L.out_shape
        if not (L.kind == OP_PWCONV_F32 and L.a_log2 > 0 and L.in_split and c % 128 == 0 and j >= 0 and
                layers[j].kind == OP_GAP and 33 <= h * w <= 288):
            continue
        G = layers[j]
        F = Layer(OP_PWGAP_PS, G.name, L.src, L.in_shape, G.out_shape, w=L.w, shift=L.shift, act=L.act, sealed=True, a_log2=L.a_log2,
                  in_split=True, tensors=list(G.tensors))
        return rebuild(layers, {i}, {j: F})
    return rebuild(layers, set(), {})


def fuse_pwdw(layers: List[Layer], keep: Sequence[int]) -> Tuple[List[Layer], Dict[int, int]]:
    consumers = consumers_of(layers)
    put: Dict[int, Layer] = {}
    drop = set()
    for i, pw in enumerate(layers):
        j = sole_reader(consumers, i, keep)
        if j >= 0 and pwdw_fusable(pw, layers[j]):
            dw = layers[j]
            put[j] = Layer(OP_PWDW_PS, dw.name, pw.src, pw.in_shape, dw.out_shape, w=pw.w, shift=pw.shift, act=pw.act, sealed=True,
                           a_log2=pw.a_log2, in_split=True, w3=dw.w, scale3=dw.scale, shift3=dw.shift, out_split=dw.out_split, kh=3, kw=3,
                           stride=dw.stride, pad_t=dw.pad_t, pad_l=dw.pad_l, tensors=list(dw.tensors))
            drop.add(i)
    return rebuild(layers, drop, put)


def lower_graph(g: Graph, input_tensor: str, outputs: Dict[int, str], input_hw: Optional[Tuple[int, int]] = None,
                feeds: Optional[Dict[str, object]] = None, fuse: bool = True, dtype: str = "f32",
                pw_math: Optional[str] = None, fuse_stem_block: Optional[bool] = None, stem_fusion: Optional[str] = None,
                block_fusion: Optional[str] = None, presplit: Optional[str] = None, input_bound: Optional[float] = None,
                pwdw_fusion: Optional[str] = None, u8_mean_bgr: Optional[Sequence[float]] = None, launch_fusion: bool = True) -> Plan:
    if dtype not in ("f32", "bf16", "f32g"):
        raise ValueError("dtype must be 'f32', 'bf16' or 'f32g', not %r" % (dtype,))
    in_node, _ = g.get_tensor_by_name(input_tensor)
    shape = g.placeholder_shape(in_node.name)
    if input_hw is None:
        if shape is None or len(shape) != 4 or shape[1] <= 0 or shape[2] <= 0:
            raise ValueError("input tensor %s has no static HxW; pass input_hw" % input_tensor)
        input_hw = (int(shape[1]), int(shape[2]))
    feeds_n = {}
    for k, v in (feeds or {}).items():
        feeds_n[g.get_tensor_by_name(k)[0].name] = v
    low = _Lowerer(g, in_node.name, input_hw, feeds_n, dtype)
    if shape is not None and len(shape) == 4 and shape[3] > 0:
        low.in_c = int(shape[3])
    out_layers: Dict[int, Tuple[int, int]] = {}
    low.mark_live([g.get_tensor_by_name(t)[0] for t in outputs.values()])
    for slot, tname in outputs.items():
        node, _ = g.get_tensor_by_name(tname)
        li = low.lower_node(node)
        if li < 0:
            raise LoweringError("output %s is the graph input" % tname)
        out_layers[slot] = (li, int(np.prod(low.layers[li].out_shape)))
    layers = low.layers

    for L in layers:
        if L.kind in (OP_CONV_C3, OP_PWCONV_F32, OP_DENSE) and L.scale is not None:
            L.w = (L.w * L.scale.reshape((1,) * (L.w.ndim - 1) + (-1,))).astype(np.float32)
            L.scale = None
        if L.kind in (OP_CONV_C3, OP_PWCONV_F32, OP_DWCONV3X3, OP_DENSE) and L.shift is None:
            L.shift = np.zeros(L.out_shape[2], np.float32)
        if L.kind == OP_DWCONV3X3 and L.scale is None:
            L.scale = np.ones(L.out_shape[2], np.float32)
        if L.kind == OP_CONV_F32 and L.act not in (ACT_NONE, ACT_RELU, ACT_RELU6):
            raise LoweringError("%s: activation %d on a general convolution" % (L.name, L.act))
        if L.kind in (OP_CONV_BF16, OP_STEM7X7_BF16):
            cout = L.out_shape[2]
            L.scale = np.ones(cout, np.float32) if L.scale is None else L.scale.astype(np.float32)
            L.shift = np.zeros(cout, np.float32) if L.shift is None else L.shift.astype(np.float32)
            if L.act not in (ACT_NONE, ACT_RELU, ACT_RELU6):
                raise LoweringError("%s: activation %d on a bf16 convolution" % (L.name, L.act))
            from .resnet50 import pack_conv_weight, pack_stem_weight
            L.w = pack_stem_weight(L.w) if L.kind == OP_STEM7X7_BF16 else pack_conv_weight(L.w)

    for slot, tname in outputs.items():
        nm = g.get_tensor_by_name(tname)[0].name
        if not low.is_final(nm):
            raise LoweringError("output %s is an intermediate of fused layer %s; fetch the layer's final tensor"
                                % (tname, layers[low.where[nm]].name))
    tensor_layer = {name: li for name, li in low.where.items() if li >= 0 and low.is_final(name)}

    def keep() -> List[int]:
        return [li for li, _ in out_layers.values()]

    def apply(fuse_pass, *args) -> None:
        nonlocal layers, out_layers, tensor_layer
        layers, remap = fuse_pass(layers, keep(), *args)
        out_layers = {slot: (remap[li], e) for slot, (li, e) in out_layers.items()}
        tensor_layer = {name: remap[li] for name, li in tensor_layer.items() if remap[li] >= 0}

    pw_math = pw_math or "auto"
    if stem_fusion is None:
        stem_fusion = "none" if fuse_stem_block is False else "stem2"
    if stem_fusion not in ("none", "stem", "stem2"):
        raise ValueError("stem_fusion must be 'none', 'stem' or 'stem2', not %r" % (stem_fusion,))
    want_stem = fuse and dtype == "f32" and pw_math != "f32" and stem_fusion != "none"
    if want_stem and stem_fusion == "stem2":
        apply(fuse_stem2)
        if input_bound is not None:
            if not (input_bound > 0 and np.isfinite(input_bound)):
                raise ValueError("input_bound must be a positive finite number, not %r" % (input_bound,))
            in_log2 = int(np.floor(np.log2(32768.0 / float(input_bound))))
            in_log2 = max(-8, min(14, in_log2))
            if float(input_bound) * 2.0 ** in_log2 <= 32768.0:
                for L in layers:
                    if L.kind == OP_STEM2_F16S:
                        L.kind, L.in_log2 = OP_STEM3_F16S, in_log2
                        if u8_mean_bgr is not None:
                            if len(u8_mean_bgr) != 3 or not all(0.0 <= float(m) <= 255.0 for m in u8_mean_bgr):
                                raise ValueError("u8_mean_bgr must be three means in [0, 255], not %r" % (u8_mean_bgr,))
                            if float(input_bound) < 256.0:
                                raise ValueError("uint8 input needs input_bound >= 256 (pixels minus a mean), not %r" % (input_bound,))
                            L.u8_mean_bgr = tuple(float(m) for m in u8_mean_bgr)
    if fuse and dtype == "bf16":
        for fuse_pass in (fuse_stem_pool, fuse_proj):
            apply(fuse_pass)
        subsample_stage_tails(layers, keep())
    if fuse:
        apply(fuse_dwpw)

    if dtype == "f32":
        choose_pointwise_math(layers, pw_math)
        if want_stem:
            apply(fuse_stem)
        block_fusion = block_fusion or "auto"
        if block_fusion not in ("auto", "none", "all"):
            raise ValueError("block_fusion must be 'auto', 'none' or 'all', not %r" % (block_fusion,))
        if fuse and block_fusion != "none":
            apply(fuse_block_f16s, block_fusion)
        presplit = presplit or "auto"
        if presplit not in ("auto", "none"):
            raise ValueError("presplit must be 'auto' or 'none', not %r" % (presplit,))
        if presplit == "auto":
            presplit_activations(layers, keep())
            pwdw_fusion = pwdw_fusion or "auto"
            if pwdw_fusion not in ("auto", "none"):
                raise ValueError("pwdw_fusion must be 'auto' or 'none', not %r" % (pwdw_fusion,))
            if fuse and pwdw_fusion == "auto":
                apply(fuse_pwdw)
                apply(fuse_pwgap)
    if fuse and launch_fusion:
        if dtype == "bf16":
            mark_pairs(layers)
            compact_pair_outputs(layers, keep())
        if dtype == "f32":
            mark_heads(layers)
    buffers = assign_buffers(layers, set(keep()))
    return Plan(layers, (input_hw[0], input_hw[1], low.in_c), buffers, out_layers, tensor_layer)
```

### include/hsefr.h

```cpp
#ifndef HSEFR_H
#define HSEFR_H

#include <stddef.h>
#include <stdint.h>

#ifdef __cplusplus
extern "C" {
#endif

#define HSEFR_VERSION 141

typedef enum hsefr_status {
    HSEFR_OK = 0,
    HSEFR_ERR_INVALID = -1,
    HSEFR_ERR_UNSUPPORTED = -2,
    HSEFR_ERR_HIP = -3,
    HSEFR_ERR_NOMEM = -4,
    HSEFR_ERR_SHAPE = -5
} hsefr_status;

typedef enum hsefr_act {
    HSEFR_ACT_NONE = 0,
    HSEFR_ACT_RELU = 1,
    HSEFR_ACT_RELU6 = 2,
    HSEFR_ACT_SIGMOID = 3
} hsefr_act;

typedef void* hsefr_stream_t;

int hsefr_version(void);
const char* hsefr_last_error_string(void);

#define HSEFR_PLAN_MAGIC 0x314c505246455348ull
#define HSEFR_NO_OFFSET 0xffffffffffffffffull
#define HSEFR_BUF_INPUT (-1)
#define HSEFR_BUF_NONE (-2)

typedef enum hsefr_op_kind {
    HSEFR_OP_CONV_C3 = 1,
    HSEFR_OP_DWCONV3X3 = 2,
    HSEFR_OP_PWCONV_F32 = 3,
    HSEFR_OP_GAP = 4,
    HSEFR_OP_DENSE = 5,
    HSEFR_OP_SOFTMAX = 6,
    HSEFR_OP_CONV_BF16 = 7,
    HSEFR_OP_MAXPOOL_BF16 = 8,
    HSEFR_OP_GAP_BF16 = 9,
    HSEFR_OP_STEM7X7_BF16 = 10,
    HSEFR_OP_DWPW_F32 = 11,
    HSEFR_OP_PWCONV_F16S = 12,
    HSEFR_OP_DWPW_F16S = 13,
    HSEFR_OP_STEM_F16S = 14,
    HSEFR_OP_CONV_F32 = 18,
    HSEFR_OP_MAXPOOL_F32 = 19,
    HSEFR_OP_STEM7X7_POOL_BF16 = 20,
    HSEFR_OP_PWCONV_PS_DW = 21,
    HSEFR_OP_PWCONV_PS_GAP = 22,
    HSEFR_OP_STEM3_F16S = 17,
    HSEFR_OP_PWCONV_PS = 16,
    HSEFR_OP_STEM2_F16S = 15
} hsefr_op_kind;

typedef enum hsefr_output_slot {
    HSEFR_OUT_FEATURES = 0,
    HSEFR_OUT_AGE = 1,
    HSEFR_OUT_GENDER = 2,
    HSEFR_N_OUTPUT_SLOTS = 3
} hsefr_output_slot;

typedef struct hsefr_plan_header {
    uint64_t magic;
    uint32_t version;
    uint32_t n_buffers;
    uint32_t n_ops;
    uint32_t in_h, in_w, in_c;
    int32_t out_buffer[HSEFR_N_OUTPUT_SLOTS];
    uint32_t out_elems[HSEFR_N_OUTPUT_SLOTS];
    uint64_t blob_bytes;
} hsefr_plan_header;

typedef struct hsefr_plan_buffer {
    uint64_t elems_per_image;
    uint32_t elem_bytes;
    uint32_t reserved;
} hsefr_plan_buffer;

typedef enum hsefr_op_flags {
    HSEFR_OPF_PAIR_NEXT = 1,
    HSEFR_OPF_HEADS = 2,
    HSEFR_OPF_OUT_SUB2 = 4
} hsefr_op_flags;

enum {
    HSEFR_AUX_C2_SHIFT = 0, HSEFR_AUX_C2_BITS = 12,
    HSEFR_AUX_STRIDE2_SHIFT = 12, HSEFR_AUX_STRIDE2_BITS = 2,
    HSEFR_AUX_H2_SHIFT = 14, HSEFR_AUX_H2_BITS = 9,
    HSEFR_AUX_W2_SHIFT = 23, HSEFR_AUX_W2_BITS = 9,
    HSEFR_AUX_LOG2_BITS = 8,
    HSEFR_AUX_OUT_LOG2_SHIFT = 8,
    HSEFR_AUX_IN_LOG2_SHIFT = 8,
    HSEFR_AUX_IN_LOG2_BIAS = 64,
    HSEFR_AUX_U8_BIT = 16,
    HSEFR_AUX_POOL_PAD_L_SHIFT = 4
};

enum { HSEFR_STEM_KW_PAD_T2_BIT = 4, HSEFR_STEM_KW_PAD_L2_BIT = 5 };

enum {
    HSEFR_STEM_PACK_CONV = 0,
    HSEFR_STEM_PACK_CONV_SHIFT = 864,
    HSEFR_STEM_PACK_DW1 = 896,
    HSEFR_STEM_PACK_DW1_SCALE = 1184,
    HSEFR_STEM_PACK_DW1_SHIFT = 1216,
    HSEFR_STEM_PACK_DW2 = 1248,
    HSEFR_STEM_PACK_DW2_SCALE = 1824,
    HSEFR_STEM_PACK_DW2_SHIFT = 1888,
    HSEFR_STEM_PACK_STEM2_END = 1952,
    HSEFR_STEM_PACK_CONV_SPLIT = 1952,
    HSEFR_STEM_PACK_CONV_DESCALE = 2976,
    HSEFR_STEM_PACK_CONV4 = 3008,
    HSEFR_STEM_PACK_CONV4_U8 = 5056,
    HSEFR_STEM_PACK_U8_SHIFT = 7104,
    HSEFR_STEM_PACK_U8_DESCALE = 7232,
    HSEFR_STEM_PACK_STEM3_END = 7264
};

enum { HSEFR_STEM_SHIFT2_DESCALE = 0, HSEFR_STEM_SHIFT2_SHIFT = 64 };

typedef struct hsefr_plan_op {
    uint32_t kind;
    uint32_t act;
    int32_t in_buf, out_buf, res_buf;
    int32_t h, w, cin;
    int32_t oh, ow, cout;
    int32_t kh, kw, stride;
    int32_t pad_t, pad_l;
    int32_t aux;
    int32_t flags;
    uint64_t w_off;
    uint64_t scale_off;
    uint64_t shift_off;
    uint64_t w2_off;
    uint64_t shift2_off;
} hsefr_plan_op;

typedef struct hsefr_engine hsefr_engine;

int hsefr_engine_create(const void* plan, size_t plan_bytes, int max_batch, hsefr_engine** out);

int hsefr_plan_validate(const void* plan, size_t plan_bytes);

int hsefr_plan_describe(const void* plan, size_t plan_bytes, int n, char* out, size_t out_bytes);

int hsefr_engine_set_graph_batch(hsefr_engine* e, int max_n);
long long hsefr_engine_graph_launches(const hsefr_engine* e);

size_t hsefr_engine_workspace_bytes(const hsefr_engine* e);
int hsefr_engine_max_batch(const hsefr_engine* e);

int hsefr_engine_forward(hsefr_engine* e, const void* d_input, int n, void* d_features,
                         void* d_age_probs, void* d_gender, hsefr_stream_t stream);

int hsefr_engine_accepts_u8(const hsefr_engine* e);
int hsefr_engine_forward_u8(hsefr_engine* e, const void* d_input_u8, int n, void* d_features, void* d_age_probs, void* d_gender,
                            hsefr_stream_t stream);

void* hsefr_engine_buffer(hsefr_engine* e, int buffer);
int hsefr_engine_copy_buffer(hsefr_engine* e, int buffer, void* d_dst, size_t bytes, hsefr_stream_t stream);

int hsefr_engine_set_profiling(hsefr_engine* e, int depth);
long long hsefr_engine_profiled_calls(const hsefr_engine* e);
int hsefr_engine_op_times_ms(hsefr_engine* e, int slot, float* ms, int n_ops);

int hsefr_engine_input_overflow(hsefr_engine* e, int* host_flag, hsefr_stream_t stream);
int hsefr_engine_input_overflow_async(hsefr_engine* e, int* pinned_host_flag, hsefr_stream_t stream);
int hsefr_engine_destroy(hsefr_engine* e);


int hsefr_conv_c3_bias_act(const float* x, const float* wgt, const float* shift, float* y, int n, int h,
                           int w, int kh, int kw, int stride, int pad_t, int pad_l, int oh, int ow,
                           int cout, int act, hsefr_stream_t stream);

int hsefr_dwconv3x3_bn_relu6(const float* x, const float* wgt, const float* scale, const float* shift,
                             float* y, int n, int h, int w, int c, int stride, int pad_t, int pad_l,
                             int oh, int ow, int act, hsefr_stream_t stream);

int hsefr_dwconv3x3_bn_relu6_split(const float* x, const float* wgt, const float* scale, const float* shift, void* y_split,
                                   int n, int h, int w, int c, int stride, int pad_t, int pad_l, int oh, int ow, int act,
                                   int a_log2, hsefr_stream_t stream);

int hsefr_pwconv1x1_bias_relu6(const float* x, const float* wgt_t, const float* shift, float* y,
                               long long m, int k, int cout, int act, hsefr_stream_t stream);

int hsefr_pwconv1x1_f16split(const float* x, const void* w_split, const float* descale, const float* shift, float* y,
                             long long m, int k, int cout, int a_log2, int act, hsefr_stream_t stream);

int hsefr_pwconv1x1_presplit(const void* x_split, const void* w_split, const float* descale, const float* shift, float* y,
                             long long m, int k, int cout, int act, hsefr_stream_t stream);

int hsefr_pwconv1x1_presplit_gap(const void* x_split, const void* w_split, const float* descale, const float* shift, float* y,
                                 long long m, int k, int cout, int act, int map_hw, hsefr_stream_t stream);

int hsefr_pwconv1x1_presplit_dw(const void* x_split, const void* w_split, const float* descale, const float* shift, const float* dw_consts,
                                void* y_split, long long m, int k, int cout, int act, int map_w, int map_hw, int dw_stride, int out_log2,
                                hsefr_stream_t stream);

int hsefr_dwpw_f16split(const float* x, const float* wd, const float* dscale, const float* dshift, const void* w_split,
                        const float* descale, const float* pshift, float* y, int n, int h, int w, int c, int stride,
                        int pad_t, int pad_l, int oh, int ow, int cout, int a_log2, int act, hsefr_stream_t stream);

int hsefr_stem2_fused(const float* x, const float* conv_w, const float* conv_shift, const float* wd1, const float* d1scale,
                      const float* d1shift, const void* w_split, const float* descale, const float* pshift, const float* wd2,
                      const float* d2scale, const float* d2shift, float* y, int n, int h, int w, int cpad_t, int cpad_l,
                      int h1, int w1, int pad_t2, int pad_l2, int oh2, int ow2, int a_log2, int act, hsefr_stream_t stream);

int hsefr_stem3_fused(const float* x, const void* cw_split, const float* cdescale, const float* conv_shift, const float* wd1,
                      const float* d1scale, const float* d1shift, const void* w_split, const float* descale, const float* pshift,
                      const float* wd2, const float* d2scale, const float* d2shift, float* y, int* d_overflow, int n, int h, int w,
                      int cpad_t, int cpad_l, int h1, int w1, int pad_t2, int pad_l2, int oh2, int ow2, int in_log2, int a_log2,
                      int act, hsefr_stream_t stream);

int hsefr_stem4_fused(const void* x, int x_is_u8, const void* cw4, const float* cdescale, const float* conv_shift, const float* wd1,
                      const float* d1scale, const float* d1shift, const void* w_split, const float* descale, const float* pshift,
                      const float* wd2, const float* d2scale, const float* d2shift, float* y, int* d_overflow, int n, int h, int w,
                      int in_log2, int a_log2, int act, hsefr_stream_t stream);
int hsefr_stem5_stream(const void* x, int x_is_u8, const void* cw4, const float* cdescale, const float* conv_shift, const float* wd1,
                      const float* d1scale, const float* d1shift, const void* w_split, const float* descale, const float* pshift,
                      const float* wd2, const float* d2scale, const float* d2shift, float* y, int* d_overflow, int n, int h, int w,
                      int in_log2, int a_log2, int act, hsefr_stream_t stream);

int hsefr_dwpw_fused(const float* x, const float* wd, const float* dscale, const float* dshift, const float* wp_t,
                     const float* pshift, float* y, int n, int h, int w, int c, int stride, int pad_t, int pad_l, int oh,
                     int ow, int cout, hsefr_stream_t stream);

int hsefr_gap(const float* x, float* y, int n, int hw, int c, hsefr_stream_t stream);

int hsefr_dense(const float* x, const float* wgt, const float* bias, float* y, int n, int k, int cout,
                int act, hsefr_stream_t stream);

int hsefr_softmax(const float* x, float* y, int n, int c, hsefr_stream_t stream);

int hsefr_heads_fused(const float* x, const float* w1, const float* b1, const float* wa, const float* ba, const float* wg, const float* bg,
                      float* hidden, float* logits, float* age_probs, float* gender, int n, int k, int a, hsefr_stream_t stream);
// ... 108 lines not shown
```

Baseline: 241,200.

## Fuse stride-2 depthwise 128->pointwise 256 pair into a warp-specialized f16-split kernel

New measurement: 247,800, median of 6. +2.7%, better.

```diff
diff --git a/hse_facerec_tf_amd/csrc/common.h b/hse_facerec_tf_amd/csrc/common.h
--- a/hse_facerec_tf_amd/csrc/common.h
+++ b/hse_facerec_tf_amd/csrc/common.h
@@ -264,6 +264,8 @@
                      const float* descale, const float* pshift, float* y, int n, int h, int w, int c, int stride, int pad_t,
                      int pad_l, int oh, int ow, int cout, int a_log2, int act, hipStream_t s);
 bool dwpw_f16s_supported(int c, int cout, int stride);
+bool dwpw_s2_covered(int c, int cout, int stride);
+bool dwpw_s2_off();
 int launch_stem_fused(const float* x, const float* cw, const float* cshift, const float* wd, const float* dscale,
                       const float* dshift, const void* wsplit, const float* descale, const float* pshift, float* y, int n,
                       int h, int w, int cpad_t, int cpad_l, int oh, int ow, int a_log2, int act, hipStream_t s);
@@ -314,6 +316,7 @@
 void set_c11_bres(int v);
 void set_c11_adv(int v);
 int read_c11_stamps(void* host_out, size_t bytes);
+void set_dwpw_s2_off(int v);
 void set_dwpws_tw(int v);
 void set_dwpws_bn(int v);
 void set_pw_tile(int v);
diff --git a/hse_facerec_tf_amd/csrc/dwpw_f16s.hip b/hse_facerec_tf_amd/csrc/dwpw_f16s.hip
--- a/hse_facerec_tf_amd/csrc/dwpw_f16s.hip
+++ b/hse_facerec_tf_amd/csrc/dwpw_f16s.hip
@@ -1,3 +1,5 @@
+#include <type_traits>
+
 #include "common.h"
 
 namespace hsefr {
@@ -495,6 +497,254 @@
     }
 }
 
+constexpr unsigned S2_GRID = 256;
+constexpr int S2_C = 128, S2_COUT = 256, S2_KT = S2_C / 32, S2_T = 8, S2_M = S2_T * S2_T;
+constexpr int S2_B_ST = S2_COUT * ROWB;
+constexpr int S2_A_ST = S2_M * ROWB;
+constexpr int S2_SCR = 16 * ROWB;
+constexpr int S2_A_OFF = S2_KT * S2_B_ST, S2_S_OFF = S2_A_OFF + 2 * S2_A_ST, S2_W_OFF = S2_S_OFF + 4 * S2_SCR;
+constexpr int S2_E_OFF = S2_W_OFF + 11 * S2_C * 4, S2_LDS = S2_E_OFF + 2 * S2_COUT * 4;
+static_assert(S2_LDS <= 160 * 1024, "LDS budget");
+
+template <int ACT>
+__global__ __launch_bounds__(512, 1) void dwpws2_f16s_kernel(DwPwSParams p) {
+    __shared__ __attribute__((aligned(1024))) unsigned char smem[S2_LDS];
+    const int tid = threadIdx.x;
+    const int lane = tid & 63;
+    const int wave = __builtin_amdgcn_readfirstlane(tid >> 6);
+    const __amdgpu_buffer_rsrc_t rx = make_rsrc(p.x, (long long)p.nimg * p.H * p.W * S2_C * 4);
+    const __amdgpu_buffer_rsrc_t rw = make_rsrc(p.wsplit, (long long)S2_COUT * S2_C * 4);
+    const __amdgpu_buffer_rsrc_t ry = make_rsrc(p.y, (long long)p.nimg * p.OH * p.OW * S2_COUT * 4);
+    const unsigned OOB = 0xFFFFFFF0u;
+    {
+        const unsigned lds0 = (unsigned)(unsigned long long)(__attribute__((address_space(3))) unsigned char*)smem;
+#pragma unroll
+        for (int j = 0; j < 16; ++j) {
+            const int pc = wave * 16 + j;
+            const int r = (pc & 31) * 8 + (lane >> 3);
+            const unsigned v = ((unsigned)r * (unsigned)S2_C + 4u * ((lane & 7) ^ ((r >> 1) & 7) ^ ((r & 1) << 2))) * 4u;
+            asm volatile("s_mov_b32 m0, %0\n\ts_nop 0\n\tbuffer_load_dwordx4 %1, %2, %3 offen lds" ::"s"(__builtin_amdgcn_readfirstlane(lds0 + pc * 1024)),
+                         "v"(v), "s"(rw), "s"(__builtin_amdgcn_readfirstlane((unsigned)(pc >> 5) * 128u))
+                         : "memory", "m0");
+        }
+        float4* wl = (float4*)(smem + S2_W_OFF);
+        for (int i = tid; i < 11 * (S2_C / 4); i += 512)
+            wl[i] = i < 9 * (S2_C / 4) ? p.wd[i] : (i < 10 * (S2_C / 4) ? p.dscale[i - 9 * (S2_C / 4)] : p.dshift[i - 10 * (S2_C / 4)]);
+        float* el = (float*)(smem + S2_E_OFF);
+        for (int i = tid; i < S2_COUT; i += 512) { el[i] = p.descale[i]; el[S2_COUT + i] = p.pshift[i]; }
+        asm volatile("s_waitcnt vmcnt(0)" ::: "memory");
+    }
+    const unsigned nitem = (p.total - blockIdx.x + gridDim.x - 1) / gridDim.x;
+    const int nsteps = (int)(nitem * S2_KT);
+    struct Item { int n, oh0, ow0; };
+    auto decode = [&](unsigned i) {
+        const unsigned lt = xcd_remap_dir(blockIdx.x + (i < nitem ? i : nitem - 1) * gridDim.x, p.total, p.reverse);
+        Item it;
+        const unsigned pr = fastdiv(lt, p.m_w);
+        it.ow0 = (lt - pr * p.tiles_w) * S2_T;
+        it.n = fastdiv(pr, p.m_h);
+        it.oh0 = (pr - it.n * p.tiles_h) * S2_T;
+        return it;
+    };
+    typedef std::integral_constant<int, 0> S0;
+    typedef std::integral_constant<int, 1> S1;
+    __syncthreads();
+
+    if (wave < 4) {
+        const int quad = tid & 7, col = (tid >> 3) & 7, row0 = 2 * wave;
+        const f32x4* wl = (const f32x4*)(smem + S2_W_OFF) + quad;
+        f32x4 xr[2][5][3];
+        unsigned vo[5][3];
+        float mk[3], rk[5];
+        unsigned pf_i = 0, ci = 0;
+        int pf_kc = 0, ckc = 0;
+        auto setup_loads = [&](unsigned i) {
+            const Item it = decode(i);
+            const int iw0 = min(it.ow0 + col, p.OW - 1) * 2 - p.pad_l;
+            const int cc[3] = {max(iw0, 0), min(max(iw0 + 1, 0), p.W - 1), min(iw0 + 2, p.W - 1)};
+            const int ih0 = (it.oh0 + row0) * 2 - p.pad_t;
+#pragma unroll
+            for (int a = 0; a < 5; ++a) {
+                const unsigned rb = (unsigned)((it.n * p.H + min(max(ih0 + a, 0), p.H - 1)) * p.W);
+#pragma unroll
+                for (int b = 0; b < 3; ++b) vo[a][b] = ((rb + (unsigned)cc[b]) * (unsigned)S2_C + 4u * quad) * 4u;
+            }
+        };
+        auto setup_factors = [&](unsigned i) {
+            const Item it = decode(i);
+            const int iw0 = min(it.ow0 + col, p.OW - 1) * 2 - p.pad_l;
+            mk[0] = iw0 >= 0 ? 1.f : 0.f;
+            mk[1] = (iw0 + 1 >= 0 && iw0 + 1 < p.W) ? 1.f : 0.f;
+            mk[2] = iw0 + 2 < p.W ? 1.f : 0.f;
+            const int ih0 = (it.oh0 + row0) * 2 - p.pad_t;
+#pragma unroll
+            for (int a = 0; a < 5; ++a) rk[a] = (ih0 + a >= 0 && ih0 + a < p.H) ? 1.f : 0.f;
+        };
+        auto gload = [&](auto SET) {
+            constexpr int S = decltype(SET)::value;
+            const unsigned so = (unsigned)pf_kc * 128u;
+#pragma unroll
+            for (int a = 0; a < 5; ++a)
+#pragma unroll
+                for (int b = 0; b < 3; ++b) xr[S][a][b] = bload16(rx, vo[a][b], so);
+            if (++pf_kc == S2_KT) {
+                pf_kc = 0;
+                setup_loads(++pf_i);
+            }
+        };
+        auto produce = [&](auto SET, unsigned char* At) {
+            constexpr int S = decltype(SET)::value;
+            f32x4 wk[9];
+#pragma unroll
+            for (int i = 0; i < 9; ++i) wk[i] = wl[i * (S2_C / 4) + ckc * 8] * mk[i % 3];
+            const f32x4 dsc = wl[9 * (S2_C / 4) + ckc * 8], dsh = wl[10 * (S2_C / 4) + ckc * 8];
+            auto row_sum = [&](int a, int b) {
+                f32x4 t = xr[S][a][0] * wk[b];
+                t = __builtin_elementwise_fma(xr[S][a][1], wk[b + 1], t);
+                return __builtin_elementwise_fma(xr[S][a][2], wk[b + 2], t);
+            };
+#pragma unroll
+            for (int j = 0; j < 2; ++j) {
+                const f32x4 sa = row_sum(2 * j, 0), sb = row_sum(2 * j + 1, 3), sc = row_sum(2 * j + 2, 6);
+                const float fb = rk[2 * j + 1], fc = rk[2 * j + 2];
+                f32x4 sum = sa * rk[2 * j];
+                sum = __builtin_elementwise_fma(sb, f32x4{fb, fb, fb, fb}, sum);
+                sum = __builtin_elementwise_fma(sc, f32x4{fc, fc, fc, fc}, sum);
+                const f32x4 o = __builtin_elementwise_fma(sum, dsc, dsh);
+                f32x4 v;
+#pragma unroll
+                for (int e = 0; e < 4; ++e) v[e] = relu6(o[e]);
+                v = v * p.a_scale;
+                const f16x4 hi = __builtin_convertvector(v, f16x4);
+                const f16x4 lo = __builtin_convertvector(v - __builtin_convertvector(hi, f32x4), f16x4);
+                const int R = (row0 + j) * S2_T + col;
+                *(f16x4*)(At + swzb(R, quad >> 1) + 8 * (quad & 1)) = hi;
+                *(f16x4*)(At + swzb(R, 4 + (quad >> 1)) + 8 * (quad & 1)) = lo;
+            }
+            if (++ckc == S2_KT) {
+                ckc = 0;
+                setup_factors(++ci);
+            }
+        };
+        setup_loads(0);
+        setup_factors(0);
+        gload(S0());
+        for (int t = 0; t < nsteps; t += 2) {
+            gload(S1());
+            produce(S0(), smem + S2_A_OFF);
+            __syncthreads();
+            gload(S0());
+            produce(S1(), smem + S2_A_OFF + S2_A_ST);
+            __syncthreads();
+        }
+    } else {
+        const int cw = wave - 4;
+        const int li = lane & 31, lh = lane >> 5;
+        const int brow = cw * 64 + li;
+        const int erow = lane >> 3, ech = lane & 7;
+        f32x16 acc[2][2];
+        auto zero_acc = [&]() {
+#pragma unroll
+            for (int mi = 0; mi < 2; ++mi)
+#pragma unroll
+                for (int ni = 0; ni < 2; ++ni)
+#pragma unroll
+                    for (int r = 0; r < 16; ++r) acc[mi][ni][r] = 0.f;
+        };
+        auto epilogue = [&](const Item& cur) {
+            unsigned char* scr = smem + S2_S_OFF + cw * S2_SCR;
+            const float* el = (const float*)(smem + S2_E_OFF);
+            unsigned sv[2][2][2];
+#pragma unroll
+            for (int mi = 0; mi < 2; ++mi)
+#pragma unroll
+                for (int hb = 0; hb < 2; ++hb)
+#pragma unroll
+                    for (int i = 0; i < 2; ++i) {
+                        const int R = mi * 32 + hb * 16 + erow + 8 * i;
+                        const int oh = cur.oh0 + R / S2_T, ow = cur.ow0 + R % S2_T;
+                        sv[mi][hb][i] = (oh < p.OH && ow < p.OW)
+                                            ? ((unsigned)((cur.n * p.OH + oh) * p.OW + ow) * (unsigned)S2_COUT + (unsigned)(cw * 64 + 4 * ech)) * 4u
+                                            : OOB;
+                    }
+#pragma unroll
+            for (int ni = 0; ni < 2; ++ni) {
+                const int nl = cw * 64 + ni * 32 + 4 * ech;
+                const f32x4 ds = *(const f32x4*)(el + nl), sh = *(const f32x4*)(el + S2_COUT + nl);
+#pragma unroll
+                for (int mi = 0; mi < 2; ++mi)
+#pragma unroll
+                    for (int hb = 0; hb < 2; ++hb) {
+                        if ((li >> 4) == hb) {
+#pragma unroll
+                            for (int j = 0; j < 4; ++j) {
+                                f32x4 v;
+#pragma unroll
+                                for (int e = 0; e < 4; ++e) v[e] = acc[mi][ni][4 * j + e];
+                                *(f32x4*)(scr + (li & 15) * 128 + 16 * ((2 * j + lh) ^ (li & 7))) = v;
+                            }
+                        }
+                        f32x4 rv[2];
+#pragma unroll
+                        for (int i = 0; i < 2; ++i) {
+                            const int r = erow + 8 * i;
+                            rv[i] = *(const f32x4*)(scr + r * 128 + 16 * (ech ^ (r & 7)));
+                        }
+#pragma unroll
+                        for (int i = 0; i < 2; ++i) {
+                            const f32x4 z = __builtin_elementwise_fma(rv[i], ds, sh);
+                            f32x4 o;
+#pragma unroll
+                            for (int e = 0; e < 4; ++e) o[e] = apply_act<ACT>(z[e]);
+                            bstore16_welded(o, ry, sv[mi][hb][i], __builtin_amdgcn_readfirstlane((unsigned)(ni * 32) * 4u));
+                        }
+                    }
+            }
+        };
+        zero_acc();
+        Item cur = decode(0);
+        unsigned ci = 0;
+        int ckc = 0;
+        bool pending = false;
+        for (int g = 0; g < nsteps; ++g) {
+            if (pending) {
+                epilogue(cur);
+                zero_acc();
+                cur = decode(++ci);
+                pending = false;
+            }
+            __syncthreads();
+            const unsigned char* As = smem + S2_A_OFF + (g & 1) * S2_A_ST;
+            const unsigned char* Bs = smem + ckc * S2_B_ST;
+#pragma unroll
+            for (int s = 0; s < 2; ++s) {
+                f16x8 ah[2], al[2], bh[2], bl[2];
+#pragma unroll
+                for (int mi = 0; mi < 2; ++mi) {
+                    ah[mi] = *(const f16x8*)(As + swzb(li + mi * 32, 2 * s + lh));
+                    al[mi] = *(const f16x8*)(As + swzb(li + mi * 32, 4 + 2 * s + lh));
+                }
+#pragma unroll
+                for (int ni = 0; ni < 2; ++ni) {
+                    bh[ni] = *(const f16x8*)(Bs + swzb(brow + ni * 32, 2 * s + lh));
+                    bl[ni] = *(const f16x8*)(Bs + swzb(brow + ni * 32, 4 + 2 * s + lh));
+                }
+#pragma unroll
+                for (int mi = 0; mi < 2; ++mi)
+#pragma unroll
+                    for (int ni = 0; ni < 2; ++ni) {
+                        acc[mi][ni] = __builtin_amdgcn_mfma_f32_32x32x16_f16(bh[ni], al[mi], acc[mi][ni], 0, 0, 0);
+                        acc[mi][ni] = __builtin_amdgcn_mfma_f32_32x32x16_f16(bl[ni], ah[mi], acc[mi][ni], 0, 0, 0);
+                        acc[mi][ni] = __builtin_amdgcn_mfma_f32_32x32x16_f16(bh[ni], ah[mi], acc[mi][ni], 0, 0, 0);
+                    }
+            }
+            if (++ckc == S2_KT) { ckc = 0; pending = true; }
+        }
+        epilogue(cur);
+    }
+}
+
+HSEFR_KNOB(g_s2_off, 0);
 HSEFR_KNOB(g_tw, 0);
 HSEFR_KNOB(g_bn, 0);
 
@@ -550,12 +800,38 @@
     return launch_status("dwpw_f16split");
 }
 
+int launch_s2(DwPwSParams& p, int n, int act, hipStream_t s) {
+    p.tiles_w = (p.OW + S2_T - 1) / S2_T;
+    p.tiles_h = (p.OH + S2_T - 1) / S2_T;
+    p.tiles_n = 1;
+    const long long total = (long long)n * p.tiles_w * p.tiles_h;
+    HSEFR_REQUIRE(total < (1ll << 31) / 16, HSEFR_ERR_UNSUPPORTED, "dwpw_f16split: grid too large");
+    p.total = (unsigned)total;
+    auto magic = [](unsigned d) { return d == 1 ? 0u : (unsigned)((0x100000000ull + d - 1) / d); };
+    p.m_n = 0; p.m_w = magic(p.tiles_w); p.m_h = magic(p.tiles_h);
+    HSEFR_REQUIRE(total * (long long)(p.tiles_w > p.tiles_h ? p.tiles_w : p.tiles_h) < (1ll << 32), HSEFR_ERR_UNSUPPORTED,
+                  "dwpw_f16split: grid too large for the quotient multipliers");
+    const unsigned g = p.total < S2_GRID ? p.total : S2_GRID;
+#define HSEFR_DWPWS2(A) HSEFR_LAUNCH((dwpws2_f16s_kernel<A>), dim3(g), dim3(512), 0, s, p)
+    if (act == HSEFR_ACT_RELU6) HSEFR_DWPWS2(HSEFR_ACT_RELU6);
+    else if (act == HSEFR_ACT_RELU) HSEFR_DWPWS2(HSEFR_ACT_RELU);
+    else if (act == HSEFR_ACT_NONE) HSEFR_DWPWS2(HSEFR_ACT_NONE);
+    else { set_error("dwpw_f16split: act %d", act); return HSEFR_ERR_UNSUPPORTED; }
+#undef HSEFR_DWPWS2
+    return launch_status("dwpw_f16split");
+}
+
 }
 
 #ifdef HSEFR_DEV
+void set_dwpw_s2_off(int v) { g_s2_off = v; }
 void set_dwpws_tw(int v) { g_tw = v; }
 void set_dwpws_bn(int v) { g_bn = v; }
 #endif
+
+bool dwpw_s2_off() { return g_s2_off != 0; }
+
+bool dwpw_s2_covered(int c, int cout, int stride) { return stride == 2 && c == S2_C && cout == S2_COUT; }
 
 bool dwpw_f16s_supported(int c, int cout, int stride) {
     return c > 0 && c % 32 == 0 && cout > 0 && cout % 64 == 0 && (stride == 1 || stride == 2);
@@ -590,6 +866,8 @@
         if (bn == 256) return tw == 16 ? launch_v3<16, 256, 2>(p, n, act, s) : launch_v3<8, 256, 2>(p, n, act, s);
         return tw == 16 ? launch_v3<16, 128, 3>(p, n, act, s) : launch_v3<8, 128, 3>(p, n, act, s);
     }
+    if (dwpw_s2_covered(c, cout, stride) && !g_s2_off && in_bytes < (1ll << 32) - 16 && out_bytes < (1ll << 32) - 16)
+        return launch_s2(p, n, act, s);
     int bn = cout % 128 == 0 ? 128 : 64;
     if (g_bn && cout % g_bn == 0) bn = g_bn;
     int tw = (ow % 16 == 0 || ow % 8 != 0) ? 16 : 8;
diff --git a/hse_facerec_tf_amd/csrc/engine.hip b/hse_facerec_tf_amd/csrc/engine.hip
--- a/hse_facerec_tf_amd/csrc/engine.hip
+++ b/hse_facerec_tf_amd/csrc/engine.hip
@@ -290,7 +290,8 @@
     }
     for (uint32_t i = 0; i < h.n_ops; ++i) {
         const hsefr_plan_op& o = ops[i];
-        HSEFR_REQUIRE((o.flags & ~(HSEFR_OPF_PAIR_NEXT | HSEFR_OPF_HEADS | HSEFR_OPF_OUT_SUB2)) == 0, HSEFR_ERR_INVALID, "plan op %u: unknown flags 0x%x", i, o.flags);
+        HSEFR_REQUIRE((o.flags & ~(HSEFR_OPF_PAIR_NEXT | HSEFR_OPF_HEADS | HSEFR_OPF_OUT_SUB2 | HSEFR_OPF_DWPW_NEXT)) == 0, HSEFR_ERR_INVALID,
+                      "plan op %u: unknown flags 0x%x", i, o.flags);
         HSEFR_REQUIRE(!(o.flags & HSEFR_OPF_OUT_SUB2) || (o.flags & HSEFR_OPF_PAIR_NEXT), HSEFR_ERR_INVALID, "plan op %u: OUT_SUB2 without PAIR_NEXT", i);
         if (o.flags & HSEFR_OPF_PAIR_NEXT) {
             HSEFR_REQUIRE(i + 1 < h.n_ops, HSEFR_ERR_INVALID, "plan op %u: PAIR_NEXT on the last op", i);
@@ -311,6 +312,30 @@
                           "plan op %u: PAIR_NEXT: the second output (buffer %d) aliases an operand of the first", i, b.out_buf);
             HSEFR_REQUIRE(conv1x1_pair_bf16_shape_supported(o.cin, o.cout, b.cout, c2), HSEFR_ERR_UNSUPPORTED,
                           "plan op %u: PAIR_NEXT %d -> %d -> %d (projection from %d) not covered", i, o.cin, o.cout, b.cout, c2);
+        }
+        if (o.flags & HSEFR_OPF_DWPW_NEXT) {
+            HSEFR_REQUIRE(o.flags == HSEFR_OPF_DWPW_NEXT && i + 1 < h.n_ops, HSEFR_ERR_INVALID, "plan op %u: DWPW_NEXT on the last op or beside another flag", i);
+            const hsefr_plan_op& b = ops[i + 1];
+            HSEFR_REQUIRE(o.kind == HSEFR_OP_DWCONV3X3 && o.stride == 2 && o.act == HSEFR_ACT_RELU6 && o.aux == 0 && o.cout == o.cin &&
+                              b.kind == HSEFR_OP_PWCONV_F16S && b.in_buf == o.out_buf && b.flags == 0 && b.h == o.oh && b.w == o.ow && b.oh == b.h &&
+                              b.ow == b.w && b.cin == o.cin && b.aux > 0 && b.aux <= 12,
+                          HSEFR_ERR_INVALID, "plan op %u: DWPW_NEXT needs a stride-2 depthwise 3x3 with ReLU6 and fp32 output, and behind it a split-f16 "
+                          "pointwise op without flags that reads it at the same pixels (a_log2 in [1, 12])", i);
+            HSEFR_REQUIRE(dwpw_s2_covered(o.cin, b.cout, o.stride), HSEFR_ERR_INVALID, "plan op %u: DWPW_NEXT %d -> %d channels not covered (128 -> 256)", i,
+                          o.cin, b.cout);
+            HSEFR_REQUIRE(b.out_buf != o.out_buf, HSEFR_ERR_INVALID, "plan op %u: DWPW_NEXT: the second output (buffer %d) aliases the depthwise tensor", i,
+                          b.out_buf);
+            HSEFR_REQUIRE(b.out_buf != o.in_buf || (uint64_t)bufs[o.in_buf].elems_per_image * bufs[o.in_buf].elem_bytes ==
+                                                       (uint64_t)bufs[o.out_buf].elems_per_image * bufs[o.out_buf].elem_bytes,
+                          HSEFR_ERR_INVALID, "plan op %u: DWPW_NEXT: buffers %d and %d exchange roles and must have one size", i, o.in_buf, o.out_buf);
+            for (uint32_t k = i + 2; k < h.n_ops; ++k) {
+                HSEFR_REQUIRE(ops[k].in_buf != o.out_buf && ops[k].res_buf != o.out_buf, HSEFR_ERR_INVALID,
+                              "plan op %u: DWPW_NEXT: op %u also reads the depthwise tensor (buffer %d)", i, k, o.out_buf);
+                if (ops[k].out_buf == o.out_buf) break;
+            }
+            for (int sl = 0; sl < HSEFR_N_OUTPUT_SLOTS; ++sl)
+                HSEFR_REQUIRE(h.out_buffer[sl] != o.out_buf && (b.out_buf != o.in_buf || h.out_buffer[sl] != o.in_buf), HSEFR_ERR_INVALID,
+                              "plan op %u: DWPW_NEXT: the depthwise tensor (or the buffer it exchanges roles with) is output slot %d", i, sl);
         }
         if (o.flags & HSEFR_OPF_HEADS) {
             HSEFR_REQUIRE(i + 3 < h.n_ops, HSEFR_ERR_INVALID, "plan op %u: HEADS needs three ops behind it", i);
@@ -472,6 +497,7 @@
     if (!strcmp(key, "dw_look2")) { set_dw_look2(value); return HSEFR_OK; }
     if (!strcmp(key, "sweep_alternate")) { g_sweep_alternate = value; return HSEFR_OK; }
     if (!strcmp(key, "clock_mode")) { set_clock_mode(value); return HSEFR_OK; }
+    if (!strcmp(key, "dwpw_s2_off")) { set_dwpw_s2_off(value); return HSEFR_OK; }
     if (!strcmp(key, "dwpws_tw")) { set_dwpws_tw(value); return HSEFR_OK; }
     if (!strcmp(key, "dwpws_bn")) { set_dwpws_bn(value); return HSEFR_OK; }
     if (!strcmp(key, "pw_ablate")) { set_pw_ablate(value); return HSEFR_OK; }
@@ -641,8 +667,9 @@
     return HSEFR_OK;
 }
 
-static int run_ops(hsefr_engine* e, const std::vector<void*>& tab, const void* d_input, int n, const std::vector<char>& needed,
-                   hipStream_t s, hipEvent_t* pev, bool input_u8 = false) {
+static int run_ops(hsefr_engine* e, const std::vector<void*>& tab_in, const void* d_input, int n, const std::vector<char>& needed,
+                   hipStream_t s, hipEvent_t* pev, bool input_u8 = false, bool every_tensor = false) {
+    std::vector<void*> tab(tab_in);
     const bool prof = pev != nullptr;
     unsigned launches = 0;
     if (prof) HSEFR_HIP_CHECK(hipEventRecord(pev[0], s));
@@ -680,6 +707,14 @@
                                     (const float*)blob_ptr(e, g.shift_off), (float*)out, (float*)tab[a.out_buf], (float*)tab[sm.out_buf],
                                     (float*)tab[g.out_buf], n, o.cin, a.cout, s);
             covered = 3;
+        } else if ((o.flags & HSEFR_OPF_DWPW_NEXT) && !every_tensor && !dwpw_s2_off() && needed[i + 1]) {
+            const hsefr_plan_op& b = e->ops[i + 1];
+            if (b.out_buf == o.in_buf) std::swap(tab[o.in_buf], tab[o.out_buf]);
+            rc = launch_dwpw_f16s((const float*)in, (const float*)blob_ptr(e, o.w_off), (const float*)blob_ptr(e, o.scale_off),
+                                  (const float*)blob_ptr(e, o.shift_off), blob_ptr(e, b.w_off), (const float*)blob_ptr(e, b.scale_off),
+                                  (const float*)blob_ptr(e, b.shift_off), (float*)tab[b.out_buf], n, o.h, o.w, o.cin, o.stride, o.pad_t, o.pad_l,
+                                  o.oh, o.ow, b.cout, b.aux, b.act, s);
+            covered = 1;
         } else
         switch (o.kind) {
             case HSEFR_OP_CONV_C3:
@@ -937,7 +972,7 @@
         }
         for (int sl = 0; sl < HSEFR_N_OUTPUT_SLOTS; ++sl)
             if (outs[sl] && src_of[sl] == e->d_bufs[e->hdr.out_buffer[sl]]) src_of[sl] = tab[e->hdr.out_buffer[sl]];
-        const int rc = run_ops(e, tab, d_input, n, needed, s, prof ? pev : nullptr, input_u8);
+        const int rc = run_ops(e, tab, d_input, n, needed, s, prof ? pev : nullptr, input_u8, mask == 0);
         if (rc != HSEFR_OK) return rc;
         for (int sl = 0; sl < HSEFR_N_OUTPUT_SLOTS; ++sl)
             if (outs[sl] && src_of[sl])
@@ -965,7 +1000,10 @@
     for (size_t i = 0; i < e.ops.size(); ++i) {
         std::fill(only.begin(), only.end(), 0);
         only[i] = 1;
-        const size_t span = (e.ops[i].flags & HSEFR_OPF_PAIR_NEXT) ? 1 : (e.ops[i].flags & HSEFR_OPF_HEADS) ? 3 : 0;
+        const size_t span = (e.ops[i].flags & HSEFR_OPF_PAIR_NEXT)                      ? 1
+                            : (e.ops[i].flags & HSEFR_OPF_HEADS)                        ? 3
+                            : ((e.ops[i].flags & HSEFR_OPF_DWPW_NEXT) && !dwpw_s2_off()) ? 1
+                                                                                        : 0;
         for (size_t k = 1; k <= span && i + k < e.ops.size(); ++k) only[i + k] = 1;
         std::string line = std::to_string(i) + "\t" + std::to_string(e.ops[i].kind) + "\t";
         g_route_sink = &line;
diff --git a/hse_facerec_tf_amd/csrc/fuzz_plan.cc b/hse_facerec_tf_amd/csrc/fuzz_plan.cc
--- a/hse_facerec_tf_amd/csrc/fuzz_plan.cc
+++ b/hse_facerec_tf_amd/csrc/fuzz_plan.cc
@@ -44,7 +44,7 @@
 int main(int argc, char** argv) {
     if (argc < 3) { fprintf(stderr, "usage: fuzz_plan <mutants per seed> <plan file>...\n"); return 2; }
     const long long per_seed = atoll(argv[1]);
-    static const int32_t edge32[] = {0, 1, -1, -2, -3, 2, 3, 7, 63, 64, 65, 127, 128, 255, 256, 511, 512, 4095, 4096, 65535, 65536, 0x7fffffff,
+    static const int32_t edge32[] = {0, 1, -1, -2, -3, 2, 3, 7, 8, 63, 64, 65, 127, 128, 255, 256, 511, 512, 4095, 4096, 65535, 65536, 0x7fffffff,
                                      (int32_t)0x80000000, (int32_t)0xffff0000, 1 << 20, 1 << 24, 1 << 30};
     static const uint64_t edge64[] = {0ull, 1ull, 15ull, 16ull, 17ull, 0xffffffffull, 0x100000000ull, 0x7fffffffffffffffull, 0x8000000000000000ull,
                                       0xffffffffffffffffull, 0xfffffffffffffff0ull};
diff --git a/hse_facerec_tf_amd/lowering.py b/hse_facerec_tf_amd/lowering.py
--- a/hse_facerec_tf_amd/lowering.py
+++ b/hse_facerec_tf_amd/lowering.py
@@ -30,7 +30,7 @@
 _HEADER = struct.Struct("<QIIIIII3i3IQ")
 _BUFFER = struct.Struct("<QII")
 _OP = struct.Struct("<II3i3i3i3i2iii5Q")
-OPF_PAIR_NEXT, OPF_HEADS, OPF_OUT_SUB2 = 1, 2, 4
+OPF_PAIR_NEXT, OPF_HEADS, OPF_OUT_SUB2, OPF_DWPW_NEXT = 1, 2, 4, 8
 AUX_C2_SHIFT, AUX_C2_BITS, AUX_STRIDE2_SHIFT, AUX_STRIDE2_BITS = 0, 12, 12, 2
 AUX_H2_SHIFT, AUX_H2_BITS, AUX_W2_SHIFT, AUX_W2_BITS = 14, 9, 23, 9
 AUX_LOG2_BITS, AUX_OUT_LOG2_SHIFT, AUX_IN_LOG2_SHIFT, AUX_IN_LOG2_BIAS, AUX_U8_BIT = 8, 8, 8, 64, 16
@@ -46,7 +46,7 @@
 PRODUCT_KERNEL_FAMILIES = frozenset({
     "stem5_stream_kernel", "stem4_fused_kernel", "stem3_fused_kernel", "stem2_fused_kernel", "conv3x3_c3_kernel", "conv3x3_c3_mfma_kernel",
     "dwconv3x3_kernel", "pwconv_f32_dma_kernel", "pwconv_f32_kernel", "pwconv_f16s_kernel", "pwconv_ps_kernel", "dwpw_fused_kernel",
-    "dwpw_f16s_kernel", "dwpw2_f16s_kernel", "dwpw3_f16s_kernel", "gap_kernel", "dense_kernel", "softmax_kernel", "heads_kernel",
+    "dwpw_f16s_kernel", "dwpw2_f16s_kernel", "dwpw3_f16s_kernel", "dwpws2_f16s_kernel", "gap_kernel", "dense_kernel", "softmax_kernel", "heads_kernel",
     "stem7s_stream_kernel", "stem7x7_pool_bf16_kernel", "stem7x7_bf16_kernel", "maxpool3x3s2_bf16_kernel", "conv_bf16_kernel", "conv1x1_bf16_kernel",
     "conv1x1_w4_bf16_kernel", "conv1x1_pair_bf16_kernel", "conv3x3_w2_bf16_kernel", "conv_dma_bf16_kernel", "gap_bf16_kernel",
     "conv_f32_mfma_kernel", "conv2d_f32_kernel", "maxpool_f32_kernel"})
@@ -776,6 +776,10 @@
         for j in range(i + 1):
             if last_use[j] == i and j not in pinned and layers[j].out_buf not in free:
                 free.append(layers[j].out_buf)
+    for i, L in enumerate(layers):
+        if L.flags & OPF_DWPW_NEXT and L.src >= 0 and i + 1 < len(layers) and layers[i + 1].out_buf == layers[L.src].out_buf:
+            a, b = layers[L.src].out_buf, L.out_buf
+            buffers[a] = buffers[b] = max(buffers[a], buffers[b])
     return buffers
 
 
@@ -1040,6 +1044,25 @@
     return rebuild(layers, drop, put)
 
 
+def dwpw_pair_covered(dw: Layer, pw: Layer) -> bool:
+    return dw.stride == 2 and dw.in_shape[2] == 128 and pw.out_shape[2] == 256
+
+
+def mark_dwpw_pairs(layers: List[Layer], keep: Sequence[int]) -> int:
+    consumers = consumers_of(layers)
+    n = 0
+    for i, dw in enumerate(layers):
+        j = sole_reader(consumers, i, keep)
+        if not (dw.kind == OP_DWCONV3X3 and dw.act == ACT_RELU6 and dw.out_split == 0 and dw.flags == 0 and j == i + 1):
+            continue
+        pw = layers[j]
+        if (pw.kind == OP_PWCONV_F32 and 0 < pw.a_log2 <= 12 and not pw.in_split and pw.flags == 0 and pw.res < 0 and
+                tuple(pw.in_shape) == tuple(dw.out_shape) and dwpw_pair_covered(dw, pw)):
+            dw.flags |= OPF_DWPW_NEXT
+            n += 1
+    return n
+
+
 def choose_pointwise_math(layers: List[Layer], pw_math: str) -> None:
     if pw_math not in ("auto", "f32", "f16split"):
         raise ValueError("pw_math must be 'auto', 'f32' or 'f16split', not %r" % (pw_math,))
@@ -1119,7 +1142,8 @@
                 feeds: Optional[Dict[str, object]] = None, fuse: bool = True, dtype: str = "f32",
                 pw_math: Optional[str] = None, fuse_stem_block: Optional[bool] = None, stem_fusion: Optional[str] = None,
                 block_fusion: Optional[str] = None, presplit: Optional[str] = None, input_bound: Optional[float] = None,
-                pwdw_fusion: Optional[str] = None, u8_mean_bgr: Optional[Sequence[float]] = None, launch_fusion: bool = True) -> Plan:
+                pwdw_fusion: Optional[str] = None, u8_mean_bgr: Optional[Sequence[float]] = None, launch_fusion: bool = True,
+                s2_fusion: Optional[str] = None) -> Plan:
     if dtype not in ("f32", "bf16", "f32g"):
         raise ValueError("dtype must be 'f32', 'bf16' or 'f32g', not %r" % (dtype,))
     in_node, _ = g.get_tensor_by_name(input_tensor)
@@ -1235,5 +1259,10 @@
             compact_pair_outputs(layers, keep())
         if dtype == "f32":
             mark_heads(layers)
+    s2_fusion = s2_fusion or "auto"
+    if s2_fusion not in ("auto", "none"):
+        raise ValueError("s2_fusion must be 'auto' or 'none', not %r" % (s2_fusion,))
+    if fuse and launch_fusion and dtype == "f32" and s2_fusion == "auto":
+        mark_dwpw_pairs(layers, keep())
     buffers = assign_buffers(layers, set(keep()))
     return Plan(layers, (input_hw[0], input_hw[1], low.in_c), buffers, out_layers, tensor_layer)
diff --git a/include/hsefr.h b/include/hsefr.h
--- a/include/hsefr.h
+++ b/include/hsefr.h
@@ -88,7 +88,8 @@
 typedef enum hsefr_op_flags {
     HSEFR_OPF_PAIR_NEXT = 1,
     HSEFR_OPF_HEADS = 2,
-    HSEFR_OPF_OUT_SUB2 = 4
+    HSEFR_OPF_OUT_SUB2 = 4,
+    HSEFR_OPF_DWPW_NEXT = 8
 } hsefr_op_flags;
 
 enum {
```
